# AnishDelft/ModelCompression

Measured on NVIDIA B200. Metric: yolov2_416_pruned_fwd_images_per_sec, higher is better.
Workload: dtype bf16

## Files before the change

include/mcb200.h:

```cpp
#ifndef MCB200_H_
#define MCB200_H_

#include <stddef.h>
#include <stdint.h>

#ifdef __cplusplus
extern "C" {
#endif

#define MCB200_VERSION 100
#define MC_MAX_SEGMENTS 64

int mc_version(void);
const char* mc_last_error_string(void);
int mc_device_ok(void);


int mc_kth_abs_select(const float* const* h_seg_ptrs, const int64_t* h_seg_sizes, int nseg,
                      int64_t k, float gamma, float* d_out3,
                      void* d_ws, size_t ws_bytes, void* stream);
size_t mc_workspace_bytes_kth_abs_select(int64_t n_total);

int mc_weight_prune_masks(const float* const* h_w_ptrs, float* const* h_mask_ptrs, const int64_t* h_seg_sizes,
                          int nseg, int64_t k, float gamma, float* d_out3, void* d_ws, size_t ws_bytes,
                          void* stream);
int mc_debug_select_used_fast(const void* d_ws, void* stream);
int mc_debug_select_tstamps(const void* d_ws, unsigned long long* h_out12, void* stream);

int mc_mask_apply_gt(float* const* h_w_ptrs, float* const* h_mask_ptrs, const int64_t* h_seg_sizes,
                     int nseg, const float* d_thr, int apply, void* stream);

int mc_apply_masks(float* const* h_w_ptrs, const float* const* h_mask_ptrs,
                   const int64_t* h_seg_sizes, int nseg, void* stream);

int mc_count_zeros(const float* const* h_w_ptrs, const int64_t* h_seg_sizes, int nseg,
                   int64_t* d_counts, void* stream);

int mc_masked_residual(const float* const* h_w_ptrs, const float* const* h_mask_ptrs,
                       const int64_t* h_seg_sizes, int nseg, double* d_out, void* stream);


int mc_filter_values(const float* const* h_w_ptrs, const int* h_O, const int* h_C, const int* h_kh,
                     const int* h_kw, int nlayers, float* d_values, void* stream);

int mc_filter_threshold(const float* d_values, int n, int64_t k, double gamma, double* d_thr,
                        void* d_ws, size_t ws_bytes, void* stream);
size_t mc_workspace_bytes_filter_threshold(int n);

int mc_filter_masks(const float* d_values, const double* d_thr, const int* h_O, const int* h_per_filter,
                    int nlayers, float* const* h_mask_ptrs, uint8_t* d_keep, void* stream);

int mc_filter_prune(const float* const* h_w_ptrs, const int* h_O, const int* h_C, const int* h_kh, const int* h_kw,
                    int nlayers, int64_t k, double gamma, float* d_values, double* d_thr,
                    float* const* h_mask_ptrs, uint8_t* d_keep, void* d_ws, size_t ws_bytes, void* stream);
size_t mc_workspace_bytes_filter_prune(void);

int mc_filter_prune_greedy(const float* const* h_w_ptrs, const int* h_O, const int* h_C, const int* h_kh,
                           const int* h_kw, int nlayers, int64_t zeros0, int64_t total_params, double perc,
                           int max_picks, int32_t* d_picks, int64_t* d_result, float* const* h_mask_ptrs,
                           void* d_ws, size_t ws_bytes, void* stream);
size_t mc_workspace_bytes_filter_prune_greedy(int n_filters);


int mc_decode_region(const float* d_head, int B, int H, int W, int A, int nc, const float* h_anchors,
                     float conf_thresh, int only_objectness,
                     float* d_boxes, float* d_cls, int* d_counts, void* stream);

int mc_nms_batched(float* d_boxes, const int* d_counts, int B, int cap, float nms_thresh,
                   int* d_keep, int* d_keep_counts, void* stream);

int mc_nms_detect(float* d_boxes, const int* d_counts, int B, int cap, float nms_thresh, int* d_keep,
                  int* d_keep_counts, const float* d_cls, int nc, float conf_thresh, int* d_row_counts,
                  int* d_cand_counts, void* stream);

int mc_compact_detections(const float* d_boxes, const int* d_keep, const int* d_keep_counts, const float* d_cls,
                          int B, int cap, int nc, float conf_thresh, int first_image,
                          const int64_t* d_row_offsets, float* d_out, void* stream);

int mc_bbox_ious(const float* d_boxes1, const float* d_boxes2, int64_t n, int x1y1x2y2, float* d_out, void* stream);


enum { MC_EPI_PNHWC = 0,
       MC_EPI_REORG2 = 1,
       MC_EPI_NCHW_F32 = 2,
       MC_EPI_DECODE = 4 };

typedef struct mc_decode_params {
  float* d_boxes;
  float* d_cls;
  float* d_head;
  int A, nc;
  float conf_thresh;
  int only_objectness;
  float anchors[32];
} mc_decode_params;

typedef struct mc_conv_desc {
  const void* d_in;
  const void* d_wpack;
  const float* d_scale;
  const float* d_shift;
  void* d_out;
  int B, H, W;
  int Cin, Cin_ld;
  int N, Npad;
  int ksize;
  int leaky;
  int epi_mode;
  int ldc, ch_off;
  int block_n;
  int stages;
  int block_k;
  int in_cols;
  const mc_decode_params* decode;
  void* d_ws;
  size_t ws_bytes;
  float* d_stat_sum;
  float* d_stat_sumsq;
} mc_conv_desc;

int mc_conv_fwd(const mc_conv_desc* desc, void* stream);
size_t mc_workspace_bytes_conv_fwd(const mc_conv_desc* desc);

int mc_conv_last_plan(int info[8]);

int mc_conv_direct_supported(int Cin, int N, int ksize);
int mc_conv_direct_fwd(const void* d_in, int in_is_nchw_f32, const float* d_w, const float* d_scale,
                       const float* d_shift, void* d_out, int B, int H, int W, int Cin, int Cin_ld, int N, int ldc,
                       int ksize, int leaky, int pool, void* stream);

int mc_conv_thin_geometry(int ksize, int Cin, int N, int pool, int N2, int* ct, int* nt, int* n2t);
int mc_conv_thin_fwd(const void* d_in, const float* h_w, const float* h_scale, const float* h_shift, const float* h_w2,
                     const float* h_scale2, const float* h_shift2, void* d_out, int B, int H, int W, int Cin, int Cin_ld,
                     int N, int ldc, int ksize, int leaky, int pool, int N2, int leaky2, void* stream);

int mc_conv_im2col_supported(int Cin, int in_is_nchw_f32, int N, int pool);
int mc_conv_im2col_geometry(int Cin, int in_is_nchw_f32, int N, int pool, int* cl, int* npos, int* nb, int* kpad);
int mc_conv_im2col_fwd(const void* d_in, int in_is_nchw_f32, const void* d_wexp, const float* d_scale,
                       const float* d_shift, void* d_out, int B, int H, int W, int Cin, int Cin_ld, int N, int ldc,
                       int leaky, int pool, void* stream);

int mc_conv_window_supported(int Cin, int in_kind, int N, int pool);
int mc_conv_window_geometry(int Cin, int in_kind, int N, int pool, int* npos, int* nb, int* kcols);
int mc_conv_window_fwd(const void* d_in, int in_kind, const void* d_w, const float* d_scale, const float* d_shift,
                       void* d_out, int B, int H, int W, int Cin, int N, int ldc, int leaky, int pool, void* stream);

int mc_debug_conv_trace(void* d_buf);

int mc_debug_im2col_timeout(void);

int mc_pack_conv_weights(const float* d_w, const float* d_mask, int O, int C, int ksize,
                         const int* d_oidx, int n_o, const int* d_cidx, int n_c,
                         void* d_wpack, int Npad, int Kc, void* stream);

int mc_maxpool2x2(const void* d_in, void* d_out, int B, int H, int W, int C, int ld_in, int ld_out,
                  void* stream);

int mc_unpack_pnhwc(const void* d_in, float* d_out, int B, int H, int W, int C, int ld_in, int ch_off,
                    void* stream);

int mc_reorg_nchw(const float* d_in, float* d_out, int B, int C, int H, int W, int stride, void* stream);

int mc_pack_pnhwc(const float* d_in, void* d_out, int B, int H, int W, int C, int ld_out, void* stream);



int mc_col_stats(const void* d_z, int64_t rows, int C, int ld, int ch_off, float* d_sum, float* d_sumsq, void* stream);

int mc_bn_finalize(const float* d_sum, const float* d_sumsq, int C, double count, const float* d_gamma,
                   const float* d_beta, float eps, float momentum, float* d_running_mean, float* d_running_var,
                   float* d_scale, float* d_shift, float* d_mean, float* d_invstd, void* stream);

int mc_bn_apply(const void* d_z, int ld_z, int B, int H, int W, int C, const float* d_scale, const float* d_shift,
                int leaky, void* d_out, int ld_out, int ch_off, int reorg, void* stream);

int mc_bn_backward(const void* d_z, int ld_z, const void* d_da, int ld_da, int ch_off, int reorg, int B, int H, int W,
                   int C, const float* d_mean, const float* d_invstd, const float* d_gamma, const float* d_beta,
                   int leaky, float* d_dbeta, float* d_dgamma, void* d_dz, int ld_dz, void* stream);

int mc_maxpool2x2_backward(const void* d_a_full, int ld_a, const void* d_dpooled, int ld_dp, int B, int H, int W, int C,
                           void* d_dfull, int ld_df, int accumulate, void* stream);

int mc_bn_pool_supported(int C);
int mc_bn_apply_pool(const void* d_z, int ld_z, int B, int H, int W, int C, const float* d_scale, const float* d_shift,
                     int leaky, void* d_pooled, int ld_p, void* stream);
int mc_bn_pool_backward(const void* d_z, int ld_z, const void* d_dpooled, int ld_dp, int B, int H, int W, int C,
                        const float* d_scale, const float* d_shift, const float* d_mean, const float* d_invstd,
                        const float* d_gamma, const float* d_beta, int leaky, float* d_dbeta, float* d_dgamma, void* d_dz,
                        int ld_dz, void* stream);

size_t mc_workspace_bytes_region_loss(int nB);
int mc_region_loss(const float* d_output, const float* d_target, int nB, int nA, int nC, int nH, int nW,
                   const double* h_anchors, float coord_scale, float noobject_scale, float object_scale,
                   float class_scale, float thresh, float* d_grad, float* d_loss, int* d_counts, void* d_ws,
                   size_t ws_bytes, void* stream);

int mc_voc_table(const float* d_dets, int64_t n, const float* d_sizes, float def_w, float def_h, int64_t* d_img,
                 int64_t* d_cls, double* d_conf, double* d_corners, void* stream);
size_t mc_workspace_bytes_voc_match(int64_t n, int64_t m);
int mc_voc_match(const int64_t* d_key, const double* d_corners, int64_t n, const int64_t* d_gkey, const double* d_gbox,
                 const uint8_t* d_gdiff, int64_t m, double ovthresh, double* d_tp, double* d_fp, void* d_ws,
                 size_t ws_bytes, void* stream);

int mc_pack_conv_weights_dgrad(const float* d_w, const float* d_mask, int O, int C, int ksize, void* d_wpack, int Cpad,
                               int Ko, void* stream);

int mc_conv_wgrad(const void* d_a, int lda, int C, const void* d_dz, int ld_dz, int O, int B, int H, int W, int ksize,
                  const float* d_mask, float* d_dw, int accumulate, void* d_ws, size_t ws_bytes, void* stream);
size_t mc_workspace_bytes_conv_wgrad(int B, int H, int W, int C, int O, int ksize);

size_t mc_workspace_bytes_conv_wgrad_first(int B, int H, int W, int C, int O);
int mc_conv_wgrad_first(const float* d_x, const void* d_dz, int ld_dz, int B, int H, int W, int C, int O,
                        const float* d_mask, float* d_dw, void* d_ws, size_t ws_bytes, void* stream);

int mc_sgd_momentum_step(float* const* h_param_ptrs, const float* const* h_grad_ptrs, float* const* h_buf_ptrs,
                         const int64_t* h_sizes, int nseg, float lr, float momentum, float weight_decay,
                         int first_step, void* stream);

#ifdef __cplusplus
}
#endif
#endif
```

modelcompression_b200/_lib.py:

```python
import ctypes
import os
from ctypes import (POINTER, c_char_p, c_double, c_float, c_int, c_int64, c_size_t, c_uint8, c_void_p)

_HERE = os.path.dirname(os.path.abspath(__file__))
LIB_PATH = os.path.join(_HERE, "libmcb200.so")

MC_MAX_SEGMENTS = 64
MC_EPI_PNHWC, MC_EPI_REORG2, MC_EPI_NCHW_F32, MC_EPI_DECODE = 0, 1, 2, 4


class McError(RuntimeError):
    """A libmcb200 entry point returned a non-zero status."""


class mc_decode_params(ctypes.Structure):
    _fields_ = [
        ("d_boxes", c_void_p), ("d_cls", c_void_p), ("d_head", c_void_p),
        ("A", c_int), ("nc", c_int), ("conf_thresh", c_float), ("only_objectness", c_int),
        ("anchors", c_float * 32),
    ]


class mc_conv_desc(ctypes.Structure):
    _fields_ = [
        ("d_in", c_void_p), ("d_wpack", c_void_p), ("d_scale", c_void_p), ("d_shift", c_void_p), ("d_out", c_void_p),
        ("B", c_int), ("H", c_int), ("W", c_int),
        ("Cin", c_int), ("Cin_ld", c_int),
        ("N", c_int), ("Npad", c_int),
        ("ksize", c_int), ("leaky", c_int), ("epi_mode", c_int),
        ("ldc", c_int), ("ch_off", c_int),
        ("block_n", c_int), ("stages", c_int), ("block_k", c_int), ("in_cols", c_int),
        ("decode", POINTER(mc_decode_params)),
        ("d_ws", c_void_p), ("ws_bytes", c_size_t),
        ("d_stat_sum", c_void_p), ("d_stat_sumsq", c_void_p),
    ]


_SIGNATURES = {
    "mc_version": (c_int, []),
    "mc_last_error_string": (c_char_p, []),
    "mc_device_ok": (c_int, []),
    "mc_kth_abs_select": (c_int, [POINTER(c_void_p), POINTER(c_int64), c_int, c_int64, c_float, c_void_p,
                                  c_void_p, c_size_t, c_void_p]),
    "mc_workspace_bytes_kth_abs_select": (c_size_t, [c_int64]),
    "mc_weight_prune_masks": (c_int, [POINTER(c_void_p), POINTER(c_void_p), POINTER(c_int64), c_int, c_int64, c_float,
                                      c_void_p, c_void_p, c_size_t, c_void_p]),
    "mc_debug_select_used_fast": (c_int, [c_void_p, c_void_p]),
    "mc_debug_select_tstamps": (c_int, [c_void_p, c_void_p, c_void_p]),
    "mc_mask_apply_gt": (c_int, [POINTER(c_void_p), POINTER(c_void_p), POINTER(c_int64), c_int, c_void_p, c_int,
                                 c_void_p]),
    "mc_apply_masks": (c_int, [POINTER(c_void_p), POINTER(c_void_p), POINTER(c_int64), c_int, c_void_p]),
    "mc_count_zeros": (c_int, [POINTER(c_void_p), POINTER(c_int64), c_int, c_void_p, c_void_p]),
    "mc_masked_residual": (c_int, [POINTER(c_void_p), POINTER(c_void_p), POINTER(c_int64), c_int, c_void_p,
                                   c_void_p]),
    "mc_filter_values": (c_int, [POINTER(c_void_p), POINTER(c_int), POINTER(c_int), POINTER(c_int), POINTER(c_int),
                                 c_int, c_void_p, c_void_p]),
    "mc_filter_threshold": (c_int, [c_void_p, c_int, c_int64, c_double, c_void_p, c_void_p, c_size_t, c_void_p]),
    "mc_workspace_bytes_filter_threshold": (c_size_t, [c_int]),
    "mc_filter_masks": (c_int, [c_void_p, c_void_p, POINTER(c_int), POINTER(c_int), c_int, POINTER(c_void_p),
                                c_void_p, c_void_p]),
    "mc_filter_prune": (c_int, [POINTER(c_void_p), POINTER(c_int), POINTER(c_int), POINTER(c_int), POINTER(c_int), c_int,
                                c_int64, c_double, c_void_p, c_void_p, POINTER(c_void_p), c_void_p, c_void_p, c_size_t,
                                c_void_p]),
    "mc_workspace_bytes_filter_prune": (c_size_t, []),
    "mc_filter_prune_greedy": (c_int, [POINTER(c_void_p), POINTER(c_int), POINTER(c_int), POINTER(c_int),
                                       POINTER(c_int), c_int, c_int64, c_int64, c_double, c_int, c_void_p, c_void_p,
                                       POINTER(c_void_p), c_void_p, c_size_t, c_void_p]),
    "mc_workspace_bytes_filter_prune_greedy": (c_size_t, [c_int]),
    "mc_decode_region": (c_int, [c_void_p, c_int, c_int, c_int, c_int, c_int, POINTER(c_float), c_float, c_int,
                                 c_void_p, c_void_p, c_void_p, c_void_p]),
    "mc_nms_batched": (c_int, [c_void_p, c_void_p, c_int, c_int, c_float, c_void_p, c_void_p, c_void_p]),
    "mc_nms_detect": (c_int, [c_void_p, c_void_p, c_int, c_int, c_float, c_void_p, c_void_p, c_void_p, c_int, c_float,
                              c_void_p, c_void_p, c_void_p]),
    "mc_compact_detections": (c_int, [c_void_p, c_void_p, c_void_p, c_void_p, c_int, c_int, c_int, c_float, c_int,
                                      c_void_p, c_void_p, c_void_p]),
    "mc_bbox_ious": (c_int, [c_void_p, c_void_p, c_int64, c_int, c_void_p, c_void_p]),
    "mc_reorg_nchw": (c_int, [c_void_p, c_void_p, c_int, c_int, c_int, c_int, c_int, c_void_p]),
    "mc_conv_fwd": (c_int, [POINTER(mc_conv_desc), c_void_p]),
    "mc_workspace_bytes_conv_fwd": (c_size_t, [POINTER(mc_conv_desc)]),
    "mc_conv_last_plan": (c_int, [POINTER(c_int)]),
    "mc_conv_direct_supported": (c_int, [c_int, c_int, c_int]),
    "mc_conv_direct_fwd": (c_int, [c_void_p, c_int, c_void_p, c_void_p, c_void_p, c_void_p, c_int, c_int, c_int, c_int,
                                   c_int, c_int, c_int, c_int, c_int, c_int, c_void_p]),
    "mc_conv_thin_geometry": (c_int, [c_int, c_int, c_int, c_int, c_int, POINTER(c_int), POINTER(c_int), POINTER(c_int)]),
    "mc_conv_thin_fwd": (c_int, [c_void_p, c_void_p, c_void_p, c_void_p, c_void_p, c_void_p, c_void_p, c_void_p, c_int,
                                 c_int, c_int, c_int, c_int, c_int, c_int, c_int, c_int, c_int, c_int, c_int, c_void_p]),
    "mc_conv_im2col_supported": (c_int, [c_int, c_int, c_int, c_int]),
    "mc_conv_im2col_geometry": (c_int, [c_int, c_int, c_int, c_int, POINTER(c_int), POINTER(c_int), POINTER(c_int),
                                        POINTER(c_int)]),
    "mc_conv_im2col_fwd": (c_int, [c_void_p, c_int, c_void_p, c_void_p, c_void_p, c_void_p, c_int, c_int, c_int, c_int,
                                   c_int, c_int, c_int, c_int, c_int, c_void_p]),
    "mc_debug_im2col_timeout": (c_int, []),
    "mc_debug_conv_trace": (c_int, [c_void_p]),
    "mc_conv_window_supported": (c_int, [c_int, c_int, c_int, c_int]),
    "mc_conv_window_geometry": (c_int, [c_int, c_int, c_int, c_int, POINTER(c_int), POINTER(c_int), POINTER(c_int)]),
    "mc_conv_window_fwd": (c_int, [c_void_p, c_int, c_void_p, c_void_p, c_void_p, c_void_p, c_int, c_int, c_int, c_int,
                                   c_int, c_int, c_int, c_int, c_void_p]),
    "mc_pack_conv_weights": (c_int, [c_void_p, c_void_p, c_int, c_int, c_int, c_void_p, c_int, c_void_p, c_int,
                                     c_void_p, c_int, c_int, c_void_p]),
    "mc_maxpool2x2": (c_int, [c_void_p, c_void_p, c_int, c_int, c_int, c_int, c_int, c_int, c_void_p]),
    "mc_unpack_pnhwc": (c_int, [c_void_p, c_void_p, c_int, c_int, c_int, c_int, c_int, c_int, c_void_p]),
    "mc_pack_pnhwc": (c_int, [c_void_p, c_void_p, c_int, c_int, c_int, c_int, c_int, c_void_p]),
    "mc_col_stats": (c_int, [c_void_p, c_int64, c_int, c_int, c_int, c_void_p, c_void_p, c_void_p]),
    "mc_bn_finalize": (c_int, [c_void_p, c_void_p, c_int, c_double, c_void_p, c_void_p, c_float, c_float, c_void_p,
                               c_void_p, c_void_p, c_void_p, c_void_p, c_void_p, c_void_p]),
    "mc_bn_apply": (c_int, [c_void_p, c_int, c_int, c_int, c_int, c_int, c_void_p, c_void_p, c_int, c_void_p, c_int,
                            c_int, c_int, c_void_p]),
    "mc_bn_backward": (c_int, [c_void_p, c_int, c_void_p, c_int, c_int, c_int, c_int, c_int, c_int, c_int, c_void_p,
                               c_void_p, c_void_p, c_void_p, c_int, c_void_p, c_void_p, c_void_p, c_int, c_void_p]),
    "mc_maxpool2x2_backward": (c_int, [c_void_p, c_int, c_void_p, c_int, c_int, c_int, c_int, c_int, c_void_p, c_int,
                                       c_int, c_void_p]),
    "mc_workspace_bytes_region_loss": (c_size_t, [c_int]),
    "mc_region_loss": (c_int, [c_void_p, c_void_p, c_int, c_int, c_int, c_int, c_int, POINTER(c_double), c_float, c_float,
                               c_float, c_float, c_float, c_void_p, c_void_p, c_void_p, c_void_p, c_size_t, c_void_p]),
    "mc_voc_table": (c_int, [c_void_p, c_int64, c_void_p, c_float, c_float, c_void_p, c_void_p, c_void_p, c_void_p, c_void_p]),
    "mc_workspace_bytes_voc_match": (c_size_t, [c_int64, c_int64]),
    "mc_voc_match": (c_int, [c_void_p, c_void_p, c_int64, c_void_p, c_void_p, c_void_p, c_int64, c_double, c_void_p,
                             c_void_p, c_void_p, c_size_t, c_void_p]),
    "mc_bn_pool_supported": (c_int, [c_int]),
    "mc_bn_apply_pool": (c_int, [c_void_p, c_int, c_int, c_int, c_int, c_int, c_void_p, c_void_p, c_int, c_void_p, c_int,
                                 c_void_p]),
    "mc_bn_pool_backward": (c_int, [c_void_p, c_int, c_void_p, c_int, c_int, c_int, c_int, c_int, c_void_p, c_void_p,
                                    c_void_p, c_void_p, c_void_p, c_void_p, c_int, c_void_p, c_void_p, c_void_p, c_int,
                                    c_void_p]),
    "mc_pack_conv_weights_dgrad": (c_int, [c_void_p, c_void_p, c_int, c_int, c_int, c_void_p, c_int, c_int, c_void_p]),
    "mc_conv_wgrad": (c_int, [c_void_p, c_int, c_int, c_void_p, c_int, c_int, c_int, c_int, c_int, c_int, c_void_p,
                              c_void_p, c_int, c_void_p, c_size_t, c_void_p]),
    "mc_workspace_bytes_conv_wgrad": (c_size_t, [c_int, c_int, c_int, c_int, c_int, c_int]),
    "mc_conv_wgrad_first": (c_int, [c_void_p, c_void_p, c_int, c_int, c_int, c_int, c_int, c_int, c_void_p, c_void_p,
                                    c_void_p, c_size_t, c_void_p]),
    "mc_workspace_bytes_conv_wgrad_first": (c_size_t, [c_int, c_int, c_int, c_int, c_int]),
    "mc_sgd_momentum_step": (c_int, [POINTER(c_void_p), POINTER(c_void_p), POINTER(c_void_p), POINTER(c_int64), c_int,
                                     c_float, c_float, c_float, c_int, c_void_p]),
}

EXPORTED_SYMBOLS = tuple(sorted(_SIGNATURES))

_lib = None


def load():
    global _lib
    if _lib is not None:
        return _lib
    if not os.path.exists(LIB_PATH):
        raise ImportError(
            "modelcompression_b200: %s is not built. There is no CPU/PyTorch fallback for this path; build it with "
            "`python -c 'import __graft_entry__ as g; g.build()'` or `make -C modelcompression_b200/csrc`." % LIB_PATH)
    lib = ctypes.CDLL(LIB_PATH)
    for name, (res, args) in _SIGNATURES.items():
        fn = getattr(lib, name)
        fn.restype = res
        fn.argtypes = args
    _lib = lib
    return lib


def check(rc, what=""):
    if rc != 0:
        msg = load().mc_last_error_string()
        raise McError("%s failed (%d): %s" % (what or "libmcb200 call", rc, msg.decode() if msg else "?"))


def stream_ptr():
    import torch
    return c_void_p(torch.cuda.current_stream().cuda_stream)


def ptr_array(tensors):
    arr = (c_void_p * len(tensors))()
    for i, t in enumerate(tensors):
        arr[i] = None if t is None else t.data_ptr()
    return arr


def int64_array(vals):
    return (c_int64 * len(vals))(*[int(v) for v in vals])


def int_array(vals):
    return (c_int * len(vals))(*[int(v) for v in vals])


def require_cuda(t, what):
    if not t.is_cuda:
        raise RuntimeError(
            "%s: tensor is on %s. modelcompression_b200 runs this path on a B200 (sm_100a) only; there is no CPU "
            "fallback (move the model/tensors to CUDA)." % (what, t.device))
```

modelcompression_b200/csrc/conv_tcgen05.cu:

```cuda
#include <cuda.h>
#include <stdio.h>
#include <stdlib.h>
#include "common.cuh"
#include "ptx_sm100.cuh"
#include "tmap.cuh"
#include "decode_math.cuh"

namespace {

constexpr int BLOCK_M = 128;
constexpr int MAX_STAGES = 8;
constexpr int MAX_A_STAGES = 3;
constexpr int A_BOX_ROWS = BLOCK_M + 8;
constexpr int A_BOX_BYTES = A_BOX_ROWS * 128;
constexpr int A_BOX_STRIDE = 18 * 1024;
constexpr int ACC_STAGES = 2;
constexpr int NUM_THREADS = 192;

struct ConvKParams {
  int M_rows;
  int N;
  int Npad;
  int num_kb;
  int kb_per_tap;
  int block_k;
  int ksize;
  int Wp, Hp, W, H;
  int block_n, stages, tmem_cols, acc_stride;
  int out_pitch;
  int out_chunk;
  int tma_bufs;
  float* stat_sum;
  float* stat_sumsq;
  unsigned int wp_mul, wp_shr, hp_mul, hp_shr;
  int last_ksteps;
  int share_dx, a_stages;
  int m_tiles, n_tiles;
  uint32_t idesc;
  const float* scale;
  const float* shift;
  void* out;
  int ldc, ch_off, epi_mode, leaky;
  int sk_first, sk_units;
  int sk_gper, sk_total_g;
  int sk_clusters;
  unsigned int* sk_count;
  float* sk_part;
  float* dec_boxes;
  float* dec_cls;
  float* dec_head;
  int dec_A, dec_nc, dec_only_obj;
  float dec_thresh;
  McAnchors dec_anc;
  unsigned long long* dbg;
};

__device__ __forceinline__ void conv_stamp(const ConvKParams& p, int slot) {
  if (p.dbg != nullptr && slot < 32) {
    unsigned long long t;
    asm volatile("mov.u64 %0, %%globaltimer;" : "=l"(t));
    p.dbg[(size_t)blockIdx.x * 32 + slot] = t;
  }
}

template <bool LEAKY>
__device__ __forceinline__ void scale_act16(const uint32_t (&r)[16], const float* __restrict__ sc,
                                            const float* __restrict__ sh, bool interior, float (&v)[16]) {
#pragma unroll
  for (int q = 0; q < 4; ++q) {
    const float4 a = *reinterpret_cast<const float4*>(sc + 4 * q);
    const float4 b = *reinterpret_cast<const float4*>(sh + 4 * q);
    v[4 * q + 0] = fmaf(__uint_as_float(r[4 * q + 0]), a.x, b.x);
    v[4 * q + 1] = fmaf(__uint_as_float(r[4 * q + 1]), a.y, b.y);
    v[4 * q + 2] = fmaf(__uint_as_float(r[4 * q + 2]), a.z, b.z);
    v[4 * q + 3] = fmaf(__uint_as_float(r[4 * q + 3]), a.w, b.w);
  }
#pragma unroll
  for (int j = 0; j < 16; ++j) {
    if (LEAKY) v[j] = fmaxf(v[j], 0.1f * v[j]);
    v[j] = interior ? v[j] : 0.f;
  }
}

template <int MODE>
__device__ __forceinline__ void store16(const ConvKParams& p, const float (&v)[16], int nbase, long long out_row_base,
                                        bool vec_ok) {
  if (MODE == MC_EPI_NCHW_F32 || MODE == MC_EPI_DECODE) {
    float* out_f = reinterpret_cast<float*>(p.out);
    const long long hw = (long long)p.H * p.W;
#pragma unroll
    for (int j = 0; j < 16; ++j)
      if (nbase + j < p.N) out_f[out_row_base + (long long)(nbase + j) * hw] = v[j];
  } else {
    __nv_bfloat16* out_bf = reinterpret_cast<__nv_bfloat16*>(p.out) + out_row_base;
#pragma unroll
    for (int g = 0; g < 2; ++g) {
      const int n = nbase + g * 8;
      if (n >= p.N) continue;
      const bool full = n + 8 <= p.N;
      if (vec_ok && (full || (MODE == MC_EPI_PNHWC && p.ch_off + n + 8 <= p.ldc))) {
        float w[8];
#pragma unroll
        for (int j = 0; j < 8; ++j) w[j] = (full || n + j < p.N) ? v[g * 8 + j] : 0.f;
        __nv_bfloat162 h0 = __floats2bfloat162_rn(w[0], w[1]);
        __nv_bfloat162 h1 = __floats2bfloat162_rn(w[2], w[3]);
        __nv_bfloat162 h2 = __floats2bfloat162_rn(w[4], w[5]);
        __nv_bfloat162 h3 = __floats2bfloat162_rn(w[6], w[7]);
        uint4 pk;
        pk.x = *reinterpret_cast<uint32_t*>(&h0);
        pk.y = *reinterpret_cast<uint32_t*>(&h1);
        pk.z = *reinterpret_cast<uint32_t*>(&h2);
        pk.w = *reinterpret_cast<uint32_t*>(&h3);
        *reinterpret_cast<uint4*>(out_bf + n) = pk;
      } else {
#pragma unroll
        for (int j = 0; j < 8; ++j)
          if (n + j < p.N) out_bf[n + j] = __float2bfloat16_rn(v[g * 8 + j]);
      }
    }
  }
}

__device__ __forceinline__ void pack16_to_smem(const float (&v)[16], uint8_t* dst) {
#pragma unroll
  for (int g = 0; g < 2; ++g) {
    __nv_bfloat162 h0 = __floats2bfloat162_rn(v[g * 8 + 0], v[g * 8 + 1]);
    __nv_bfloat162 h1 = __floats2bfloat162_rn(v[g * 8 + 2], v[g * 8 + 3]);
    __nv_bfloat162 h2 = __floats2bfloat162_rn(v[g * 8 + 4], v[g * 8 + 5]);
    __nv_bfloat162 h3 = __floats2bfloat162_rn(v[g * 8 + 6], v[g * 8 + 7]);
    uint4 pk;
    pk.x = *reinterpret_cast<uint32_t*>(&h0);
    pk.y = *reinterpret_cast<uint32_t*>(&h1);
    pk.z = *reinterpret_cast<uint32_t*>(&h2);
    pk.w = *reinterpret_cast<uint32_t*>(&h3);
    *reinterpret_cast<uint4*>(dst + g * 16) = pk;
  }
}

__device__ __forceinline__ void pack16_to_slab(const float (&v)[16], uint8_t* row, int chunk, int lane) {
#pragma unroll
  for (int g = 0; g < 2; ++g) {
    __nv_bfloat162 h0 = __floats2bfloat162_rn(v[g * 8 + 0], v[g * 8 + 1]);
    __nv_bfloat162 h1 = __floats2bfloat162_rn(v[g * 8 + 2], v[g * 8 + 3]);
    __nv_bfloat162 h2 = __floats2bfloat162_rn(v[g * 8 + 4], v[g * 8 + 5]);
    __nv_bfloat162 h3 = __floats2bfloat162_rn(v[g * 8 + 6], v[g * 8 + 7]);
    uint4 pk;
    pk.x = *reinterpret_cast<uint32_t*>(&h0);
    pk.y = *reinterpret_cast<uint32_t*>(&h1);
    pk.z = *reinterpret_cast<uint32_t*>(&h2);
    pk.w = *reinterpret_cast<uint32_t*>(&h3);
    *reinterpret_cast<uint4*>(row + (((chunk + g) ^ (lane & 7)) << 4)) = pk;
  }
}

__device__ __forceinline__ void slab_stats(const uint8_t* sb, float* acc , int col0, int lane) {
  float s0 = 0.f, s1 = 0.f, q0 = 0.f, q1 = 0.f;
  const int j = lane >> 2, w = lane & 3;
#pragma unroll 8
  for (int r = 0; r < 32; ++r) {
    const uint32_t u = *reinterpret_cast<const uint32_t*>(sb + r * 128 + ((j ^ (r & 7)) << 4) + w * 4);
    const float a = __uint_as_float(u << 16), b = __uint_as_float(u & 0xffff0000u);
    s0 += a; s1 += b;
    q0 = fmaf(a, a, q0); q1 = fmaf(b, b, q1);
  }
  acc[col0 + 2 * lane] += s0;
  acc[col0 + 2 * lane + 1] += s1;
  acc[256 + col0 + 2 * lane] += q0;
  acc[256 + col0 + 2 * lane + 1] += q1;
}
__device__ __forceinline__ void flush_stats(const ConvKParams& p, float* acc, int n0, int lane) {
  for (int c = lane; c < p.block_n; c += 32) {
    if (n0 + c < p.N) {
      atomicAdd(p.stat_sum + n0 + c, acc[c]);
      atomicAdd(p.stat_sumsq + n0 + c, acc[256 + c]);
    }
    acc[c] = 0.f;
    acc[256 + c] = 0.f;
  }
  __syncwarp();
}

template <bool LEAKY, bool PAIR, bool WIDE_LD, typename AddFn>
__device__ __forceinline__ void epilogue_tile_tma(const ConvKParams& p, const CUtensorMap* tm_out, uint32_t taddr_row,
                                                  const float* sc, const float* sh, bool interior, bool in_buf,
                                                  int row0, int n0, long long out_row_base, bool vec_ok, uint8_t* slab,
                                                  int& buf, uint64_t* empty_bar, AddFn add, float* stat_acc = nullptr) {
  const int lane = threadIdx.x & 31;
  int cols_valid = ((p.N - n0 + 7) >> 3) << 3;
  if (cols_valid > p.block_n) cols_valid = p.block_n;
  const int full_cols = p.block_n & ~63;
  for (int cc = 0; cc < full_cols && cc < cols_valid; cc += 64) {
    uint8_t* sb = slab + (size_t)buf * 4096;
    if (lane == 0) {
      if (p.tma_bufs >= 2) ptx::bulk_wait_group_read<1>();
      else ptx::bulk_wait_group_read<0>();
    }
    __syncwarp();
    uint8_t* mine = sb + lane * 128;
    if (WIDE_LD) {
      uint32_t r[4][16];
#pragma unroll
      for (int q = 0; q < 4; ++q) ptx::tmem_ld_32x32b_x16(taddr_row + (uint32_t)(cc + 16 * q), r[q]);
      ptx::tmem_ld_wait();
#pragma unroll
      for (int q = 0; q < 4; ++q) {
        add(r[q], cc + 16 * q);
        float v[16];
        scale_act16<LEAKY>(r[q], sc + cc + 16 * q, sh + cc + 16 * q, interior, v);
        pack16_to_slab(v, mine, 2 * q, lane);
      }
    } else {
#pragma unroll
      for (int h = 0; h < 2; ++h) {
        uint32_t r0[16], r1[16];
        ptx::tmem_ld_32x32b_x16(taddr_row + (uint32_t)(cc + 32 * h), r0);
        ptx::tmem_ld_32x32b_x16(taddr_row + (uint32_t)(cc + 32 * h + 16), r1);
        ptx::tmem_ld_wait();
        add(r0, cc + 32 * h);
        add(r1, cc + 32 * h + 16);
        float v[16];
        scale_act16<LEAKY>(r0, sc + cc + 32 * h, sh + cc + 32 * h, interior, v);
        pack16_to_slab(v, mine, 4 * h, lane);
        scale_act16<LEAKY>(r1, sc + cc + 32 * h + 16, sh + cc + 32 * h + 16, interior, v);
        pack16_to_slab(v, mine, 4 * h + 2, lane);
      }
    }
    ptx::fence_proxy_async_smem();
    __syncwarp();
    if (lane == 0) {
      ptx::tma_store_2d(tm_out, sb, n0 + cc, row0);
      ptx::bulk_commit_group();
    }
    if (stat_acc != nullptr) slab_stats(sb, stat_acc, cc, lane);
    if (p.tma_bufs >= 2) buf ^= 1;
  }
  for (int c0 = full_cols; c0 < p.block_n; c0 += 32) {
    uint32_t r0[16], r1[16];
    const bool two = c0 + 16 < p.block_n;
    ptx::tmem_ld_32x32b_x16(taddr_row + (uint32_t)c0, r0);
    if (two) ptx::tmem_ld_32x32b_x16(taddr_row + (uint32_t)(c0 + 16), r1);
    ptx::tmem_ld_wait();
    if (!in_buf) continue;
    add(r0, c0);
    if (two) add(r1, c0 + 16);
    float v[16];
    scale_act16<LEAKY>(r0, sc + c0, sh + c0, interior, v);
    store16<MC_EPI_PNHWC>(p, v, n0 + c0, out_row_base, vec_ok);
    if (two) {
      scale_act16<LEAKY>(r1, sc + c0 + 16, sh + c0 + 16, interior, v);
      store16<MC_EPI_PNHWC>(p, v, n0 + c0 + 16, out_row_base, vec_ok);
    }
  }
  ptx::tc_fence_before();
  __syncwarp();
  if (lane == 0) {
    if (PAIR) ptx::mbar_arrive_leader(empty_bar);
    else ptx::mbar_arrive(empty_bar);
  }
}

template <int MODE, bool LEAKY, bool PAIR = false, bool WIDE_LD = false>
__device__ __forceinline__ void epilogue_loop(const ConvKParams& p, uint32_t tmem_base, uint64_t* tmem_full_bar,
                                              uint64_t* tmem_empty_bar, float* s_ss, uint8_t* s_out = nullptr,
                                              const CUtensorMap* tm_out = nullptr,
                                              int tile0 = -1, int tile_step = 0, int total_units = 0, int pair_rank = 0) {
  const int warp_idx = threadIdx.x >> 5;
  const int lane = threadIdx.x & 31;
  const int et = threadIdx.x - 64;
  const int quarter = warp_idx & 3;
  const int total_tiles = PAIR ? total_units : p.m_tiles * p.n_tiles;
  if (!PAIR) { tile0 = blockIdx.x; tile_step = gridDim.x; }
  const bool vec_ok = ((p.ldc | p.ch_off) & 7) == 0 && (MODE != MC_EPI_REORG2 || (p.N & 7) == 0);
  int as = 0;
  uint32_t aphase = 0;
  int slab_buf = 0;
  float* stat_acc = nullptr;
  int stat_n0 = -1;
  if (MODE == MC_EPI_PNHWC && p.tma_bufs > 0 && p.stat_sum != nullptr) {
    stat_acc = reinterpret_cast<float*>(s_out + (size_t)4 * p.tma_bufs * 4096) + quarter * 512;
    for (int c = lane; c < 512; c += 32) stat_acc[c] = 0.f;
    __syncwarp();
  }
  const bool one_n_tile = p.n_tiles == 1;
  if (one_n_tile) {
    for (int i = et; i < p.block_n; i += 128) {
      const bool ok = i < p.Npad;
      s_ss[i] = ok ? __ldg(p.scale + i) : 0.f;
      s_ss[256 + i] = ok ? __ldg(p.shift + i) : 0.f;
    }
    asm volatile("bar.sync 1, 128;" ::: "memory");
  }
  int ti = 0;
  for (int tile = tile0; tile < total_tiles; tile += tile_step, ++ti) {
    const int n0 = (tile % p.n_tiles) * p.block_n;
    const int m0 = (PAIR ? 2 * (tile / p.n_tiles) + pair_rank : tile / p.n_tiles) * BLOCK_M;
    float* sc = s_ss + (one_n_tile ? 0 : as * 512);
    float* sh = sc + 256;
    if (!one_n_tile) {
      for (int i = et; i < p.block_n; i += 128) {
        const bool ok = (n0 + i) < p.Npad;
        sc[i] = ok ? __ldg(p.scale + n0 + i) : 0.f;
        sh[i] = ok ? __ldg(p.shift + n0 + i) : 0.f;
      }
    }
    const int row = m0 + quarter * 32 + lane;
    const int t = (int)(__umulhi((unsigned int)row, p.wp_mul) >> p.wp_shr);
    const int x = row - t * p.Wp;
    const int b = (int)(__umulhi((unsigned int)t, p.hp_mul) >> p.hp_shr);
    const int y = t - b * p.Hp;
    const bool in_buf = row < p.M_rows;
    const bool interior = in_buf && (x < p.W) && (y < p.H);
    long long out_row_base = 0;
    bool do_store = false;
    if (MODE == MC_EPI_PNHWC) {
      out_row_base = (long long)row * p.ldc + p.ch_off;
      do_store = in_buf;
    } else if (MODE == MC_EPI_REORG2) {
      const int Wo = p.W / 2 + 1, Ho = p.H / 2 + 1;
      const long long orow = ((long long)b * Ho + (y >> 1)) * Wo + (x >> 1);
      out_row_base = orow * p.ldc + p.ch_off + ((y & 1) * 2 + (x & 1)) * p.N;
      do_store = interior;
    } else {
      out_row_base = ((long long)b * p.N * p.H + y) * p.W + x;
      do_store = interior;
    }
    if (!one_n_tile) asm volatile("bar.sync 1, 128;" ::: "memory");

    ptx::mbar_wait(&tmem_full_bar[as], aphase);
    ptx::tc_fence_after();
    if (!PAIR && et == 0 && ti < 8) conv_stamp(p, 12 + 2 * ti);
    const uint32_t taddr_row = tmem_base + ((uint32_t)(quarter * 32) << 16) + (uint32_t)(as * p.acc_stride);

    if (MODE == MC_EPI_PNHWC && p.tma_bufs > 0) {
      if (stat_acc != nullptr && n0 != stat_n0) {
        if (stat_n0 >= 0) flush_stats(p, stat_acc, stat_n0, lane);
        stat_n0 = n0;
      }
      epilogue_tile_tma<LEAKY, PAIR, WIDE_LD>(p, tm_out, taddr_row, sc, sh, interior, in_buf, m0 + quarter * 32, n0, out_row_base,
                                     vec_ok, s_out + (size_t)quarter * p.tma_bufs * 4096, slab_buf, &tmem_empty_bar[as],
                                     [](uint32_t (&)[16], int) {}, stat_acc);
      if (!PAIR && et == 0 && ti < 8) conv_stamp(p, 13 + 2 * ti);
      if (++as == ACC_STAGES) { as = 0; aphase ^= 1u; }
      continue;
    }

    if (MODE == MC_EPI_PNHWC && s_out != nullptr) {
      const int pitch = p.out_pitch;
      const int chunk = p.out_chunk;
      uint8_t* wbuf = s_out + (size_t)quarter * 32 * pitch;
      uint8_t* mine = wbuf + (size_t)lane * pitch;
      const int row0 = m0 + quarter * 32;
      int cols_left = ((p.N - n0 + 7) >> 3) << 3;
      if (cols_left > p.block_n) cols_left = p.block_n;
      for (int cc = 0; cc < p.block_n; cc += chunk) {
        const int cw = (p.block_n - cc < chunk) ? p.block_n - cc : chunk;
        for (int c0 = 0; c0 < cw; c0 += 32) {
          uint32_t r0[16], r1[16];
          const bool two = c0 + 16 < cw;
          ptx::tmem_ld_32x32b_x16(taddr_row + (uint32_t)(cc + c0), r0);
          if (two) ptx::tmem_ld_32x32b_x16(taddr_row + (uint32_t)(cc + c0 + 16), r1);
          ptx::tmem_ld_wait();
          float v[16];
          scale_act16<LEAKY>(r0, sc + cc + c0, sh + cc + c0, interior, v);
          pack16_to_smem(v, mine + c0 * 2);
          if (two) {
            scale_act16<LEAKY>(r1, sc + cc + c0 + 16, sh + cc + c0 + 16, interior, v);
            pack16_to_smem(v, mine + (c0 + 16) * 2);
          }
        }
        if (cc + chunk >= p.block_n) {
          ptx::tc_fence_before();
          __syncwarp();
          if (lane == 0) {
            if (PAIR) ptx::mbar_arrive_leader(&tmem_empty_bar[as]);
            else ptx::mbar_arrive(&tmem_empty_bar[as]);
          }
        } else {
          __syncwarp();
        }
        int cols_w = cols_left - cc;
        if (cols_w > cw) cols_w = cw;
        if (cols_w > 0) {
          const int cpr = cols_w >> 3;
          int r = lane / cpr, c = lane - r * cpr;
          const int dr = 32 / cpr, dc = 32 - dr * cpr;
          __nv_bfloat16* obase = reinterpret_cast<__nv_bfloat16*>(p.out) + p.ch_off + n0 + cc;
          while (r < 32) {
            if (row0 + r < p.M_rows)
              *reinterpret_cast<uint4*>(obase + (long long)(row0 + r) * p.ldc + c * 8) =
                  *reinterpret_cast<const uint4*>(wbuf + (size_t)r * pitch + c * 16);
            r += dr; c += dc;
            if (c >= cpr) { c -= cpr; ++r; }
          }
        }
        __syncwarp();
      }
      if (!PAIR && et == 0 && ti < 8) conv_stamp(p, 13 + 2 * ti);
      if (++as == ACC_STAGES) { as = 0; aphase ^= 1u; }
      continue;
    }

    if (MODE == MC_EPI_DECODE) {
      const int pitch_f = p.block_n + 1;
      float* mine = reinterpret_cast<float*>(s_out) + (size_t)(quarter * 32 + lane) * pitch_f;
      for (int c0 = 0; c0 < p.block_n; c0 += 16) {
        uint32_t r0[16];
        ptx::tmem_ld_32x32b_x16(taddr_row + (uint32_t)c0, r0);
        ptx::tmem_ld_wait();
        float v[16];
        scale_act16<LEAKY>(r0, sc + c0, sh + c0, true, v);
#pragma unroll
        for (int j = 0; j < 16; ++j) mine[c0 + j] = v[j];
      }
      ptx::tc_fence_before();
      __syncwarp();
      if (lane == 0) ptx::mbar_arrive(&tmem_empty_bar[as]);
      if (interior) {
        const int A = p.dec_A, nc = p.dec_nc, F = 5 + p.dec_nc;
        const long long P = (long long)p.H * p.W * A;
        const long long slot0 = (long long)(y * p.W + x) * A;
        if (p.dec_head != nullptr) {
          float* hd = p.dec_head + ((long long)b * p.N * p.H + y) * p.W + x;
          const long long hw = (long long)p.H * p.W;
          for (int n = 0; n < p.N; ++n) hd[n * hw] = mine[n];
        }
        for (int a = 0; a < A; ++a) {
          const float* row = mine + a * F;
          const McDecoded d = mc_decode_anchor([row](int f) { return row[f]; }, nc, x, y, p.W, p.H, p.dec_anc.w[a],
                                               p.dec_anc.h[a], p.dec_thresh, p.dec_only_obj);
          float* dst = p.dec_boxes + ((long long)b * P + slot0 + a) * 8;
          reinterpret_cast<float4*>(dst)[0] = make_float4(d.bx, d.by, d.bw, d.bh);
          reinterpret_cast<float4*>(dst)[1] =
              make_float4(d.conf, d.cmax, (float)d.cid, d.cand ? (float)(slot0 + a) : -1.0f);
          if (d.cand && p.dec_cls != nullptr) {
            float* cd = p.dec_cls + ((long long)b * P + slot0 + a) * nc;
            for (int c = 0; c < nc; ++c) cd[c] = __fdiv_rn(expf(__fsub_rn(row[5 + c], d.cls_max_logit)), d.cls_sum);
          }
        }
      }
      __syncwarp();
      if (++as == ACC_STAGES) { as = 0; aphase ^= 1u; }
      continue;
    }

    for (int c0 = 0; c0 < p.block_n; c0 += 32) {
      uint32_t r0[16], r1[16];
      const bool two = c0 + 16 < p.block_n;
      ptx::tmem_ld_32x32b_x16(taddr_row + (uint32_t)c0, r0);
      if (two) ptx::tmem_ld_32x32b_x16(taddr_row + (uint32_t)(c0 + 16), r1);
      ptx::tmem_ld_wait();
      if (!do_store) continue;
      float v[16];
      scale_act16<LEAKY>(r0, sc + c0, sh + c0, interior, v);
      store16<MODE>(p, v, n0 + c0, out_row_base, vec_ok);
      if (two) {
        scale_act16<LEAKY>(r1, sc + c0 + 16, sh + c0 + 16, interior, v);
        store16<MODE>(p, v, n0 + c0 + 16, out_row_base, vec_ok);
      }
    }
    ptx::tc_fence_before();
    __syncwarp();
    if (lane == 0) {
      if (PAIR) ptx::mbar_arrive_leader(&tmem_empty_bar[as]);
      else ptx::mbar_arrive(&tmem_empty_bar[as]);
    }
    if (!PAIR && et == 0 && ti < 8) conv_stamp(p, 13 + 2 * ti);
    if (++as == ACC_STAGES) { as = 0; aphase ^= 1u; }
  }
  if (stat_acc != nullptr && stat_n0 >= 0) flush_stats(p, stat_acc, stat_n0, lane);
  if (MODE == MC_EPI_PNHWC && p.tma_bufs > 0 && lane == 0) ptx::bulk_wait_group_read<0>();
}

template <int MINB>
__global__ void __launch_bounds__(NUM_THREADS, MINB)
conv_gemm_tcgen05_kernel(const __grid_constant__ CUtensorMap tmap_a, const __grid_constant__ CUtensorMap tmap_b,
                         const __grid_constant__ CUtensorMap tmap_abox, const __grid_constant__ CUtensorMap tmap_out,
                         const ConvKParams p) {
  extern __shared__ __align__(1024) uint8_t smem_raw[];
  const uint32_t a_tile_bytes = (uint32_t)(BLOCK_M * p.block_k * 2);
  const uint32_t b_tile_bytes = (uint32_t)(p.block_n * p.block_k * 2);
  const uint32_t stage_bytes = a_tile_bytes + b_tile_bytes;
  uint8_t* smem = smem_raw;
  {
    uint32_t a = ptx::smem_u32(smem);
    smem += (1024u - (a & 1023u)) & 1023u;
  }
  uint8_t* tiles = smem;
  const uint32_t a_row_bytes = (uint32_t)p.block_k * 2u;
  const uint32_t a_box_bytes = (uint32_t)A_BOX_ROWS * a_row_bytes;
  const uint32_t a_box_stride = p.block_k == 64 ? (uint32_t)A_BOX_STRIDE : (uint32_t)A_BOX_STRIDE / 2u;
  uint8_t* b_ring = tiles + (size_t)p.a_stages * a_box_stride;
  uint8_t* aux = p.share_dx ? b_ring + (size_t)p.stages * b_tile_bytes : tiles + (size_t)p.stages * stage_bytes;
  uint64_t* full_bar = reinterpret_cast<uint64_t*>(aux);
  uint64_t* empty_bar = full_bar + MAX_STAGES;
  uint64_t* tmem_full_bar = empty_bar + MAX_STAGES;
  uint64_t* tmem_empty_bar = tmem_full_bar + ACC_STAGES;
  uint64_t* afull_bar = tmem_empty_bar + ACC_STAGES;
  uint64_t* aempty_bar = afull_bar + MAX_A_STAGES;
  uint32_t* tmem_ptr_smem = reinterpret_cast<uint32_t*>(aempty_bar + MAX_A_STAGES);
  float* s_ss = reinterpret_cast<float*>(aux + 512);
  uint8_t* s_out = aux + 5120;

  const int warp_idx = threadIdx.x >> 5;
  const int lane = threadIdx.x & 31;
  const int total_tiles = p.m_tiles * p.n_tiles;
  if (threadIdx.x == 0) conv_stamp(p, 0);

  if (warp_idx == 0 && lane == 0) {
    ptx::prefetch_tensormap(&tmap_a);
    ptx::prefetch_tensormap(&tmap_b);
    for (int s = 0; s < p.stages; ++s) {
      ptx::mbar_init(&full_bar[s], 1);
      ptx::mbar_init(&empty_bar[s], 1);
    }
    for (int a = 0; a < ACC_STAGES; ++a) {
      ptx::mbar_init(&tmem_full_bar[a], 1);
      ptx::mbar_init(&tmem_empty_bar[a], 4);
    }
    for (int a = 0; a < MAX_A_STAGES; ++a) {
      ptx::mbar_init(&afull_bar[a], 1);
      ptx::mbar_init(&aempty_bar[a], 1);
    }
    ptx::prefetch_tensormap(&tmap_abox);
    if (p.tma_bufs > 0) ptx::prefetch_tensormap(&tmap_out);
    ptx::fence_barrier_init();
  }
  if (warp_idx == 1) {
    ptx::tmem_alloc(tmem_ptr_smem, (uint32_t)p.tmem_cols);
    ptx::tmem_relinquish();
  }
  ptx::tc_fence_before();
  __syncthreads();
  ptx::tc_fence_after();
  const uint32_t tmem_base = *tmem_ptr_smem;
  if (threadIdx.x == 0) conv_stamp(p, 1);

  if (warp_idx == 0) {
    if (lane == 0 && p.share_dx) {
      int s = 0, sa = 0;
      uint32_t phase = 0, pha = 0;
      for (int tile = blockIdx.x; tile < total_tiles; tile += gridDim.x) {
        const int n0 = (tile % p.n_tiles) * p.block_n;
        const int m0 = (tile / p.n_tiles) * BLOCK_M;
        for (int g = 0; g < 3 * p.kb_per_tap; ++g) {
          const int dy = g / p.kb_per_tap, cb = g - dy * p.kb_per_tap;
          ptx::mbar_wait(&aempty_bar[sa], pha ^ 1u);
          ptx::mbar_arrive_expect_tx(&afull_bar[sa], a_box_bytes);
          ptx::tma_load_2d(tiles + (size_t)sa * a_box_stride, &tmap_abox, &afull_bar[sa], cb * p.block_k,
                           m0 + (dy - 1) * p.Wp - 1);
          if (++sa == p.a_stages) { sa = 0; pha ^= 1u; }
          for (int dx = 0; dx < 3; ++dx) {
            const int kb = (dy * 3 + dx) * p.kb_per_tap + cb;
            ptx::mbar_wait(&empty_bar[s], phase ^ 1u);
            ptx::mbar_arrive_expect_tx(&full_bar[s], b_tile_bytes);
            ptx::tma_load_2d(b_ring + (size_t)s * b_tile_bytes, &tmap_b, &full_bar[s], kb * p.block_k, n0);
            if (++s == p.stages) { s = 0; phase ^= 1u; }
          }
        }
      }
      conv_stamp(p, 3);
    } else if (lane == 0) {
      int s = 0;
      uint32_t phase = 0;
      for (int tile = blockIdx.x; tile < total_tiles; tile += gridDim.x) {
        const int n0 = (tile % p.n_tiles) * p.block_n;
        const int m0 = (tile / p.n_tiles) * BLOCK_M;
        for (int kb = 0; kb < p.num_kb; ++kb) {
          const int tap = kb / p.kb_per_tap;
          const int cb = kb - tap * p.kb_per_tap;
          int row_off = 0;
          if (p.ksize == 3) row_off = (tap / 3 - 1) * p.Wp + (tap % 3 - 1);
          ptx::mbar_wait(&empty_bar[s], phase ^ 1u);
          uint8_t* a_dst = tiles + (size_t)s * stage_bytes;
          uint8_t* b_dst = a_dst + a_tile_bytes;
          ptx::mbar_arrive_expect_tx(&full_bar[s], stage_bytes);
          ptx::tma_load_2d(a_dst, &tmap_a, &full_bar[s], cb * p.block_k, m0 + row_off);
          ptx::tma_load_2d(b_dst, &tmap_b, &full_bar[s], kb * p.block_k, n0);
          if (++s == p.stages) { s = 0; phase ^= 1u; }
        }
      }
      conv_stamp(p, 3);
    }
  } else if (warp_idx == 1) {
    if (p.share_dx) {
      int s = 0, sa = 0, as = 0;
      uint32_t phase = 0, pha = 0, aphase = 0;
      int ti = 0;
      for (int tile = blockIdx.x; tile < total_tiles; tile += gridDim.x, ++ti) {
        ptx::mbar_wait(&tmem_empty_bar[as], aphase ^ 1u);
        ptx::tc_fence_after();
        const uint32_t tmem_acc = tmem_base + (uint32_t)(as * p.acc_stride);
        for (int g = 0; g < 3 * p.kb_per_tap; ++g) {
          const int dy = g / p.kb_per_tap, cb = g - dy * p.kb_per_tap;
          const int nk = (cb == p.kb_per_tap - 1) ? p.last_ksteps : (int)(a_row_bytes >> 5);
          ptx::mbar_wait(&afull_bar[sa], pha);
          if (ti == 0 && g == 0 && lane == 0) conv_stamp(p, 4);
          const uint32_t a_addr = ptx::smem_u32(tiles + (size_t)sa * a_box_stride);
          for (int dx = 0; dx < 3; ++dx) {
            ptx::mbar_wait(&full_bar[s], phase);
            ptx::tc_fence_after();
            const uint32_t b_addr = ptx::smem_u32(b_ring + (size_t)s * b_tile_bytes);
            const bool k64 = p.block_k == 64;
            const uint64_t adesc = k64 ? ptx::make_sw128_kmajor_desc(a_addr + (uint32_t)dx * 128u)
                                       : ptx::make_sw64_kmajor_desc(a_addr + (uint32_t)dx * 64u);
            const uint64_t bdesc = k64 ? ptx::make_sw128_kmajor_desc(b_addr) : ptx::make_sw64_kmajor_desc(b_addr);
            if (ptx::elect_one()) {
#pragma unroll
              for (int k = 0; k < 4; ++k)
                if (k < nk)
                  ptx::umma_bf16_ss(tmem_acc, adesc + (uint64_t)(2 * k), bdesc + (uint64_t)(2 * k), p.idesc,
                                    (g > 0 || dx > 0 || k > 0) ? 1u : 0u);
              ptx::umma_commit(&empty_bar[s]);
              if (dx == 2) ptx::umma_commit(&aempty_bar[sa]);
              if (dx == 2 && g == 3 * p.kb_per_tap - 1) ptx::umma_commit(&tmem_full_bar[as]);
            }
            __syncwarp();
            if (++s == p.stages) { s = 0; phase ^= 1u; }
          }
          if (++sa == p.a_stages) { sa = 0; pha ^= 1u; }
        }
        if (lane == 0 && ti < 6) conv_stamp(p, 5 + ti);
        if (++as == ACC_STAGES) { as = 0; aphase ^= 1u; }
      }
    } else {
      int s = 0;
      uint32_t phase = 0;
      int as = 0;
      uint32_t aphase = 0;
      int ti = 0;
      for (int tile = blockIdx.x; tile < total_tiles; tile += gridDim.x, ++ti) {
        ptx::mbar_wait(&tmem_empty_bar[as], aphase ^ 1u);
        ptx::tc_fence_after();
        const uint32_t tmem_acc = tmem_base + (uint32_t)(as * p.acc_stride);
        int cb_i = 0;
        for (int kb = 0; kb < p.num_kb; ++kb) {
          ptx::mbar_wait(&full_bar[s], phase);
          ptx::tc_fence_after();
          if (ti == 0 && kb == 0 && lane == 0) conv_stamp(p, 4);
          const uint32_t a_addr = ptx::smem_u32(tiles + (size_t)s * stage_bytes);
          const bool k64 = p.block_k == 64;
          const uint64_t adesc = k64 ? ptx::make_sw128_kmajor_desc(a_addr) : ptx::make_sw64_kmajor_desc(a_addr);
          const uint64_t bdesc = k64 ? ptx::make_sw128_kmajor_desc(a_addr + a_tile_bytes)
                                     : ptx::make_sw64_kmajor_desc(a_addr + a_tile_bytes);
          const int ksteps = (cb_i == p.kb_per_tap - 1) ? p.last_ksteps : p.block_k / 16;
          if (++cb_i == p.kb_per_tap) cb_i = 0;
          if (ptx::elect_one()) {
#pragma unroll
            for (int k = 0; k < 4; ++k) {
              if (k < ksteps)
                ptx::umma_bf16_ss(tmem_acc, adesc + (uint64_t)(2 * k), bdesc + (uint64_t)(2 * k), p.idesc,
                                  (kb > 0 || k > 0) ? 1u : 0u);
            }
            ptx::umma_commit(&empty_bar[s]);
            if (kb == p.num_kb - 1) ptx::umma_commit(&tmem_full_bar[as]);
          }
          __syncwarp();
          if (++s == p.stages) { s = 0; phase ^= 1u; }
        }
        if (lane == 0 && ti < 6) conv_stamp(p, 5 + ti);
        if (++as == ACC_STAGES) { as = 0; aphase ^= 1u; }
      }
    }
  } else {
    if (p.epi_mode == MC_EPI_PNHWC) {
      uint8_t* so = (p.out_pitch || p.tma_bufs) ? s_out : nullptr;
      if (p.leaky) epilogue_loop<MC_EPI_PNHWC, true, false, MINB == 1>(p, tmem_base, tmem_full_bar, tmem_empty_bar, s_ss, so, &tmap_out);
      else epilogue_loop<MC_EPI_PNHWC, false, false, MINB == 1>(p, tmem_base, tmem_full_bar, tmem_empty_bar, s_ss, so, &tmap_out);
    } else if (p.epi_mode == MC_EPI_REORG2) {
      if (p.leaky) epilogue_loop<MC_EPI_REORG2, true>(p, tmem_base, tmem_full_bar, tmem_empty_bar, s_ss);
      else epilogue_loop<MC_EPI_REORG2, false>(p, tmem_base, tmem_full_bar, tmem_empty_bar, s_ss);
    } else if (p.epi_mode == MC_EPI_DECODE) {
      epilogue_loop<MC_EPI_DECODE, false>(p, tmem_base, tmem_full_bar, tmem_empty_bar, s_ss, s_out);
    } else {
      if (p.leaky) epilogue_loop<MC_EPI_NCHW_F32, true>(p, tmem_base, tmem_full_bar, tmem_empty_bar, s_ss);
      else epilogue_loop<MC_EPI_NCHW_F32, false>(p, tmem_base, tmem_full_bar, tmem_empty_bar, s_ss);
    }
  }

  ptx::tc_fence_before();
  __syncthreads();
  if (threadIdx.x == 0) conv_stamp(p, 30);
  if (warp_idx == 1) ptx::tmem_dealloc(tmem_base, (uint32_t)p.tmem_cols);
}

struct PairWork {
  int unit;
  int g0, g1;
  int kind;
  int aux;
};

struct PairWorkIter {
  int next_full, step, sk_first;
  int sk_state;
  int c, G, gper, T, units;
  __device__ __forceinline__ void init(const ConvKParams& p, int cluster_id, int num_clusters) {
    next_full = cluster_id;
    step = num_clusters;
    sk_first = p.sk_first;
    c = cluster_id; G = p.sk_clusters; gper = p.sk_gper; T = p.sk_total_g; units = p.sk_units;
    sk_state = (p.sk_units > 0 && c < G) ? 0 : 2;
  }
  __device__ __forceinline__ int span_begin(int cl) const { return (int)(((long long)cl * T) / G); }
  __device__ __forceinline__ void describe(int u, int a, int b, PairWork& w) const {
    w.unit = sk_first + u;
    w.g0 = a;
    w.g1 = b;
    int cf = c;
    while (cf > 0 && span_begin(cf) > u * gper) --cf;
    if (b == gper) {
      w.kind = (a == 0) ? 0 : 2;
      w.aux = c - cf;
    } else {
      w.kind = 1;
      w.aux = c - cf;
    }
  }
  __device__ __forceinline__ bool next(PairWork& w) {
    if (next_full < sk_first) {
      w.unit = next_full; w.g0 = 0; w.g1 = -1; w.kind = 0; w.aux = 0;
      next_full += step;
      return true;
    }
    if (sk_state == 2) return false;
    const int r0 = span_begin(c), r1 = span_begin(c + 1);
    if (r1 <= r0) { sk_state = 2; return false; }
    const int u0 = r0 / gper, u1 = (r1 - 1) / gper;
    if (u0 == u1) {
      sk_state = 2;
      describe(u0, r0 - u0 * gper, r1 - u0 * gper, w);
      return true;
    }
    if (sk_state == 0) {
      sk_state = 1;
      describe(u1, 0, r1 - u1 * gper, w);
      return true;
    }
    sk_state = 2;
    describe(u0, r0 - u0 * gper, gper, w);
    return true;
  }
};

template <int MODE, bool LEAKY>
__device__ __forceinline__ void epilogue_loop_pair(const ConvKParams& p, uint32_t tmem_base, uint64_t* tmem_full_bar,
                                                   uint64_t* tmem_empty_bar, float* s_ss, int cluster_id, int num_clusters,
                                                   int pair_rank, uint8_t* s_out, const CUtensorMap* tm_out) {
  const int warp_idx = threadIdx.x >> 5;
  const int lane = threadIdx.x & 31;
  const int et = threadIdx.x - 64;
  const int quarter = warp_idx & 3;
  const bool vec_ok = ((p.ldc | p.ch_off) & 7) == 0 && (MODE != MC_EPI_REORG2 || (p.N & 7) == 0);
  int as = 0;
  uint32_t aphase = 0;
  int slab_buf = 0;
  float* stat_acc = nullptr;
  int stat_n0 = -1;
  if (MODE == MC_EPI_PNHWC && p.tma_bufs > 0 && p.stat_sum != nullptr) {
    stat_acc = reinterpret_cast<float*>(s_out + (size_t)4 * p.tma_bufs * 4096) + quarter * 512;
    for (int c = lane; c < 512; c += 32) stat_acc[c] = 0.f;
    __syncwarp();
  }
  const bool one_n_tile = p.n_tiles == 1;
  if (one_n_tile) {
    for (int i = et; i < p.block_n; i += 128) {
      const bool ok = i < p.Npad;
      s_ss[i] = ok ? __ldg(p.scale + i) : 0.f;
      s_ss[256 + i] = ok ? __ldg(p.shift + i) : 0.f;
    }
    asm volatile("bar.sync 1, 128;" ::: "memory");
  }
  PairWorkIter it;
  it.init(p, cluster_id, num_clusters);
  PairWork w;
  int ti = -1;
  while (it.next(w)) {
    ++ti;
    const int tile = w.unit;
    const int n0 = (tile % p.n_tiles) * p.block_n;
    const int m0 = (2 * (tile / p.n_tiles) + pair_rank) * BLOCK_M;
    float* sc = s_ss + (one_n_tile ? 0 : as * 512);
    float* sh = sc + 256;
    if (!one_n_tile) {
      for (int i = et; i < p.block_n; i += 128) {
        const bool ok = (n0 + i) < p.Npad;
        sc[i] = ok ? __ldg(p.scale + n0 + i) : 0.f;
        sh[i] = ok ? __ldg(p.shift + n0 + i) : 0.f;
      }
    }
    const int row = m0 + quarter * 32 + lane;
    const int t = (int)(__umulhi((unsigned int)row, p.wp_mul) >> p.wp_shr);
    const int x = row - t * p.Wp;
    const int b = (int)(__umulhi((unsigned int)t, p.hp_mul) >> p.hp_shr);
    const int y = t - b * p.Hp;
    const bool in_buf = row < p.M_rows;
    const bool interior = in_buf && (x < p.W) && (y < p.H);
    long long out_row_base = 0;
    bool do_store = false;
    if (MODE == MC_EPI_PNHWC) {
      out_row_base = (long long)row * p.ldc + p.ch_off;
      do_store = in_buf;
    } else if (MODE == MC_EPI_REORG2) {
      const int Wo = p.W / 2 + 1, Ho = p.H / 2 + 1;
      const long long orow = ((long long)b * Ho + (y >> 1)) * Wo + (x >> 1);
      out_row_base = orow * p.ldc + p.ch_off + ((y & 1) * 2 + (x & 1)) * p.N;
      do_store = interior;
    } else {
      out_row_base = ((long long)b * p.N * p.H + y) * p.W + x;
      do_store = interior;
    }
    if (!one_n_tile) asm volatile("bar.sync 1, 128;" ::: "memory");

    ptx::mbar_wait(&tmem_full_bar[as], aphase);
    ptx::tc_fence_after();
    if (et == 0 && ti < 8) conv_stamp(p, 12 + 2 * ti);
    const uint32_t taddr_row = tmem_base + ((uint32_t)(quarter * 32) << 16) + (uint32_t)(as * p.acc_stride);
    const int u_sk = tile - p.sk_first;
    const int prow = pair_rank * 128 + quarter * 32 + lane;
    const size_t slot_stride = (size_t)256 * p.block_n;
    float* part_unit = p.sk_part + (size_t)(u_sk < 0 ? 0 : u_sk) * 3 * slot_stride;
    auto part_ptr = [&](int slot, int col) -> float* {
      return part_unit + (size_t)slot * slot_stride + ((size_t)(col >> 2) * 256 + prow) * 4;
    };
    if (w.kind == 1) {
      for (int c0 = 0; c0 < p.block_n; c0 += 32) {
        uint32_t r0[16], r1[16];
        const bool two = c0 + 16 < p.block_n;
        ptx::tmem_ld_32x32b_x16(taddr_row + (uint32_t)c0, r0);
        if (two) ptx::tmem_ld_32x32b_x16(taddr_row + (uint32_t)(c0 + 16), r1);
        ptx::tmem_ld_wait();
#pragma unroll
        for (int q = 0; q < 4; ++q)
          *reinterpret_cast<uint4*>(part_ptr(w.aux, c0 + 4 * q)) = make_uint4(r0[4 * q], r0[4 * q + 1], r0[4 * q + 2], r0[4 * q + 3]);
        if (two) {
#pragma unroll
          for (int q = 0; q < 4; ++q)
            *reinterpret_cast<uint4*>(part_ptr(w.aux, c0 + 16 + 4 * q)) = make_uint4(r1[4 * q], r1[4 * q + 1], r1[4 * q + 2], r1[4 * q + 3]);
        }
      }
      ptx::tc_fence_before();
      __threadfence();
      __syncwarp();
      if (lane == 0) {
        atomicAdd(p.sk_count + u_sk, 1u);
        ptx::mbar_arrive_leader(&tmem_empty_bar[as]);
      }
    } else {
      const int nparts = w.kind == 2 ? w.aux : 0;
      if (nparts > 0) {
        if (lane == 0) {
          const unsigned int want = 8u * (unsigned int)nparts;
          unsigned int spins = 0;
          while (*reinterpret_cast<volatile unsigned int*>(p.sk_count + u_sk) < want) {
            if (++spins > (1u << 24)) __trap();
          }
          if (atomicAdd(p.sk_count + 256 + u_sk, 1u) == 7u) {
            p.sk_count[256 + u_sk] = 0u;
            p.sk_count[u_sk] = 0u;
          }
        }
        __syncwarp();
        __threadfence();
      }
      if (MODE == MC_EPI_PNHWC && p.tma_bufs > 0) {
        if (stat_acc != nullptr && n0 != stat_n0) {
          if (stat_n0 >= 0) flush_stats(p, stat_acc, stat_n0, lane);
          stat_n0 = n0;
        }
        epilogue_tile_tma<LEAKY, true, true>(p, tm_out, taddr_row, sc, sh, interior, in_buf, m0 + quarter * 32, n0, out_row_base,
                                       vec_ok, s_out + (size_t)quarter * p.tma_bufs * 4096, slab_buf, &tmem_empty_bar[as],
                                       [&](uint32_t (&r)[16], int col) {
                                         for (int s2 = 0; s2 < nparts; ++s2) {
#pragma unroll
                                           for (int q = 0; q < 4; ++q) {
                                             const float4 a = __ldcg(reinterpret_cast<const float4*>(part_ptr(s2, col + 4 * q)));
                                             r[4 * q] = __float_as_uint(__uint_as_float(r[4 * q]) + a.x);
                                             r[4 * q + 1] = __float_as_uint(__uint_as_float(r[4 * q + 1]) + a.y);
                                             r[4 * q + 2] = __float_as_uint(__uint_as_float(r[4 * q + 2]) + a.z);
                                             r[4 * q + 3] = __float_as_uint(__uint_as_float(r[4 * q + 3]) + a.w);
                                           }
                                         }
                                       }, stat_acc);
        if (et == 0 && ti < 8) conv_stamp(p, 13 + 2 * ti);
        if (++as == ACC_STAGES) { as = 0; aphase ^= 1u; }
        continue;
      }
      for (int c0 = 0; c0 < p.block_n; c0 += 32) {
        uint32_t r0[16], r1[16];
        const bool two = c0 + 16 < p.block_n;
        ptx::tmem_ld_32x32b_x16(taddr_row + (uint32_t)c0, r0);
        if (two) ptx::tmem_ld_32x32b_x16(taddr_row + (uint32_t)(c0 + 16), r1);
        ptx::tmem_ld_wait();
        if (!do_store) continue;
        for (int s2 = 0; s2 < nparts; ++s2) {
#pragma unroll
          for (int q = 0; q < 4; ++q) {
            const float4 a = __ldcg(reinterpret_cast<const float4*>(part_ptr(s2, c0 + 4 * q)));
            r0[4 * q] = __float_as_uint(__uint_as_float(r0[4 * q]) + a.x);
            r0[4 * q + 1] = __float_as_uint(__uint_as_float(r0[4 * q + 1]) + a.y);
            r0[4 * q + 2] = __float_as_uint(__uint_as_float(r0[4 * q + 2]) + a.z);
            r0[4 * q + 3] = __float_as_uint(__uint_as_float(r0[4 * q + 3]) + a.w);
          }
          if (two) {
#pragma unroll
            for (int q = 0; q < 4; ++q) {
              const float4 a = __ldcg(reinterpret_cast<const float4*>(part_ptr(s2, c0 + 16 + 4 * q)));
              r1[4 * q] = __float_as_uint(__uint_as_float(r1[4 * q]) + a.x);
              r1[4 * q + 1] = __float_as_uint(__uint_as_float(r1[4 * q + 1]) + a.y);
              r1[4 * q + 2] = __float_as_uint(__uint_as_float(r1[4 * q + 2]) + a.z);
              r1[4 * q + 3] = __float_as_uint(__uint_as_float(r1[4 * q + 3]) + a.w);
            }
          }
        }
        float v[16];
        scale_act16<LEAKY>(r0, sc + c0, sh + c0, interior, v);
        store16<MODE>(p, v, n0 + c0, out_row_base, vec_ok);
        if (two) {
          scale_act16<LEAKY>(r1, sc + c0 + 16, sh + c0 + 16, interior, v);
          store16<MODE>(p, v, n0 + c0 + 16, out_row_base, vec_ok);
        }
      }
      ptx::tc_fence_before();
      __syncwarp();
      if (lane == 0) ptx::mbar_arrive_leader(&tmem_empty_bar[as]);
    }
    if (et == 0 && ti < 8) conv_stamp(p, 13 + 2 * ti);
    if (++as == ACC_STAGES) { as = 0; aphase ^= 1u; }
  }
  if (stat_acc != nullptr && stat_n0 >= 0) flush_stats(p, stat_acc, stat_n0, lane);
  if (MODE == MC_EPI_PNHWC && p.tma_bufs > 0 && lane == 0) ptx::bulk_wait_group_read<0>();
}

__global__ void __cluster_dims__(2, 1, 1) __launch_bounds__(NUM_THREADS, 1)
conv_gemm_tcgen05_pair_kernel(const __grid_constant__ CUtensorMap tmap_b, const __grid_constant__ CUtensorMap tmap_abox,
                              const __grid_constant__ CUtensorMap tmap_out, const ConvKParams p) {
  extern __shared__ __align__(1024) uint8_t smem_raw[];
  const uint32_t b_half_bytes = (uint32_t)(p.block_n / 2 * 128);
  uint8_t* smem = smem_raw;
  {
    uint32_t a = ptx::smem_u32(smem);
    smem += (1024u - (a & 1023u)) & 1023u;
  }
  uint8_t* tiles = smem;
  uint8_t* b_ring = tiles + (size_t)p.a_stages * A_BOX_STRIDE;
  uint8_t* aux = b_ring + (size_t)p.stages * b_half_bytes;
  uint64_t* full_bar = reinterpret_cast<uint64_t*>(aux);
  uint64_t* empty_bar = full_bar + MAX_STAGES;
  uint64_t* tmem_full_bar = empty_bar + MAX_STAGES;
  uint64_t* tmem_empty_bar = tmem_full_bar + ACC_STAGES;
  uint64_t* afull_bar = tmem_empty_bar + ACC_STAGES;
  uint64_t* aempty_bar = afull_bar + MAX_A_STAGES;
  uint32_t* tmem_ptr_smem = reinterpret_cast<uint32_t*>(aempty_bar + MAX_A_STAGES);
  float* s_ss = reinterpret_cast<float*>(aux + 512);
  uint8_t* s_out = aux + 5120;

  const int warp_idx = threadIdx.x >> 5;
  const int lane = threadIdx.x & 31;
  const int rank = (int)ptx::cluster_ctarank();
  const int cluster_id = blockIdx.x >> 1, num_clusters = gridDim.x >> 1;
  if (threadIdx.x == 0) conv_stamp(p, 0);

  if (warp_idx == 0 && lane == 0) {
    ptx::prefetch_tensormap(&tmap_b);
    ptx::prefetch_tensormap(&tmap_abox);
    if (p.tma_bufs > 0) ptx::prefetch_tensormap(&tmap_out);
    for (int s = 0; s < p.stages; ++s) {
      ptx::mbar_init(&full_bar[s], 1);
      ptx::mbar_init(&empty_bar[s], 1);
    }
    for (int a = 0; a < ACC_STAGES; ++a) {
      ptx::mbar_init(&tmem_full_bar[a], 1);
      ptx::mbar_init(&tmem_empty_bar[a], 8);
    }
    for (int a = 0; a < MAX_A_STAGES; ++a) {
      ptx::mbar_init(&afull_bar[a], 1);
      ptx::mbar_init(&aempty_bar[a], 1);
    }
    ptx::fence_barrier_init();
  }
  if (warp_idx == 1) {
    ptx::tmem_alloc_pair(tmem_ptr_smem, (uint32_t)p.tmem_cols);
    ptx::tmem_relinquish_pair();
  }
  ptx::tc_fence_before();
  ptx::cluster_sync_all();
  ptx::tc_fence_after();
  const uint32_t tmem_base = *tmem_ptr_smem;
  if (threadIdx.x == 0) conv_stamp(p, 1);

  if (warp_idx == 0) {
    if (lane == 0) {
      int s = 0, sa = 0;
      uint32_t phase = 0, pha = 0;
      PairWorkIter it;
      it.init(p, cluster_id, num_clusters);
      PairWork w;
      while (it.next(w)) {
        const int unit = w.unit;
        const int n0 = (unit % p.n_tiles) * p.block_n + rank * (p.block_n / 2);
        const int m0 = (2 * (unit / p.n_tiles) + rank) * BLOCK_M;
        const int gb = w.g0, ge = w.g1 < 0 ? 3 * p.kb_per_tap : w.g1;
        for (int g = gb; g < ge; ++g) {
          const int dy = g / p.kb_per_tap, cb = g - dy * p.kb_per_tap;
          ptx::mbar_wait(&aempty_bar[sa], pha ^ 1u);
          if (rank == 0) ptx::mbar_arrive_expect_tx(&afull_bar[sa], 2 * A_BOX_BYTES);
          ptx::tma_load_2d_pair(tiles + (size_t)sa * A_BOX_STRIDE, &tmap_abox, &afull_bar[sa], cb * 64,
                                m0 + (dy - 1) * p.Wp - 1);
          if (++sa == p.a_stages) { sa = 0; pha ^= 1u; }
          for (int dx = 0; dx < 3; ++dx) {
            const int kb = (dy * 3 + dx) * p.kb_per_tap + cb;
            ptx::mbar_wait(&empty_bar[s], phase ^ 1u);
            if (rank == 0) ptx::mbar_arrive_expect_tx(&full_bar[s], 2 * b_half_bytes);
            ptx::tma_load_2d_pair(b_ring + (size_t)s * b_half_bytes, &tmap_b, &full_bar[s], kb * 64, n0);
            if (++s == p.stages) { s = 0; phase ^= 1u; }
          }
        }
      }
      conv_stamp(p, 3);
    }
  } else if (warp_idx == 1) {
    if (rank == 0) {
      int s = 0, sa = 0, as = 0;
      uint32_t phase = 0, pha = 0, aphase = 0;
      PairWorkIter it;
      it.init(p, cluster_id, num_clusters);
      PairWork w;
      int ti = -1;
      while (it.next(w)) {
        ++ti;
        ptx::mbar_wait(&tmem_empty_bar[as], aphase ^ 1u);
        ptx::tc_fence_after();
        const uint32_t tmem_acc = tmem_base + (uint32_t)(as * p.acc_stride);
        const int gb = w.g0, ge = w.g1 < 0 ? 3 * p.kb_per_tap : w.g1;
        for (int g = gb; g < ge; ++g) {
          const int nk = ((g % p.kb_per_tap) == p.kb_per_tap - 1) ? p.last_ksteps : 4;
          ptx::mbar_wait(&afull_bar[sa], pha);
          if (ti == 0 && g == gb && lane == 0) conv_stamp(p, 4);
          const uint32_t a_addr = ptx::smem_u32(tiles + (size_t)sa * A_BOX_STRIDE);
          for (int dx = 0; dx < 3; ++dx) {
            ptx::mbar_wait(&full_bar[s], phase);
            ptx::tc_fence_after();
            const uint64_t adesc = ptx::make_sw128_kmajor_desc(a_addr + (uint32_t)dx * 128u);
            const uint64_t bdesc = ptx::make_sw128_kmajor_desc(ptx::smem_u32(b_ring + (size_t)s * b_half_bytes));
            if (ptx::elect_one()) {
#pragma unroll
              for (int k = 0; k < 4; ++k)
                if (k < nk)
                  ptx::umma_bf16_ss_pair(tmem_acc, adesc + (uint64_t)(2 * k), bdesc + (uint64_t)(2 * k), p.idesc,
                                         (g > gb || dx > 0 || k > 0) ? 1u : 0u);
              ptx::umma_commit_pair(&empty_bar[s]);
              if (dx == 2) ptx::umma_commit_pair(&aempty_bar[sa]);
              if (dx == 2 && g == ge - 1) ptx::umma_commit_pair(&tmem_full_bar[as]);
            }
            __syncwarp();
            if (++s == p.stages) { s = 0; phase ^= 1u; }
          }
          if (++sa == p.a_stages) { sa = 0; pha ^= 1u; }
        }
        if (lane == 0 && ti < 6) conv_stamp(p, 5 + ti);
        if (++as == ACC_STAGES) { as = 0; aphase ^= 1u; }
      }
    }
  } else {
    if (p.epi_mode == MC_EPI_PNHWC) {
      if (p.leaky) epilogue_loop_pair<MC_EPI_PNHWC, true>(p, tmem_base, tmem_full_bar, tmem_empty_bar, s_ss, cluster_id, num_clusters, rank, s_out, &tmap_out);
      else epilogue_loop_pair<MC_EPI_PNHWC, false>(p, tmem_base, tmem_full_bar, tmem_empty_bar, s_ss, cluster_id, num_clusters, rank, s_out, &tmap_out);
    } else if (p.epi_mode == MC_EPI_REORG2) {
      if (p.leaky) epilogue_loop_pair<MC_EPI_REORG2, true>(p, tmem_base, tmem_full_bar, tmem_empty_bar, s_ss, cluster_id, num_clusters, rank, s_out, &tmap_out);
      else epilogue_loop_pair<MC_EPI_REORG2, false>(p, tmem_base, tmem_full_bar, tmem_empty_bar, s_ss, cluster_id, num_clusters, rank, s_out, &tmap_out);
    } else {
      if (p.leaky) epilogue_loop_pair<MC_EPI_NCHW_F32, true>(p, tmem_base, tmem_full_bar, tmem_empty_bar, s_ss, cluster_id, num_clusters, rank, s_out, &tmap_out);
      else epilogue_loop_pair<MC_EPI_NCHW_F32, false>(p, tmem_base, tmem_full_bar, tmem_empty_bar, s_ss, cluster_id, num_clusters, rank, s_out, &tmap_out);
    }
  }

  ptx::tc_fence_before();
  ptx::cluster_sync_all();
  if (warp_idx == 1) ptx::tmem_dealloc_pair(tmem_base, (uint32_t)p.tmem_cols);
}

int pick_block_n(int Npad, int m_tiles, int num_kb, int num_sms, bool share_dx) {
  int best = 16;
  double best_cost = 1e30;
  for (int bn = 16; bn <= 256; bn += 16) {
    const int n_tiles = (Npad + bn - 1) / bn;
    const long long tiles = (long long)n_tiles * m_tiles;
    const long long rounds = (tiles + num_sms - 1) / num_sms;
    double per_kb = 2.0 * bn;
    if (128.0 + bn > per_kb) per_kb = 128.0 + bn;
    const double feed = 13.3 * ((share_dx ? 17.0 / 3.0 : 16.0) + bn / 8.0);
    if (feed > per_kb) per_kb = feed;
    const double main = per_kb * num_kb, epi = 12.0 * bn + 400.0;
    const double cost = (double)rounds * (main > epi ? main : epi) + epi + 2500.0;
    if (cost < best_cost - 1e-9) {
      best_cost = cost;
      best = bn;
    }
  }
  return best;
}

}

static thread_local int g_last_plan[8] = {0, 0, 0, 0, 0, 0, 0, 0};
static unsigned long long* g_conv_dbg = nullptr;

extern "C" int mc_debug_conv_trace(void* d_buf) {
  g_conv_dbg = reinterpret_cast<unsigned long long*>(d_buf);
  return 0;
}

extern "C" int mc_conv_last_plan(int info[8]) {
  MC_CHECK_ARG(info != nullptr, "mc_conv_last_plan: null pointer");
  for (int i = 0; i < 8; ++i) info[i] = g_last_plan[i];
  return 0;
}

extern "C" size_t mc_workspace_bytes_conv_fwd(const mc_conv_desc* d) {
  if (d == nullptr || d->ksize != 3 || d->Cin <= 32 || d->Npad < 192) return 0;
  const int clusters = mc_num_sms() / 2;
  return (size_t)2048 + (size_t)clusters * 3 * 256 * 256 * sizeof(float);
}

extern "C" int mc_conv_fwd(const mc_conv_desc* d, void* stream_) {
  cudaStream_t stream = reinterpret_cast<cudaStream_t>(stream_);
  MC_CHECK_ARG(d != nullptr, "mc_conv_fwd: null descriptor");
  MC_CHECK_ARG(d->d_in && d->d_wpack && d->d_scale && d->d_shift && (d->d_out || d->epi_mode == MC_EPI_DECODE),
               "mc_conv_fwd: null pointer");
  MC_CHECK_ARG(d->ksize == 1 || d->ksize == 3, "mc_conv_fwd: ksize must be 1 or 3 (got %d)", d->ksize);
  MC_CHECK_ARG(d->B > 0 && d->H > 0 && d->W > 0 && d->Cin > 0 && d->N > 0, "mc_conv_fwd: bad dims");
  MC_CHECK_ARG((d->Cin_ld % 8) == 0 && d->Cin <= d->Cin_ld, "mc_conv_fwd: Cin_ld must be a multiple of 8 >= Cin");
  MC_CHECK_ARG((d->Npad % 16) == 0 && d->Npad >= d->N, "mc_conv_fwd: Npad must be a multiple of 16 >= N");
  MC_CHECK_ARG(((uintptr_t)d->d_in & 15) == 0 && ((uintptr_t)d->d_wpack & 15) == 0 && ((uintptr_t)d->d_out & 15) == 0,
               "mc_conv_fwd: pointers must be 16-byte aligned");
  MC_CHECK_ARG(d->epi_mode == MC_EPI_PNHWC || d->epi_mode == MC_EPI_REORG2 || d->epi_mode == MC_EPI_NCHW_F32 ||
                   d->epi_mode == MC_EPI_DECODE,
               "mc_conv_fwd: unsupported epilogue mode %d", d->epi_mode);
  const bool decode = d->epi_mode == MC_EPI_DECODE;
  if (decode) {
    const mc_decode_params* q = d->decode;
    MC_CHECK_ARG(q != nullptr && q->d_boxes != nullptr, "mc_conv_fwd: MC_EPI_DECODE needs decode parameters with d_boxes");
    MC_CHECK_ARG(q->A > 0 && q->A <= MC_MAX_ANCHORS && q->nc > 0 && q->A * (5 + q->nc) == d->N,
                 "mc_conv_fwd: decode needs N == A*(5+nc) (N %d, A %d, nc %d)", d->N, q->A, q->nc);
    MC_CHECK_ARG(d->Npad <= 256 && d->leaky == 0, "mc_conv_fwd: decode needs a linear head of <= 256 channels");
    MC_CHECK_ARG(((uintptr_t)q->d_boxes & 15) == 0, "mc_conv_fwd: d_boxes must be 16-byte aligned");
  }
  if (d->epi_mode == MC_EPI_REORG2) MC_CHECK_ARG((d->H % 2) == 0 && (d->W % 2) == 0, "mc_conv_fwd: reorg needs even H,W");

  const int ntaps = d->ksize * d->ksize;
  const int BLOCK_K = d->block_k == 32 ? 32 : 64;
  MC_CHECK_ARG(d->block_k == 0 || d->block_k == 32 || d->block_k == 64, "mc_conv_fwd: block_k must be 0, 32 or 64");
  const int A_TILE_BYTES = BLOCK_M * BLOCK_K * 2;
  const int Kc = ((d->Cin + BLOCK_K - 1) / BLOCK_K) * BLOCK_K;
  const long long M_rows = (long long)d->B * (d->H + 1) * (d->W + 1);
  MC_CHECK_ARG(M_rows < (1ll << 31), "mc_conv_fwd: too many rows");
  const int m_tiles = (int)((M_rows + BLOCK_M - 1) / BLOCK_M);

  const int share_dx = (d->ksize == 3 && (BLOCK_K == 64 || m_tiles >= 2048)) ? 1 : 0;
  const int a_box_stride = BLOCK_K == 64 ? A_BOX_STRIDE : A_BOX_STRIDE / 2;
  int block_n = d->block_n;
  if (decode) block_n = d->Npad;
  if (block_n <= 0) block_n = pick_block_n(d->Npad, m_tiles, (ntaps * Kc + 63) / 64, mc_num_sms(), false);
  const bool want_stats = d->d_stat_sum != nullptr || d->d_stat_sumsq != nullptr;
  if (want_stats) {
    MC_CHECK_ARG(d->d_stat_sum != nullptr && d->d_stat_sumsq != nullptr, "mc_conv_fwd: d_stat_sum and d_stat_sumsq go together");
    MC_CHECK_ARG(d->epi_mode == MC_EPI_PNHWC && ((d->ldc | d->ch_off) & 7) == 0 && d->N >= 33,
                 "mc_conv_fwd: statistics need the PNHWC epilogue, 8-aligned pitch / offset and more than 32 channels");
    block_n = (block_n + 63) / 64 * 64;
    if (block_n > 256) block_n = 256;
  }
  MC_CHECK_ARG(block_n >= 16 && block_n <= 256 && (block_n % 16) == 0, "mc_conv_fwd: block_n %d invalid", block_n);
  const int n_tiles = (d->Npad + block_n - 1) / block_n;

  const int stage_bytes = A_TILE_BYTES + block_n * BLOCK_K * 2;
  const long long total_tiles = (long long)n_tiles * m_tiles;
  const int acc_stride = block_n == 16 ? 16 : ((block_n + 31) / 32) * 32;
  int tmem_cols = 32;
  while (tmem_cols < ACC_STAGES * acc_stride) tmem_cols <<= 1;
  const int num_kb = ntaps * (Kc / BLOCK_K);
  constexpr size_t AUX_BYTES = 5120 + 1024;

  const bool wide_ok = d->ksize == 3 && m_tiles >= 1024;
  const bool tma_out = d->epi_mode == MC_EPI_PNHWC && block_n >= 64 && ((d->ldc | d->ch_off) & 7) == 0;
  auto tma_bufs_for = [&](int ctas_) -> int { return tma_out ? (ctas_ == 1 ? 2 : 1) : 0; };
  const bool stage_out = !tma_out && d->epi_mode == MC_EPI_PNHWC && block_n >= 32 && (block_n <= 96 || wide_ok) &&
                         ((d->ldc | d->ch_off) & 7) == 0;
  const int out_chunk = block_n <= 96 ? block_n : 64;
  const int out_pitch = stage_out ? out_chunk * 2 + 16 : 0;
  auto out_stage_for = [&](int ctas_) -> size_t {
    return decode ? (size_t)128 * (block_n + 1) * 4
                  : (tma_out ? (size_t)tma_bufs_for(ctas_) * 4 * 4096 + (want_stats ? 4 * 512 * sizeof(float) : 0)
                             : (size_t)128 * out_pitch);
  };
  auto plan_ring = [&](int ctas, int* st, int* ast, size_t* bytes) -> bool {
    const size_t out_stage_bytes = out_stage_for(ctas);
    const long long cap = (ctas == 1 ? 220 * 1024 - (long long)AUX_BYTES : (227 * 1024) / ctas - 1024 - (long long)AUX_BYTES) - (long long)out_stage_bytes;
    if (share_dx) {
      const int b_bytes = block_n * BLOCK_K * 2;
      int a = ctas == 1 ? MAX_A_STAGES : 2;
      long long stg = (cap - (long long)a * a_box_stride) / b_bytes;
      if (stg > MAX_STAGES) stg = MAX_STAGES;
      if (stg < 3) return false;
      *st = (int)stg; *ast = a;
      *bytes = (size_t)a * a_box_stride + (size_t)stg * b_bytes + AUX_BYTES + out_stage_bytes;
    } else {
      long long stg = cap / stage_bytes;
      if (stg > MAX_STAGES) stg = MAX_STAGES;
      if (stg > num_kb * 4) stg = num_kb * 4;
      if (stg < (ctas == 1 ? 1 : 3)) return false;
      *st = (int)stg; *ast = 0;
      *bytes = (size_t)stg * stage_bytes + AUX_BYTES + out_stage_bytes;
    }
    return true;
  };
  int ctas = 1;
  {
    const double main_cycles = (double)num_kb * (BLOCK_K / 64.0) * (2.0 * block_n > 128.0 + block_n ? 2.0 * block_n : 128.0 + block_n);
    const bool narrow = main_cycles < 6000.0;
    for (int c = 3; c >= 2 && narrow; --c) {
      int st, ast;
      size_t bytes;
      if (c * tmem_cols > 512 || total_tiles < (long long)c * mc_num_sms() || !plan_ring(c, &st, &ast, &bytes)) continue;
      ctas = c;
      break;
    }
  }
  int stages = d->stages;
  int a_stages = 0;
  size_t smem_bytes;
  if (stages <= 0) {
    MC_CHECK_ARG(plan_ring(ctas, &stages, &a_stages, &smem_bytes), "mc_conv_fwd: no shared-memory ring fits block_n %d", block_n);
  } else {
    ctas = 1;
    if (share_dx) {
      a_stages = MAX_A_STAGES;
      MC_CHECK_ARG(stages >= 2 && stages <= MAX_STAGES, "mc_conv_fwd: stages %d invalid", stages);
      smem_bytes = (size_t)a_stages * a_box_stride + (size_t)stages * block_n * BLOCK_K * 2 + AUX_BYTES + out_stage_for(1);
    } else {
      MC_CHECK_ARG(stages >= 1 && stages <= MAX_STAGES, "mc_conv_fwd: stages %d invalid", stages);
      smem_bytes = (size_t)stages * stage_bytes + AUX_BYTES + out_stage_for(1);
    }
  }
  MC_CHECK_ARG(smem_bytes <= 227 * 1024, "mc_conv_fwd: smem %zu too large", smem_bytes);

  const bool pair_legal = share_dx && BLOCK_K == 64 && d->stages <= 0 && (block_n % 16) == 0 && block_n >= 64 && m_tiles >= 2;
  const bool use_pair = !decode && pair_legal && block_n >= 192 && num_kb >= 36;
  if (use_pair) {
    ctas = 1;
    a_stages = MAX_A_STAGES;
    const int b_half = block_n / 2 * 128;
    const int slab_bytes = tma_bufs_for(1) * 4 * 4096 + (want_stats ? 4 * 512 * (int)sizeof(float) : 0);
    stages = (220 * 1024 - a_stages * A_BOX_STRIDE - slab_bytes) / b_half;
    if (stages > MAX_STAGES) stages = MAX_STAGES;
    smem_bytes = (size_t)a_stages * A_BOX_STRIDE + (size_t)stages * b_half + AUX_BYTES + slab_bytes;
  }

  CUtensorMap tm_a, tm_b, tm_abox;
  MC_CHECK_ARG(d->in_cols == 0 || (d->in_cols >= d->Cin && d->in_cols <= d->Cin_ld), "mc_conv_fwd: in_cols %d outside [Cin, Cin_ld]", d->in_cols);
  const uint64_t in_cols = d->in_cols ? (uint64_t)d->in_cols : (uint64_t)d->Cin;
  int rc = mc_make_tmap_2d_bf16_k(&tm_a, d->d_in, (uint64_t)M_rows, in_cols, (uint64_t)d->Cin_ld, BLOCK_M, BLOCK_K);
  if (rc) return rc;
  tm_abox = tm_a;
  if (share_dx) {
    rc = mc_make_tmap_2d_bf16_k(&tm_abox, d->d_in, (uint64_t)M_rows, in_cols, (uint64_t)d->Cin_ld, A_BOX_ROWS, BLOCK_K);
    if (rc) return rc;
  }
  rc = mc_make_tmap_2d_bf16_k(&tm_b, d->d_wpack, (uint64_t)d->Npad, (uint64_t)ntaps * Kc, (uint64_t)ntaps * Kc,
                              (uint32_t)(use_pair ? block_n / 2 : block_n), BLOCK_K);
  if (rc) return rc;

  CUtensorMap tm_out = tm_a;
  const int tma_bufs = tma_bufs_for(use_pair ? 1 : ctas);
  if (tma_bufs) {
    uint64_t ocols = (uint64_t)((d->N + 7) / 8 * 8);
    if (ocols > (uint64_t)(d->ldc - d->ch_off)) ocols = (uint64_t)(d->ldc - d->ch_off);
    rc = mc_make_tmap_2d_bf16_k(&tm_out, reinterpret_cast<const __nv_bfloat16*>(d->d_out) + d->ch_off, (uint64_t)M_rows, ocols,
                                (uint64_t)d->ldc, 32, 64);
    if (rc) return rc;
  }

  ConvKParams p;
  p.M_rows = (int)M_rows;
  p.N = d->N;
  p.Npad = d->Npad;
  p.kb_per_tap = Kc / BLOCK_K;
  p.block_k = BLOCK_K;
  p.num_kb = ntaps * p.kb_per_tap;
  p.ksize = d->ksize;
  p.W = d->W;
  p.H = d->H;
  p.Wp = d->W + 1;
  p.Hp = d->H + 1;
  p.block_n = block_n;
  p.stages = stages;
  p.share_dx = share_dx;
  {
    const int rem = d->Cin - (Kc / BLOCK_K - 1) * BLOCK_K;
    p.last_ksteps = (rem + 15) / 16;
  }
  p.a_stages = a_stages;
  p.out_pitch = use_pair ? 0 : out_pitch;
  p.out_chunk = out_chunk;
  p.tma_bufs = tma_bufs;
  p.stat_sum = d->d_stat_sum;
  p.stat_sumsq = d->d_stat_sumsq;
  {
    auto magic = [](unsigned int dv, unsigned int* mul, unsigned int* shr) {
      unsigned int l = 0;
      while ((1u << l) < dv) ++l;
      const unsigned long long pw = 31ull + l;
      *mul = (unsigned int)((((unsigned long long)1 << pw) + dv - 1) / dv);
      *shr = (unsigned int)(pw - 32);
    };
    magic((unsigned int)(d->W + 1), &p.wp_mul, &p.wp_shr);
    magic((unsigned int)(d->H + 1), &p.hp_mul, &p.hp_shr);
  }
  p.acc_stride = acc_stride;
  p.tmem_cols = tmem_cols;
  p.m_tiles = m_tiles;
  p.n_tiles = n_tiles;
  p.idesc = (1u << 4) | (1u << 7) | (1u << 10) | ((uint32_t)(block_n >> 3) << 17) | ((uint32_t)(BLOCK_M >> 4) << 24);
  p.scale = d->d_scale;
  p.shift = d->d_shift;
  p.out = d->d_out;
  p.ldc = d->ldc;
  p.ch_off = d->ch_off;
  p.epi_mode = d->epi_mode;
  p.leaky = d->leaky;
  p.sk_first = 0; p.sk_units = 0; p.sk_gper = 0; p.sk_total_g = 0; p.sk_clusters = 0; p.sk_count = nullptr; p.sk_part = nullptr;
  p.dbg = g_conv_dbg;
  p.dec_boxes = p.dec_cls = p.dec_head = nullptr;
  p.dec_A = p.dec_nc = p.dec_only_obj = 0;
  p.dec_thresh = 0.f;
  if (decode) {
    const mc_decode_params* q = d->decode;
    p.dec_boxes = q->d_boxes;
    p.dec_cls = q->d_cls;
    p.dec_head = q->d_head;
    p.dec_A = q->A;
    p.dec_nc = q->nc;
    p.dec_only_obj = q->only_objectness;
    p.dec_thresh = q->conf_thresh;
    for (int a = 0; a < MC_MAX_ANCHORS; ++a) {
      p.dec_anc.w[a] = a < q->A ? q->anchors[2 * a] : 0.f;
      p.dec_anc.h[a] = a < q->A ? q->anchors[2 * a + 1] : 0.f;
    }
  }

  if (use_pair) {
    p.idesc = (1u << 4) | (1u << 7) | (1u << 10) | ((uint32_t)(block_n >> 3) << 17) | ((uint32_t)(256 >> 4) << 24);
    p.acc_stride = ((block_n + 31) / 32) * 32;
    p.tmem_cols = 32;
    while (p.tmem_cols < ACC_STAGES * p.acc_stride) p.tmem_cols <<= 1;
    static int max_clusters = -1;
    if (max_clusters < 0) {
      MC_CUDA(cudaFuncSetAttribute(conv_gemm_tcgen05_pair_kernel, cudaFuncAttributeMaxDynamicSharedMemorySize, 227 * 1024));
      cudaLaunchConfig_t cfg = {};
      cfg.gridDim = dim3(2 * (mc_num_sms() / 2));
      cfg.blockDim = dim3(NUM_THREADS);
      cfg.dynamicSmemBytes = 222 * 1024;
      cudaLaunchAttribute at[1];
      at[0].id = cudaLaunchAttributeClusterDimension;
      at[0].val.clusterDim.x = 2; at[0].val.clusterDim.y = 1; at[0].val.clusterDim.z = 1;
      cfg.attrs = at;
      cfg.numAttrs = 1;
      int n = 0;
      if (cudaOccupancyMaxActiveClusters(&n, conv_gemm_tcgen05_pair_kernel, &cfg) != cudaSuccess || n < 1) {
        cudaGetLastError();
        n = mc_num_sms() / 2;
      }
      max_clusters = n;
    }
    const int m_pairs = (m_tiles + 1) / 2;
    const long long units = (long long)m_pairs * n_tiles;
    const int clusters = (int)(units < max_clusters ? units : max_clusters);
    p.sk_first = (int)units;
    p.sk_units = 0;
    p.sk_gper = 3 * p.kb_per_tap;
    p.sk_total_g = 0;
    p.sk_clusters = 0;
    p.sk_count = nullptr;
    p.sk_part = nullptr;
    {
      const long long full = units / clusters, rem = units % clusters;
      const size_t need = mc_workspace_bytes_conv_fwd(d);
      if (full >= 1 && rem > 0 && rem * 2 <= (long long)clusters && d->d_ws != nullptr && need > 0 &&
          d->ws_bytes >= need && ((uintptr_t)d->d_ws & 255) == 0) {
        p.sk_first = (int)(full * clusters);
        p.sk_units = (int)rem;
        p.sk_total_g = (int)rem * p.sk_gper;
        p.sk_clusters = (int)(3 * rem < clusters ? 3 * rem : clusters);
        p.sk_count = reinterpret_cast<unsigned int*>(d->d_ws);
        p.sk_part = reinterpret_cast<float*>(reinterpret_cast<uint8_t*>(d->d_ws) + 2048);
      }
    }
    g_last_plan[0] = 1; g_last_plan[1] = block_n; g_last_plan[2] = 1; g_last_plan[3] = p.sk_units; g_last_plan[4] = 1;
    g_last_plan[5] = stages; g_last_plan[6] = 2 * clusters; g_last_plan[7] = BLOCK_K;
    conv_gemm_tcgen05_pair_kernel<<<2 * clusters, NUM_THREADS, smem_bytes, stream>>>(tm_b, tm_abox, tm_out, p);
    MC_LAUNCH_CHECK("conv_gemm_tcgen05_pair_kernel");
    return 0;
  }

  static bool attr_set = false;
  if (!attr_set) {
    MC_CUDA(cudaFuncSetAttribute(conv_gemm_tcgen05_kernel<1>, cudaFuncAttributeMaxDynamicSharedMemorySize, 227 * 1024));
    MC_CUDA(cudaFuncSetAttribute(conv_gemm_tcgen05_kernel<2>, cudaFuncAttributeMaxDynamicSharedMemorySize, 113 * 1024));
    MC_CUDA(cudaFuncSetAttribute(conv_gemm_tcgen05_kernel<3>, cudaFuncAttributeMaxDynamicSharedMemorySize, 112 * 1024));
    attr_set = true;
  }
  const long long max_ctas = (long long)mc_num_sms() * ctas;
  const int grid = (int)(total_tiles < max_ctas ? total_tiles : max_ctas);
  g_last_plan[0] = 0; g_last_plan[1] = block_n; g_last_plan[2] = ctas; g_last_plan[3] = 0;
  g_last_plan[4] = share_dx; g_last_plan[5] = stages; g_last_plan[6] = grid; g_last_plan[7] = BLOCK_K;
  if (ctas >= 3)
    conv_gemm_tcgen05_kernel<3><<<grid, NUM_THREADS, smem_bytes, stream>>>(tm_a, tm_b, tm_abox, tm_out, p);
  else if (ctas == 2)
    conv_gemm_tcgen05_kernel<2><<<grid, NUM_THREADS, smem_bytes, stream>>>(tm_a, tm_b, tm_abox, tm_out, p);
  else
    conv_gemm_tcgen05_kernel<1><<<grid, NUM_THREADS, smem_bytes, stream>>>(tm_a, tm_b, tm_abox, tm_out, p);
  MC_LAUNCH_CHECK("conv_gemm_tcgen05_kernel");
  return 0;
}
```

modelcompression_b200/csrc/ptx_sm100.cuh:

```cuda
#pragma once
#include <stdint.h>
#include <cuda_runtime.h>

namespace ptx {

__device__ __forceinline__ uint32_t smem_u32(const void* p) {
  return static_cast<uint32_t>(__cvta_generic_to_shared(p));
}

__device__ __forceinline__ bool elect_one() {
  uint32_t pred = 0;
  asm volatile(
      "{\n\t"
      ".reg .pred P;\n\t"
      "elect.sync _|P, 0xffffffff;\n\t"
      "selp.b32 %0, 1, 0, P;\n\t"
      "}\n"
      : "=r"(pred));
  return pred != 0;
}

__device__ __forceinline__ void mbar_init(uint64_t* bar, uint32_t count) {
  asm volatile("mbarrier.init.shared::cta.b64 [%0], %1;" ::"r"(smem_u32(bar)), "r"(count) : "memory");
}
__device__ __forceinline__ void fence_barrier_init() {
  asm volatile("fence.mbarrier_init.release.cluster;" ::: "memory");
}
__device__ __forceinline__ void fence_proxy_async_smem() {
  asm volatile("fence.proxy.async.shared::cta;" ::: "memory");
}
__device__ __forceinline__ void mbar_arrive_expect_tx(uint64_t* bar, uint32_t bytes) {
  asm volatile("mbarrier.arrive.expect_tx.shared::cta.b64 _, [%0], %1;" ::"r"(smem_u32(bar)), "r"(bytes)
               : "memory");
}
__device__ __forceinline__ void mbar_arrive(uint64_t* bar) {
  asm volatile("mbarrier.arrive.shared::cta.b64 _, [%0];" ::"r"(smem_u32(bar)) : "memory");
}
__device__ __forceinline__ bool mbar_try_wait(uint64_t* bar, uint32_t parity) {
  uint32_t ok;
#ifdef MC_SPIN_WAIT
  asm volatile(
      "{\n\t"
      ".reg .pred P;\n\t"
      "mbarrier.try_wait.parity.shared::cta.b64 P, [%1], %2;\n\t"
      "selp.b32 %0, 1, 0, P;\n\t"
      "}\n"
      : "=r"(ok)
      : "r"(smem_u32(bar)), "r"(parity)
      : "memory");
#else
  asm volatile(
      "{\n\t"
      ".reg .pred P;\n\t"
      "mbarrier.try_wait.parity.shared::cta.b64 P, [%1], %2, %3;\n\t"
      "selp.b32 %0, 1, 0, P;\n\t"
      "}\n"
      : "=r"(ok)
      : "r"(smem_u32(bar)), "r"(parity), "r"(10000u)
      : "memory");
#endif
  return ok != 0;
}
__device__ __forceinline__ void mbar_wait(uint64_t* bar, uint32_t parity, unsigned int* dbg_flag = nullptr,
                                          unsigned int dbg_code = 0) {
  uint32_t spins = 0;
  while (!mbar_try_wait(bar, parity)) {
    if (++spins > (1u << 16)) {
      if (dbg_flag != nullptr) {
        atomicCAS(dbg_flag, 0u, dbg_code);
        return;
      }
      if (spins > (1u << 18)) __trap();
    }
  }
}

__device__ __forceinline__ void prefetch_tensormap(const void* tmap) {
  asm volatile("prefetch.tensormap [%0];" ::"l"(reinterpret_cast<uint64_t>(tmap)) : "memory");
}
__device__ __forceinline__ void tma_load_2d(void* smem_dst, const void* tmap, uint64_t* bar, int c0, int c1) {
  asm volatile(
      "cp.async.bulk.tensor.2d.shared::cluster.global.mbarrier::complete_tx::bytes [%0], [%1, {%3, %4}], [%2];"
      ::"r"(smem_u32(smem_dst)), "l"(reinterpret_cast<uint64_t>(tmap)), "r"(smem_u32(bar)), "r"(c0), "r"(c1)
      : "memory");
}
__device__ __forceinline__ void tma_load_3d(void* smem_dst, const void* tmap, uint64_t* bar, int c0, int c1,
                                            int c2) {
  asm volatile(
      "cp.async.bulk.tensor.3d.shared::cluster.global.mbarrier::complete_tx::bytes [%0], [%1, {%3, %4, %5}], [%2];"
      ::"r"(smem_u32(smem_dst)), "l"(reinterpret_cast<uint64_t>(tmap)), "r"(smem_u32(bar)), "r"(c0), "r"(c1),
      "r"(c2)
      : "memory");
}

__device__ __forceinline__ void tma_load_4d(void* smem_dst, const void* tmap, uint64_t* bar, int c0, int c1,
                                            int c2, int c3) {
  asm volatile(
      "cp.async.bulk.tensor.4d.shared::cluster.global.mbarrier::complete_tx::bytes [%0], [%1, {%3, %4, %5, %6}], [%2];"
      ::"r"(smem_u32(smem_dst)), "l"(reinterpret_cast<uint64_t>(tmap)), "r"(smem_u32(bar)), "r"(c0), "r"(c1),
      "r"(c2), "r"(c3)
      : "memory");
}

__device__ __forceinline__ void tma_store_2d(const void* tmap, const void* smem_src, int c0, int c1) {
  asm volatile("cp.async.bulk.tensor.2d.global.shared::cta.bulk_group [%0, {%2, %3}], [%1];"
               ::"l"(reinterpret_cast<uint64_t>(tmap)), "r"(smem_u32(smem_src)), "r"(c0), "r"(c1)
               : "memory");
}
__device__ __forceinline__ void bulk_commit_group() { asm volatile("cp.async.bulk.commit_group;" ::: "memory"); }
template <int N>
__device__ __forceinline__ void bulk_wait_group_read() {
  asm volatile("cp.async.bulk.wait_group.read %0;" ::"n"(N) : "memory");
}

__device__ __forceinline__ void tmem_alloc(uint32_t* smem_dst, uint32_t ncols) {
  asm volatile("tcgen05.alloc.cta_group::1.sync.aligned.shared::cta.b32 [%0], %1;" ::"r"(smem_u32(smem_dst)),
               "r"(ncols)
               : "memory");
}
__device__ __forceinline__ void tmem_relinquish() {
  asm volatile("tcgen05.relinquish_alloc_permit.cta_group::1.sync.aligned;" ::: "memory");
}
__device__ __forceinline__ void tmem_dealloc(uint32_t taddr, uint32_t ncols) {
  asm volatile("tcgen05.dealloc.cta_group::1.sync.aligned.b32 %0, %1;" ::"r"(taddr), "r"(ncols) : "memory");
}
__device__ __forceinline__ void tc_fence_before() {
  asm volatile("tcgen05.fence::before_thread_sync;" ::: "memory");
}
__device__ __forceinline__ void tc_fence_after() {
  asm volatile("tcgen05.fence::after_thread_sync;" ::: "memory");
}
__device__ __forceinline__ void umma_bf16_ss(uint32_t tmem_d, uint64_t adesc, uint64_t bdesc, uint32_t idesc,
                                             uint32_t accumulate) {
  asm volatile(
      "{\n\t"
      ".reg .pred p;\n\t"
      "setp.ne.b32 p, %4, 0;\n\t"
      "tcgen05.mma.cta_group::1.kind::f16 [%0], %1, %2, %3, p;\n\t"
      "}\n" ::"r"(tmem_d),
      "l"(adesc), "l"(bdesc), "r"(idesc), "r"(accumulate)
      : "memory");
}
__device__ __forceinline__ void umma_commit(uint64_t* bar) {
  asm volatile("tcgen05.commit.cta_group::1.mbarrier::arrive::one.shared::cluster.b64 [%0];" ::"r"(smem_u32(bar))
               : "memory");
}
constexpr uint32_t kPeerBitMask = 0xFEFFFFFFu;

__device__ __forceinline__ uint32_t cluster_ctarank() {
  uint32_t r;
  asm volatile("mov.u32 %0, %%cluster_ctarank;" : "=r"(r));
  return r;
}
__device__ __forceinline__ void cluster_sync_all() {
  asm volatile("barrier.cluster.arrive.release.aligned;\n\tbarrier.cluster.wait.acquire.aligned;" ::: "memory");
}
__device__ __forceinline__ void tma_load_2d_pair(void* smem_dst, const void* tmap, uint64_t* bar, int c0, int c1) {
  asm volatile(
      "cp.async.bulk.tensor.2d.cta_group::2.shared::cluster.global.mbarrier::complete_tx::bytes [%0], [%1, {%3, %4}], [%2];"
      ::"r"(smem_u32(smem_dst)), "l"(reinterpret_cast<uint64_t>(tmap)), "r"(smem_u32(bar) & kPeerBitMask), "r"(c0), "r"(c1)
      : "memory");
}
__device__ __forceinline__ void mbar_arrive_leader(uint64_t* bar) {
  asm volatile("mbarrier.arrive.release.cluster.shared::cluster.b64 _, [%0];" ::"r"(smem_u32(bar) & kPeerBitMask)
               : "memory");
}
__device__ __forceinline__ void tmem_alloc_pair(uint32_t* smem_dst, uint32_t ncols) {
  asm volatile("tcgen05.alloc.cta_group::2.sync.aligned.shared::cta.b32 [%0], %1;" ::"r"(smem_u32(smem_dst)),
               "r"(ncols)
               : "memory");
}
__device__ __forceinline__ void tmem_relinquish_pair() {
  asm volatile("tcgen05.relinquish_alloc_permit.cta_group::2.sync.aligned;" ::: "memory");
}
__device__ __forceinline__ void tmem_dealloc_pair(uint32_t taddr, uint32_t ncols) {
  asm volatile("tcgen05.dealloc.cta_group::2.sync.aligned.b32 %0, %1;" ::"r"(taddr), "r"(ncols) : "memory");
}
__device__ __forceinline__ void umma_bf16_ss_pair(uint32_t tmem_d, uint64_t adesc, uint64_t bdesc, uint32_t idesc,
                                                  uint32_t accumulate) {
  asm volatile(
      "{\n\t"
      ".reg .pred p;\n\t"
      "setp.ne.b32 p, %4, 0;\n\t"
      "tcgen05.mma.cta_group::2.kind::f16 [%0], %1, %2, %3, p;\n\t"
      "}\n" ::"r"(tmem_d),
      "l"(adesc), "l"(bdesc), "r"(idesc), "r"(accumulate)
      : "memory");
}
__device__ __forceinline__ void umma_commit_pair(uint64_t* bar) {
  asm volatile(
      "tcgen05.commit.cta_group::2.mbarrier::arrive::one.shared::cluster.multicast::cluster.b64 [%0], %1;"
      ::"r"(smem_u32(bar)), "h"((uint16_t)3)
      : "memory");
}

__device__ __forceinline__ void tmem_ld_32x32b_x16(uint32_t taddr, uint32_t (&r)[16]) {
  asm volatile(
      "tcgen05.ld.sync.aligned.32x32b.x16.b32 "
      "{%0, %1, %2, %3, %4, %5, %6, %7, %8, %9, %10, %11, %12, %13, %14, %15}, [%16];"
      : "=r"(r[0]), "=r"(r[1]), "=r"(r[2]), "=r"(r[3]), "=r"(r[4]), "=r"(r[5]), "=r"(r[6]), "=r"(r[7]),
        "=r"(r[8]), "=r"(r[9]), "=r"(r[10]), "=r"(r[11]), "=r"(r[12]), "=r"(r[13]), "=r"(r[14]), "=r"(r[15])
      : "r"(taddr));
}
__device__ __forceinline__ void tmem_ld_wait() { asm volatile("tcgen05.wait::ld.sync.aligned;" ::: "memory"); }

__device__ __forceinline__ uint64_t make_sw128_kmajor_desc(uint32_t smem_addr) {
  uint64_t d = 0;
  d |= (uint64_t)((smem_addr & 0x3FFFF) >> 4);
  d |= (uint64_t)1 << 16;
  d |= (uint64_t)(1024 >> 4) << 32;
  d |= (uint64_t)1 << 46;
  d |= (uint64_t)2 << 61;
  return d;
}

__device__ __forceinline__ uint64_t make_sw64_kmajor_desc(uint32_t smem_addr) {
  uint64_t d = 0;
  d |= (uint64_t)((smem_addr & 0x3FFFF) >> 4);
  d |= (uint64_t)1 << 16;
  d |= (uint64_t)(512 >> 4) << 32;
  d |= (uint64_t)1 << 46;
  d |= (uint64_t)4 << 61;
  return d;
}

}
```

modelcompression_b200/engine.py:

```python
import ctypes
import weakref

import torch
import torch.nn as nn

from . import _lib


def _round_up(x, m):
    return (x + m - 1) // m * m


def _pitch(n):
    ld = _round_up(n, 8)
    if n <= 16:
        return ld
    if n <= 32:
        return 32
    full = _round_up(n, 64)
    return full if full * 4 <= ld * 5 else ld


def _c_floats(t):
    vals = t.flatten().tolist()
    return (ctypes.c_float * len(vals))(*vals)


def _thin_host_weights(wd, sc, sh, ct, nt):
    n, c, k, _ = wd.shape
    wt = torch.zeros(k * k, ct, nt)
    wt[:, :c, :n] = wd.to(torch.bfloat16).float().permute(2, 3, 1, 0).reshape(k * k, c, n).cpu()
    sct = torch.zeros(nt)
    sht = torch.zeros(nt)
    sct[:n] = sc.float().cpu()
    sht[:n] = sh.float().cpu()
    return _c_floats(wt), _c_floats(sct), _c_floats(sht)


class _TensorRef(object):

    def __init__(self, buf_id, H, W, c_orig, colsrc, const, ch_off=0):
        self.buf_id = buf_id
        self.H, self.W = H, W
        self.c_orig = c_orig
        self.colsrc = colsrc
        self.const = const
        self.ch_off = ch_off

    @property
    def c_phys(self):
        return len(self.colsrc)


class _Buf(object):
    def __init__(self, H, W, ld, zero_init=False, fp32_nchw_channels=0):
        self.H, self.W, self.ld = H, W, ld
        self.zero_init = zero_init
        self.dead = False
        self.fp32_nchw_channels = fp32_nchw_channels


class CompiledDarknet(object):
    def __init__(self, model, shrink=True):
        self.lib = _lib.load()
        params = list(model.parameters())
        if not params:
            raise RuntimeError("Darknet has no parameters")
        self.device = params[0].device
        _lib.require_cuda(params[0], "Darknet.forward")
        with torch.cuda.device(self.device):
            if self.lib.mc_device_ok() != 1:
                raise RuntimeError("Darknet.forward: " + self.lib.mc_last_error_string().decode())
        self.shrink = bool(shrink)
        self.use_thin = int(getattr(model, 'b200_thin', 2))
        self.bufs = []
        self.ops = []
        self.block_out = {}
        self.flops_per_image = 0
        self._alloc = {}
        self._graphs = {}
        self._graph_seen = {}
        self.use_graph = True
        self.in_hw = None
        self._compile(model)

    def _new_buf(self, H, W, ld, **kw):
        self.bufs.append(_Buf(H, W, ld, **kw))
        return len(self.bufs) - 1

    def _compile(self, model):
        blocks = model.blocks
        H, W = model.height, model.width
        if H % 32 or W % 32:
            raise NotImplementedError("input size must be a multiple of 32 (cfg has %dx%d)" % (W, H))
        self.in_hw = (H, W)
        cat_of = {}
        ind = -2
        for block in blocks:
            ind += 1
            if block['type'] == 'route':
                layers = [int(i) if int(i) > 0 else int(i) + ind for i in block['layers'].split(',')]
                if len(layers) == 2:
                    cat_of[layers[0]] = (ind, 0)
                    cat_of[layers[1]] = (ind, 1)
                elif len(layers) != 1:
                    raise NotImplementedError("route with %d inputs" % len(layers))
        n_models = len(model.models)
        last_conv = max(i for i, b in enumerate(blocks[1:]) if b['type'] == 'convolutional')

        cur = None
        cur_hw = (H, W)
        cat_state = {}
        ind = -2
        skip_next_pool = False
        for bi, block in enumerate(blocks):
            ind += 1
            btype = block['type']
            if btype == 'net':
                in_ch = int(block['channels'])
                continue
            if btype == 'convolutional':
                seq = model.models[ind]
                conv = seq[0]
                bn = seq[1] if int(block['batch_normalize']) else None
                act = block['activation']
                if act not in ('leaky', 'linear'):
                    raise NotImplementedError("activation '%s'" % act)
                k = conv.kernel_size[0]
                if conv.kernel_size != (k, k) or k not in (1, 3) or conv.stride != (1, 1) or \
                        conv.padding != ((k - 1) // 2, (k - 1) // 2) or conv.groups != 1 or conv.dilation != (1, 1):
                    raise NotImplementedError("conv %s is outside the B200 path (need k in {1,3}, stride 1, 'same' "
                                              "padding)" % (conv,))
                is_head = (ind == last_conv)
                nxt = blocks[bi + 1] if bi + 1 < len(blocks) else None
                nxt_is_pool = nxt is not None and nxt['type'] == 'maxpool' and int(nxt['size']) == 2 and \
                    int(nxt['stride']) == 2
                nxt_is_reorg = nxt is not None and nxt['type'] == 'reorg' and int(nxt['stride']) == 2
                cur, fused = self._compile_conv(conv, bn, act == 'leaky', cur, cur_hw, in_ch, is_head, ind, cat_of,
                                                cat_state, nxt_is_pool, nxt_is_reorg)
                self.block_out[ind] = cur
                if fused == 'pool':
                    skip_next_pool = True
                    cur_hw = (cur.H, cur.W)
                elif fused == 'reorg':
                    skip_next_pool = True
                    cur_hw = (cur.H, cur.W)
            elif btype == 'maxpool':
                if skip_next_pool:
                    skip_next_pool = False
                    self.block_out[ind] = cur
                    continue
                if int(block['size']) != 2 or int(block['stride']) != 2:
                    raise NotImplementedError("maxpool size=%s stride=%s" % (block['size'], block['stride']))
                src = cur
                Ho, Wo = src.H // 2, src.W // 2
                ld = _pitch(src.c_phys)
                bid = self._new_buf(Ho, Wo, ld, zero_init=True)
                self.ops.append(dict(kind='pool', src=src, dst_buf=bid, C=src.c_phys, name='pool@%d' % ind))
                cur = _TensorRef(bid, Ho, Wo, src.c_orig, list(src.colsrc), src.const)
                cur_hw = (Ho, Wo)
                self.block_out[ind] = cur
            elif btype == 'reorg':
                if skip_next_pool:
                    skip_next_pool = False
                    self.block_out[ind] = cur
                    continue
                raise NotImplementedError("reorg that does not directly follow a convolution")
            elif btype == 'route':
                layers = [int(i) if int(i) > 0 else int(i) + ind for i in block['layers'].split(',')]
                if len(layers) == 1:
                    cur = self.block_out[layers[0]]
                else:
                    st = cat_state.get(ind)
                    if st is None or len(st['parts']) != 2:
                        raise NotImplementedError("concat inputs must both be produced by convolutions (cfg block %d)" % bi)
                    p0, p1 = st['parts'][0], st['parts'][1]
                    colsrc = list(p0.colsrc) + [-1] * (p1.ch_off - p0.c_phys)
                    have_ones = -2 in colsrc
                    for c in p1.colsrc:
                        if c >= 0:
                            colsrc.append(c + p0.c_orig)
                        elif c == -2 and not have_ones:
                            colsrc.append(-2)
                            have_ones = True
                        else:
                            colsrc.append(-1)
                    cur = _TensorRef(st['buf_id'], p0.H, p0.W, p0.c_orig + p1.c_orig, colsrc,
                                     torch.cat([p0.const, p1.const]))
                cur_hw = (cur.H, cur.W)
                self.block_out[ind] = cur
            elif btype == 'region':
                continue
            else:
                raise NotImplementedError("cfg block type '%s'" % btype)
        self.out_ref = cur
        del n_models
        if self.use_thin >= 2:
            routed = set()
            ind = -2
            for block in blocks:
                ind += 1
                if block['type'] == 'route':
                    routed.update(int(i) if int(i) > 0 else int(i) + ind for i in block['layers'].split(','))
            self._fuse_thin_pairs(routed)

    def _fuse_thin_pairs(self, routed):
        i = 0
        while i + 1 < len(self.ops):
            a, b = self.ops[i], self.ops[i + 1]
            i += 1
            if a['kind'] != 'thin' or a['pool'] or a['ksize'] != 3 or a['N2'] or a['ind'] in routed:
                continue
            if b['kind'] == 'conv':
                if b['ksize'] != 1 or not b.get('plain') or b['epi'] != _lib.MC_EPI_PNHWC or b['ch_off'] != 0:
                    continue
                b_ld = b['ldc']
            elif b['kind'] == 'thin':
                if b['ksize'] != 1 or b['N2']:
                    continue
                b_ld = b['ld']
            else:
                continue
            if b['src'].buf_id != a['dst_buf'] or b['src'].ch_off != 0 or b['Cin'] != a['N']:
                continue
            ct, nt, n2t = ctypes.c_int(), ctypes.c_int(), ctypes.c_int()
            if self.lib.mc_conv_thin_geometry(3, a['Cin'], a['N'], 0, b['N'], ctypes.byref(ct), ctypes.byref(nt),
                                              ctypes.byref(n2t)) != 1:
                continue
            ct, nt, n2t = ct.value, nt.value, n2t.value
            if self.bufs[a['src'].buf_id].ld < ct or b_ld < _round_up(n2t, 8):
                continue
            taps, ct0, nt0 = 9, a['hw_shape'][1], a['hw_shape'][2]
            w1 = torch.tensor(list(a['hw'])).view(taps, ct0, nt0)
            w1p = torch.zeros(taps, ct, nt)
            w1p[:, :min(ct, ct0), :min(nt, nt0)] = w1[:, :min(ct, ct0), :min(nt, nt0)]
            sc1 = torch.zeros(nt)
            sh1 = torch.zeros(nt)
            sc1[:a['N']] = torch.tensor(list(a['hsc']))[:a['N']]
            sh1[:a['N']] = torch.tensor(list(a['hsh']))[:a['N']]
            w2 = torch.zeros(nt, n2t)
            sc2 = torch.zeros(n2t)
            sh2 = torch.zeros(n2t)
            if b['kind'] == 'conv':
                w2[:a['N'], :b['N']] = b['wpack'][:b['N'], :a['N']].float().t().cpu()
                sc2[:b['N']] = b['scale'][:b['N']].cpu()
                sh2[:b['N']] = b['shift'][:b['N']].cpu()
            else:
                wb = torch.tensor(list(b['hw'])).view(b['hw_shape'])[0]
                w2[:a['N'], :b['N']] = wb[:a['N'], :b['N']]
                sc2[:b['N']] = torch.tensor(list(b['hsc']))[:b['N']]
                sh2[:b['N']] = torch.tensor(list(b['hsh']))[:b['N']]
            fused = dict(a)
            fused.update(hw=_c_floats(w1p), hsc=_c_floats(sc1), hsh=_c_floats(sh1), hw_shape=(taps, ct, nt),
                         hw2=_c_floats(w2), hsc2=_c_floats(sc2), hsh2=_c_floats(sh2), N2=b['N'], leaky2=b['leaky'],
                         dst_buf=b['dst_buf'], ld=b_ld, name='thin@%d+%d' % (a['ind'], b['ind']),
                         flops_per_image=a['flops_per_image'] + b['flops_per_image'], fused_n1=a['N'])
            self.bufs[a['dst_buf']].dead = True
            self.block_out.pop(a['ind'], None)
            self.ops[i - 1:i + 1] = [fused]

    def _compile_conv(self, conv, bn, leaky, src, src_hw, in_ch, is_head, ind, cat_of, cat_state, nxt_is_pool,
                      nxt_is_reorg):
        dev = self.device
        H, W = src_hw
        w = conv.weight.data.float()
        if getattr(conv, 'mask_flag', False):
            w = w * conv.mask.to(dev)
        O, Corig = w.shape[0], w.shape[1]
        k = w.shape[2]
        taps = k * k
        if bn is not None:
            scale = bn.weight.data.float() / torch.sqrt(bn.running_var.float() + bn.eps)
            shift = bn.bias.data.float() - bn.running_mean.float() * scale
        else:
            scale = torch.ones(O, device=dev)
            shift = conv.bias.data.float() if conv.bias is not None else torch.zeros(O, device=dev)
        if src is None:
            in_colsrc, in_const, c_in_orig = list(range(in_ch)), torch.zeros(in_ch), in_ch
        else:
            in_colsrc, in_const, c_in_orig = src.colsrc, src.const, src.c_orig
        if c_in_orig != Corig:
            raise RuntimeError("conv at block %d expects %d input channels, graph provides %d" % (ind, Corig, c_in_orig))
        if self.shrink and not is_head:
            alive = (w.abs().amax(dim=(1, 2, 3)) > 0)
            if not bool(alive.any()):
                alive[0] = True
            keep = torch.nonzero(alive).flatten()
        else:
            keep = torch.arange(O, device=dev)
        n_keep = int(keep.numel())
        const_out = torch.zeros(O)
        need_ones_out = False
        if n_keep < O:
            dead = torch.ones(O, dtype=torch.bool, device=dev)
            dead[keep] = False
            cval = shift.clone()
            if leaky:
                cval = torch.where(cval > 0, cval, 0.1 * cval)
            cval = torch.where(dead, cval, torch.zeros_like(cval))
            const_out = cval.cpu()
            need_ones_out = bool((const_out != 0).any())
        out_colsrc = [int(i) for i in keep.tolist()] + ([-2] if need_ones_out else [])
        n_phys = len(out_colsrc)
        in_has_const = bool((in_const != 0).any())
        w_aug = w
        if in_has_const:
            if -2 not in in_colsrc:
                raise RuntimeError("internal: constant input channels without a ones channel")
            w1 = torch.einsum('ocrs,c->ors', w, in_const.to(dev))
            w_aug = torch.cat([w, w1[:, None]], dim=1)
        cidx = [(c if c >= 0 else (Corig if (c == -2 and in_has_const) else -1)) for c in in_colsrc]
        c_phys_in = len(cidx)
        op_flops = 2 * H * W * n_keep * sum(1 for c in in_colsrc if c >= 0) * taps
        self.flops_per_image += op_flops
        o_list = [int(i) for i in keep.tolist()] + ([-1] if need_ones_out else [])
        sc = torch.cat([scale[keep], torch.zeros(1, device=dev)]) if need_ones_out else scale[keep]
        sh = torch.cat([shift[keep], torch.ones(1, device=dev)]) if need_ones_out else shift[keep]
        Npad = _round_up(n_phys, 16)
        scale_p = torch.zeros(Npad, device=dev)
        shift_p = torch.zeros(Npad, device=dev)
        scale_p[:n_phys] = sc
        shift_p[:n_phys] = sh

        plain_dst = (ind not in cat_of) and not (nxt_is_reorg and (ind + 1) in cat_of) and not is_head
        first = src is None
        pool = 1 if nxt_is_pool else 0

        def gathered_fp32():
            rows = torch.tensor([o if o >= 0 else 0 for o in o_list], dtype=torch.long, device=dev)
            cols = torch.tensor([c if c >= 0 else 0 for c in cidx], dtype=torch.long, device=dev)
            wd = w_aug[rows][:, cols].clone()
            wd[torch.tensor([o < 0 for o in o_list], device=dev)] = 0
            wd[:, torch.tensor([c < 0 for c in cidx], device=dev)] = 0
            return wd

        if self.use_thin and plain_dst and not first and src.ch_off == 0 and (not pool or (H % 2 == 0 and W % 2 == 0)):
            ct, nt = ctypes.c_int(), ctypes.c_int()
            src_ld = self.bufs[src.buf_id].ld
            if self.lib.mc_conv_thin_geometry(k, c_phys_in, n_phys, pool, 0, ctypes.byref(ct), ctypes.byref(nt), None) == 1 \
                    and src_ld >= ct.value and _pitch(n_phys) >= _round_up(nt.value, 8):
                ct, nt = ct.value, nt.value
                Ho, Wo = (H // 2, W // 2) if pool else (H, W)
                ld = _pitch(n_phys)
                bid = self._new_buf(Ho, Wo, ld, zero_init=True)
                hw, hsc, hsh = _thin_host_weights(gathered_fp32(), sc, sh, ct, nt)
                self.ops.append(dict(kind='thin', src=src, hw=hw, hsc=hsc, hsh=hsh, hw_shape=(taps, ct, nt), dst_buf=bid, N=n_phys, Cin=c_phys_in,
                                     H=H, W=W, ld=ld, pool=pool, ksize=k, leaky=int(leaky), N2=0, leaky2=0, ind=ind,
                                     name='thin%s@%d' % ('+pool' if pool else '', ind), flops_per_image=op_flops))
                return _TensorRef(bid, Ho, Wo, O, out_colsrc, const_out), ('pool' if pool else None)

        win_kind = None
        if plain_dst and k == 3 and (not pool or (H % 2 == 0 and W % 2 == 0)):
            if first and pool and c_phys_in <= 3 and n_phys <= 8:
                win_kind = 1
            elif not first and not pool and src.ch_off == 0 and self.bufs[src.buf_id].ld == 8 and c_phys_in <= 8:
                win_kind = 0
        if win_kind is not None and self.lib.mc_conv_window_supported(c_phys_in, win_kind, n_phys, pool) == 1:
            npos, nb, kcols = ctypes.c_int(), ctypes.c_int(), ctypes.c_int()
            _lib.check(self.lib.mc_conv_window_geometry(c_phys_in, win_kind, n_phys, pool, ctypes.byref(npos),
                                                        ctypes.byref(nb), ctypes.byref(kcols)), "mc_conv_window_geometry")
            npos, nb, kcols = npos.value, nb.value, kcols.value
            wd = gathered_fp32().permute(0, 2, 3, 1)
            if win_kind == 0:
                wk = torch.zeros(nb, 10, 8, device=dev)
                wk[:n_phys, :9, :c_phys_in] = wd.reshape(n_phys, 9, c_phys_in)
            else:
                wk = torch.zeros(nb, 4, 4, 4, device=dev)
                for dy in range(2):
                    for dx in range(2):
                        r0 = (dy * 2 + dx) * npos
                        wk[r0:r0 + n_phys, dy:dy + 3, dx:dx + 3, :c_phys_in] = wd
            wk = wk.reshape(nb, kcols).to(torch.bfloat16).contiguous()
            Ho, Wo = (H // 2, W // 2) if pool else (H, W)
            ld = _pitch(n_phys)
            bid = self._new_buf(Ho, Wo, ld, zero_init=True)
            n_sc = max(_round_up(npos, 16), 16)
            sc2 = torch.zeros(n_sc, device=dev)
            sh2 = torch.zeros(n_sc, device=dev)
            sc2[:n_phys] = sc
            sh2[:n_phys] = sh
            self.ops.append(dict(kind='window', src=src, w=wk, scale=sc2, shift=sh2, dst_buf=bid, N=n_phys, Cin=c_phys_in,
                                 H=H, W=W, ld=ld, pool=pool, leaky=int(leaky), in_kind=win_kind,
                                 name='window%s@%d' % ('+pool' if pool else '', ind), flops_per_image=op_flops))
            return _TensorRef(bid, Ho, Wo, O, out_colsrc, const_out), ('pool' if pool else None)

        src_ok = first or (src.ch_off == 0 and self.bufs[src.buf_id].ld == (8 if c_phys_in <= 8 else 16))
        if plain_dst and k == 3 and src_ok and (H % 2 == 0 and W % 2 == 0 or not pool) and \
                self.lib.mc_conv_im2col_supported(c_phys_in, 1 if first else 0, n_phys, pool) == 1:
            cl, npos, nb, kpad = (ctypes.c_int(), ctypes.c_int(), ctypes.c_int(), ctypes.c_int())
            _lib.check(self.lib.mc_conv_im2col_geometry(c_phys_in, 1 if first else 0, n_phys, pool, ctypes.byref(cl),
                                                        ctypes.byref(npos), ctypes.byref(nb), ctypes.byref(kpad)),
                       "mc_conv_im2col_geometry")
            cl, npos, nb, kpad = cl.value, npos.value, nb.value, kpad.value
            wd = gathered_fp32().permute(0, 2, 3, 1)
            nb_pad = _round_up(nb, 16)
            if pool:
                wexp = torch.zeros(nb_pad, 4, 4, cl, device=dev)
                for dy in range(2):
                    for dx in range(2):
                        r0 = (dy * 2 + dx) * npos
                        wexp[r0:r0 + n_phys, dy:dy + 3, dx:dx + 3, :c_phys_in] = wd
                wexp = wexp.reshape(nb_pad, 16 * cl)
            else:
                wexp = torch.zeros(nb_pad, 3, 3, cl, device=dev)
                wexp[:n_phys, :, :, :c_phys_in] = wd
                wexp = wexp.reshape(nb_pad, 9 * cl)
            wfull = torch.zeros(nb_pad, kpad, device=dev)
            wfull[:, :wexp.shape[1]] = wexp
            Ho, Wo = (H // 2, W // 2) if pool else (H, W)
            ld = _pitch(n_phys)
            bid = self._new_buf(Ho, Wo, ld, zero_init=True)
            n_sc = max(_round_up(npos, 16), 16)
            sc2 = torch.zeros(n_sc, device=dev)
            sh2 = torch.zeros(n_sc, device=dev)
            sc2[:n_phys] = sc
            sh2[:n_phys] = sh
            self.ops.append(dict(kind='im2col', src=src, w=wfull.to(torch.bfloat16).contiguous(), scale=sc2, shift=sh2,
                                 dst_buf=bid, N=n_phys, Cin=c_phys_in, H=H, W=W, ld=ld, pool=pool, leaky=int(leaky),
                                 name='im2col%s@%d' % ('+pool' if pool else '', ind), flops_per_image=op_flops))
            return _TensorRef(bid, Ho, Wo, O, out_colsrc, const_out), ('pool' if pool else None)
        if first and plain_dst and self.lib.mc_conv_direct_supported(c_phys_in, n_phys, k) == 1:
            wd = gathered_fp32().reshape(n_phys, c_phys_in, taps)
            Ho, Wo = (H // 2, W // 2) if pool else (H, W)
            ld = _pitch(n_phys)
            bid = self._new_buf(Ho, Wo, ld, zero_init=True)
            self.ops.append(dict(kind='direct', src=src, w=wd.contiguous(), scale=scale_p, shift=shift_p, dst_buf=bid,
                                 N=n_phys, Cin=c_phys_in, H=H, W=W, ld=ld, pool=pool, ksize=k, leaky=int(leaky),
                                 name='direct%s@%d' % ('+pool' if pool else '', ind), flops_per_image=op_flops))
            return _TensorRef(bid, Ho, Wo, O, out_colsrc, const_out), ('pool' if pool else None)
        if src is None:
            bid_in = self._new_buf(H, W, 8)
            self.ops.append(dict(kind='pack_input', dst_buf=bid_in, C=in_ch, H=H, W=W, name='pack_input'))
            src = _TensorRef(bid_in, H, W, in_ch, list(range(in_ch)), torch.zeros(in_ch))

        kblk = 32 if c_phys_in <= 32 else 64
        Kc = _round_up(c_phys_in, kblk)
        wpack = torch.empty(Npad, taps * Kc, dtype=torch.bfloat16, device=dev)
        oidx_t = torch.tensor(o_list, dtype=torch.int32, device=dev)
        cidx_t = torch.tensor(cidx, dtype=torch.int32, device=dev)
        w_src = w_aug.contiguous()
        with torch.cuda.device(dev):
            _lib.check(self.lib.mc_pack_conv_weights(w_src.data_ptr(), None, w_src.shape[0], w_src.shape[1], k,
                                                     oidx_t.data_ptr(), n_phys, cidx_t.data_ptr(), c_phys_in,
                                                     wpack.data_ptr(), Npad, Kc, _lib.stream_ptr()),
                       "mc_pack_conv_weights")
        op = dict(kind='conv', src=src, wpack=wpack, scale=scale_p, shift=shift_p, N=n_phys, Npad=Npad, ksize=k,
                  leaky=int(leaky), Cin=c_phys_in, name='conv@%d' % ind, H=H, W=W, flops_per_image=op_flops, block_k=kblk,
                  ind=ind, plain=bool(plain_dst))
        fused = None
        if is_head:
            bid = self._new_buf(H, W, 0, fp32_nchw_channels=n_phys)
            op.update(epi=_lib.MC_EPI_NCHW_F32, dst_buf=bid, ldc=0, ch_off=0)
            out = _TensorRef(bid, H, W, O, out_colsrc, const_out)
        elif nxt_is_reorg and (ind + 1) in cat_of:
            route, slot = cat_of[ind + 1]
            Ho, Wo = H // 2, W // 2
            st = cat_state.setdefault(route, dict(buf_id=None, parts={}, pending=[]))
            colsrc4 = []
            for q in range(4):
                for c in out_colsrc:
                    colsrc4.append(c + q * O if c >= 0 else (c if (c == -2 and q == 0) else -1))
            out = _TensorRef(None, Ho, Wo, 4 * O, colsrc4, const_out.repeat(4))
            op.update(epi=_lib.MC_EPI_REORG2)
            st['parts'][slot] = out
            st['pending'].append((op, slot))
            fused = 'reorg'
        elif ind in cat_of:
            route, slot = cat_of[ind]
            st = cat_state.setdefault(route, dict(buf_id=None, parts={}, pending=[]))
            out = _TensorRef(None, H, W, O, out_colsrc, const_out)
            op.update(epi=_lib.MC_EPI_PNHWC)
            st['parts'][slot] = out
            st['pending'].append((op, slot))
        else:
            ld = _pitch(n_phys)
            bid = self._new_buf(H, W, ld)
            op.update(epi=_lib.MC_EPI_PNHWC, dst_buf=bid, ldc=ld, ch_off=0)
            out = _TensorRef(bid, H, W, O, out_colsrc, const_out)
        self.ops.append(op)
        for route, st in cat_state.items():
            if st['buf_id'] is None and len(st['parts']) == 2:
                p0, p1 = st['parts'][0], st['parts'][1]
                if (p0.H, p0.W) != (p1.H, p1.W):
                    raise NotImplementedError("concat of different resolutions")
                off1 = _round_up(p0.c_phys, 8)
                ld = _pitch(off1 + p1.c_phys)
                st['buf_id'] = self._new_buf(p0.H, p0.W, ld, zero_init=True)
                for pop, slot in st['pending']:
                    pop.update(dst_buf=st['buf_id'], ldc=ld, ch_off=0 if slot == 0 else off1)
                p0.buf_id = p1.buf_id = st['buf_id']
                p1.ch_off = off1
        return out, fused

    def _buffers(self, B, H, W):
        key = (B, H, W)
        got = self._alloc.get(key)
        if got is not None:
            return got
        if (H, W) != self.in_hw:
            raise NotImplementedError("this plan was compiled for %dx%d inputs (cfg width/height); got %dx%d" %
                                      (self.in_hw[1], self.in_hw[0], W, H))
        tensors = []
        for b in self.bufs:
            if b.fp32_nchw_channels or b.dead:
                tensors.append(None)
            else:
                rows = B * (b.H + 1) * (b.W + 1)
                tensors.append(torch.zeros(rows, b.ld, dtype=torch.bfloat16, device=self.device))
        self._alloc[key] = tensors
        return tensors

    def run(self, x, events=None, detect=None, repeat=1):
        if events is not None or not self.use_graph or not x.is_cuda or x.dtype not in (torch.float32, torch.uint8) or \
                not x.is_contiguous() or x.requires_grad:
            return self._run_eager(x, events, detect, repeat)
        base = (tuple(x.shape), torch.cuda.current_stream(x.device).cuda_stream, x.dtype, detect)
        key = base + (x.data_ptr(),)
        entry = self._graphs.get(key)
        if entry is not None and entry[2] is not x:
            entry = None
            key = None
        if entry is None:
            seen = 0
            if key is not None:
                ref = self._graph_seen.get(key)
                seen = (ref[1] if ref is not None and ref[0]() is x else 0) + 1
                if len(self._graph_seen) > 4096:
                    self._graph_seen.clear()
                self._graph_seen[key] = (weakref.ref(x), seen)
            if seen >= 3 and sum(1 for k in self._graphs if k[:4] == base and k[4] != 'static') < 8:
                entry = self._capture(key, x, detect)
            else:
                skey = base + ('static',)
                entry = self._graphs.get(skey)
                if entry is None:
                    cnt = self._graph_seen.get(skey, 0) + 1
                    self._graph_seen[skey] = cnt
                    if cnt < 2:
                        return self._run_eager(x, None, detect)
                    entry = self._capture(skey, torch.empty_like(x), detect)
                entry[2].copy_(x)
        entry[0].replay()
        if detect is None:
            return entry[1].clone()
        return tuple(None if t is None else t.clone() for t in entry[1])

    def _capture(self, key, x, detect):
        if len(self._graphs) >= 24:
            self._graphs.pop(next(iter(self._graphs)))
        with torch.cuda.device(self.device):
            torch.cuda.synchronize()
            graph = torch.cuda.CUDAGraph()
            with torch.cuda.graph(graph):
                out = self._run_eager(x, None, detect)
        entry = (graph, out, x)
        self._graphs[key] = entry
        return entry

    def _conv_workspace(self, nbytes):
        ws = getattr(self, '_ws', None)
        if ws is None or ws.numel() < nbytes:
            if ws is not None and self._graphs:
                raise RuntimeError("internal: conv workspace grew after a CUDA graph captured its address")
            ws = self._ws = torch.zeros(nbytes, dtype=torch.uint8, device=self.device)
        return ws

    def supports_detect(self, model):
        if not self.ops or self.ops[-1].get('epi') != _lib.MC_EPI_NCHW_F32:
            return False
        n = self.ops[-1]['N']
        return n == model.num_anchors * (5 + model.num_classes) and self.ops[-1]['Npad'] <= 256 and \
            len(model.anchors) == 2 * model.num_anchors and model.num_anchors <= 16

    def _run_eager(self, x, events=None, detect=None, repeat=1):
        if x.dim() != 4:
            raise ValueError("expected [B,3,H,W] input")
        _lib.require_cuda(x, "Darknet.forward")
        if x.device != self.device:
            raise RuntimeError("input on %s, model on %s" % (x.device, self.device))
        x = x.detach()
        u8 = x.dtype == torch.uint8 and self.ops and self.ops[0]['kind'] in ('im2col', 'window') and \
            self.ops[0]['src'] is None
        if x.dtype == torch.uint8 and not u8:
            x = x.float().div_(255.0)
        elif x.dtype not in (torch.float32, torch.uint8):
            x = x.float()
        x = x.contiguous()
        B, _, H, W = x.shape
        lib = self.lib
        with torch.cuda.device(self.device):
            bufs = list(self._buffers(B, H, W))
            stream = _lib.stream_ptr()
            out = None
            self._prev_op = None
            for op in (o for o in self.ops for _ in range(repeat if events is not None else 1)):
                kind = op['kind']
                first_rep = op is not getattr(self, '_prev_op', None)
                self._prev_op = op
                if events is not None and first_rep:
                    ev0 = torch.cuda.Event(enable_timing=True)
                    ev0.record()
                    reps_left = repeat
                if kind == 'im2col':
                    s = op['src']
                    if s is None:
                        in_ptr, nchw, cin_ld = x.data_ptr(), (2 if u8 else 1), op['Cin']
                    else:
                        in_ptr, nchw, cin_ld = bufs[s.buf_id].data_ptr(), 0, self.bufs[s.buf_id].ld
                    _lib.check(lib.mc_conv_im2col_fwd(in_ptr, nchw, op['w'].data_ptr(), op['scale'].data_ptr(),
                                                      op['shift'].data_ptr(), bufs[op['dst_buf']].data_ptr(), B,
                                                      op['H'], op['W'], op['Cin'], cin_ld, op['N'], op['ld'],
                                                      op['leaky'], op['pool'], stream), op['name'])
                elif kind == 'window':
                    s = op['src']
                    if s is None:
                        in_ptr, in_kind = x.data_ptr(), (2 if u8 else 1)
                    else:
                        in_ptr, in_kind = bufs[s.buf_id].data_ptr(), 0
                    _lib.check(lib.mc_conv_window_fwd(in_ptr, in_kind, op['w'].data_ptr(), op['scale'].data_ptr(),
                                                      op['shift'].data_ptr(), bufs[op['dst_buf']].data_ptr(), B, op['H'],
                                                      op['W'], op['Cin'], op['N'], op['ld'], op['leaky'], op['pool'],
                                                      stream), op['name'])
                elif kind == 'thin':
                    s = op['src']
                    _lib.check(lib.mc_conv_thin_fwd(bufs[s.buf_id].data_ptr(), op['hw'], op['hsc'], op['hsh'],
                                                    op.get('hw2'), op.get('hsc2'), op.get('hsh2'),
                                                    bufs[op['dst_buf']].data_ptr(), B, op['H'], op['W'], op['Cin'],
                                                    self.bufs[s.buf_id].ld, op['N'], op['ld'], op['ksize'], op['leaky'],
                                                    op['pool'], op['N2'], op['leaky2'], stream), op['name'])
                elif kind == 'direct':
                    s = op['src']
                    if s is None:
                        in_ptr, nchw, cin_ld = x.data_ptr(), 1, op['Cin']
                    else:
                        in_ptr, nchw, cin_ld = bufs[s.buf_id].data_ptr() + 2 * s.ch_off, 0, self.bufs[s.buf_id].ld
                    _lib.check(lib.mc_conv_direct_fwd(in_ptr, nchw, op['w'].data_ptr(), op['scale'].data_ptr(),
                                                      op['shift'].data_ptr(), bufs[op['dst_buf']].data_ptr(), B,
                                                      op['H'], op['W'], op['Cin'], cin_ld, op['N'], op['ld'],
                                                      op['ksize'], op['leaky'], op['pool'], stream), op['name'])
                elif kind == 'pack_input':
                    _lib.check(lib.mc_pack_pnhwc(x.data_ptr(), bufs[op['dst_buf']].data_ptr(), B, op['H'], op['W'],
                                                 op['C'], 8, stream), op['name'])
                elif kind == 'pool':
                    s = op['src']
                    sb = self.bufs[s.buf_id]
                    if s.ch_off != 0:
                        raise NotImplementedError("maxpool on a channel slice")
                    _lib.check(lib.mc_maxpool2x2(bufs[s.buf_id].data_ptr(), bufs[op['dst_buf']].data_ptr(), B, s.H, s.W,
                                                 op['C'], sb.ld, self.bufs[op['dst_buf']].ld, stream), op['name'])
                elif kind == 'conv':
                    s = op['src']
                    d = _lib.mc_conv_desc()
                    sb = self.bufs[s.buf_id]
                    d.d_in = bufs[s.buf_id].data_ptr() + 2 * s.ch_off
                    d.d_wpack = op['wpack'].data_ptr()
                    d.d_scale = op['scale'].data_ptr()
                    d.d_shift = op['shift'].data_ptr()
                    epi = op['epi']
                    dec = None
                    if epi == _lib.MC_EPI_NCHW_F32 and detect is not None:
                        thr, only_obj, want_cls = detect
                        A, nc = self.detect_geom
                        P = op['H'] * op['W'] * A
                        boxes = torch.empty(B, P, 8, dtype=torch.float32, device=self.device)
                        cls = torch.empty(B, P, nc, dtype=torch.float32, device=self.device) if want_cls else None
                        dec = _lib.mc_decode_params()
                        dec.d_boxes = boxes.data_ptr()
                        dec.d_cls = cls.data_ptr() if cls is not None else None
                        dec.d_head = None
                        dec.A, dec.nc, dec.conf_thresh, dec.only_objectness = A, nc, float(thr), 1 if only_obj else 0
                        for i, a in enumerate(self.detect_anchors):
                            dec.anchors[i] = float(a)
                        epi = _lib.MC_EPI_DECODE
                        out = (boxes, cls)
                        d.decode = ctypes.pointer(dec)
                        d.d_out = None
                    elif epi == _lib.MC_EPI_NCHW_F32:
                        out = torch.empty(B, op['N'], op['H'], op['W'], dtype=torch.float32, device=self.device)
                        bufs[op['dst_buf']] = out
                        d.d_out = out.data_ptr()
                    else:
                        d.d_out = bufs[op['dst_buf']].data_ptr()
                    d.B, d.H, d.W = B, op['H'], op['W']
                    d.Cin, d.Cin_ld = op['Cin'], sb.ld
                    d.in_cols = sb.ld - s.ch_off
                    d.N, d.Npad = op['N'], op['Npad']
                    d.ksize, d.leaky, d.epi_mode = op['ksize'], op['leaky'], epi
                    d.ldc, d.ch_off = op['ldc'], op['ch_off']
                    d.block_n = op.get('block_n', 0)
                    d.stages = op.get('stages', 0)
                    d.block_k = op.get('block_k', 0)
                    if op.get('ws_bytes') is None:
                        op['ws_bytes'] = int(lib.mc_workspace_bytes_conv_fwd(ctypes.byref(d)))
                    if op['ws_bytes']:
                        ws = self._conv_workspace(op['ws_bytes'])
                        d.d_ws, d.ws_bytes = ws.data_ptr(), ws.numel()
                    _lib.check(lib.mc_conv_fwd(ctypes.byref(d), stream), op['name'])
                else:
                    raise RuntimeError("unknown op " + kind)
                if events is not None:
                    reps_left -= 1
                    if reps_left == 0:
                        ev1 = torch.cuda.Event(enable_timing=True)
                        ev1.record()
                        events.append((op, ev0, ev1))
            self._prev_op = None
            self._last_bufs = bufs
        return out

    @property
    def num_launches(self):
        return len(self.ops)

    def block_activation(self, ind):
        ref = self.block_out[ind]
        bufs = self._last_bufs
        t = bufs[ref.buf_id]
        if t.dtype == torch.float32:
            return t
        B = t.shape[0] // ((ref.H + 1) * (ref.W + 1))
        phys = torch.empty(B, ref.c_phys, ref.H, ref.W, dtype=torch.float32, device=self.device)
        with torch.cuda.device(self.device):
            _lib.check(self.lib.mc_unpack_pnhwc(t.data_ptr(), phys.data_ptr(), B, ref.H, ref.W, ref.c_phys,
                                                self.bufs[ref.buf_id].ld, ref.ch_off, _lib.stream_ptr()),
                       "mc_unpack_pnhwc")
        full = ref.const.to(self.device).view(1, -1, 1, 1).expand(B, ref.c_orig, ref.H, ref.W).clone()
        for p, c in enumerate(ref.colsrc):
            if c >= 0:
                full[:, c] = phys[:, p]
        return full


def _plan_key(model):
    watch = getattr(model, '_b200_watch', None)
    if watch is None:
        tensors = list(model.parameters()) + list(model.buffers())
        convs = [m for m in model.modules() if getattr(m, 'name', None) == 'MaskedConv2d']
        watch = model._b200_watch = (tensors, convs, len(tensors))
    tensors, convs, _ = watch
    return (bool(getattr(model, 'b200_shrink', True)), tuple(t._version for t in tensors),
            tuple(c.weight.data_ptr() for c in convs),
            tuple((getattr(c, '_mask_epoch', 0), c.mask.data_ptr() if c.mask_flag else 0) for c in convs))


def compile_darknet(model, force=False):
    key = _plan_key(model)
    if force or model._b200_plan is None or model._b200_plan_key != key:
        model._b200_plan = CompiledDarknet(model, shrink=key[0])
        model._b200_plan_key = key
    return model._b200_plan


def darknet_detect_forward(model, x, conf_thresh, only_objectness, want_cls):
    if model.training:
        return None
    plan = compile_darknet(model)
    if not plan.supports_detect(model):
        return None
    plan.detect_geom = (int(model.num_anchors), int(model.num_classes))
    plan.detect_anchors = [float(a) for a in model.anchors]
    return plan.run(x, detect=(float(conf_thresh), 1 if only_objectness else 0, bool(want_cls)))


def darknet_forward(model, x):
    if model.training:
        from .engine_train import darknet_train_forward
        return darknet_train_forward(model, x)
    return compile_darknet(model).run(x)


def single_conv_forward(conv, x):
    lib = _lib.load()
    _lib.require_cuda(x, "MaskedConv2d.forward")
    k = conv.kernel_size[0]
    if conv.kernel_size != (k, k) or k not in (1, 3) or conv.stride != (1, 1) or \
            conv.padding != ((k - 1) // 2, (k - 1) // 2) or conv.groups != 1 or conv.dilation != (1, 1):
        raise NotImplementedError("MaskedConv2d on the B200 path needs k in {1,3}, stride 1, 'same' padding")
    dev = x.device
    x = x.detach().float().contiguous()
    B, C, H, W = x.shape
    w = conv.weight.data.float().contiguous()
    mask = conv.mask.to(dev).contiguous() if getattr(conv, 'mask_flag', False) else None
    O = w.shape[0]
    kblk = 32 if C <= 32 else 64
    ld_in, Kc, Npad, ld_out = _round_up(C, 8), _round_up(C, kblk), _round_up(O, 16), _round_up(O, 8)
    xin = torch.empty(B * (H + 1) * (W + 1), ld_in, dtype=torch.bfloat16, device=dev)
    wpack = torch.empty(Npad, k * k * Kc, dtype=torch.bfloat16, device=dev)
    scale = torch.zeros(Npad, device=dev)
    shift = torch.zeros(Npad, device=dev)
    scale[:O] = 1
    if conv.bias is not None:
        shift[:O] = conv.bias.data.float()
    yb = torch.empty(B * (H + 1) * (W + 1), ld_out, dtype=torch.bfloat16, device=dev)
    y = torch.empty(B, O, H, W, dtype=torch.float32, device=dev)
    with torch.cuda.device(dev):
        s = _lib.stream_ptr()
        _lib.check(lib.mc_pack_pnhwc(x.data_ptr(), xin.data_ptr(), B, H, W, C, ld_in, s), "mc_pack_pnhwc")
        _lib.check(lib.mc_pack_conv_weights(w.data_ptr(), None if mask is None else mask.data_ptr(), O, C, k, None, O,
                                            None, C, wpack.data_ptr(), Npad, Kc, s), "mc_pack_conv_weights")
        d = _lib.mc_conv_desc()
        d.d_in, d.d_wpack, d.d_scale, d.d_shift, d.d_out = (xin.data_ptr(), wpack.data_ptr(), scale.data_ptr(),
                                                            shift.data_ptr(), yb.data_ptr())
        d.B, d.H, d.W, d.Cin, d.Cin_ld, d.N, d.Npad = B, H, W, C, ld_in, O, Npad
        d.ksize, d.leaky, d.epi_mode, d.ldc, d.ch_off, d.block_n, d.stages = k, 0, _lib.MC_EPI_PNHWC, ld_out, 0, 0, 0
        d.block_k = kblk
        need = int(lib.mc_workspace_bytes_conv_fwd(ctypes.byref(d)))
        if need and not getattr(conv, 'b200_no_workspace', False):
            ws = torch.zeros(need, dtype=torch.uint8, device=dev)
            d.d_ws, d.ws_bytes = ws.data_ptr(), need
        _lib.check(lib.mc_conv_fwd(ctypes.byref(d), s), "mc_conv_fwd")
        _lib.check(lib.mc_unpack_pnhwc(yb.data_ptr(), y.data_ptr(), B, H, W, O, ld_out, 0, s), "mc_unpack_pnhwc")
    return y
```

Before: 82090.

## Chain consecutive 3x3 pair-cluster convs into one persistent kernel with row-counter dependencies

Adds a chained variant of the tcgen05 pair-cluster conv kernel that runs up to four consecutive 3x3 PNHWC convolutions in a single persistent launch. Work tiles are handed out through a global ticket counter and a cluster-shared ring. Each tile of a later layer spin-waits on per-row-block completion counters released by the previous layer's epilogue. This removes launch gaps and tail idle time between layers and lets layers overlap. In exchange it adds global atomics, polling with a timeout, proxy fences, and scheduling complexity on the Python side.

New measurement: 85730, median of 6. 4.4% higher.

```diff
diff --git a/include/mcb200.h b/include/mcb200.h
--- a/include/mcb200.h
+++ b/include/mcb200.h
@@ -122,6 +122,9 @@
 int mc_conv_fwd(const mc_conv_desc* desc, void* stream);
 size_t mc_workspace_bytes_conv_fwd(const mc_conv_desc* desc);
 
+int mc_conv_chain_fwd(const mc_conv_desc* descs, int n, void* stream);
+size_t mc_workspace_bytes_conv_chain(const mc_conv_desc* descs, int n);
+
 int mc_conv_last_plan(int info[8]);
 
 int mc_conv_direct_supported(int Cin, int N, int ksize);
diff --git a/modelcompression_b200/_lib.py b/modelcompression_b200/_lib.py
--- a/modelcompression_b200/_lib.py
+++ b/modelcompression_b200/_lib.py
@@ -77,6 +77,8 @@
     "mc_bbox_ious": (c_int, [c_void_p, c_void_p, c_int64, c_int, c_void_p, c_void_p]),
     "mc_reorg_nchw": (c_int, [c_void_p, c_void_p, c_int, c_int, c_int, c_int, c_int, c_void_p]),
     "mc_conv_fwd": (c_int, [POINTER(mc_conv_desc), c_void_p]),
+    "mc_conv_chain_fwd": (c_int, [POINTER(mc_conv_desc), c_int, c_void_p]),
+    "mc_workspace_bytes_conv_chain": (c_size_t, [POINTER(mc_conv_desc), c_int]),
     "mc_workspace_bytes_conv_fwd": (c_size_t, [POINTER(mc_conv_desc)]),
     "mc_conv_last_plan": (c_int, [POINTER(c_int)]),
     "mc_conv_direct_supported": (c_int, [c_int, c_int, c_int]),
diff --git a/modelcompression_b200/csrc/conv_tcgen05.cu b/modelcompression_b200/csrc/conv_tcgen05.cu
--- a/modelcompression_b200/csrc/conv_tcgen05.cu
+++ b/modelcompression_b200/csrc/conv_tcgen05.cu
@@ -1,6 +1,7 @@
 #include <cuda.h>
 #include <stdio.h>
 #include <stdlib.h>
+#include <string.h>
 #include "common.cuh"
 #include "ptx_sm100.cuh"
 #include "tmap.cuh"
@@ -684,6 +685,7 @@
 }
 
 struct PairWork {
+  int layer;
   int unit;
   int g0, g1;
   int kind;
@@ -717,6 +719,7 @@
     }
   }
   __device__ __forceinline__ bool next(PairWork& w) {
+    w.layer = 0;
     if (next_full < sk_first) {
       w.unit = next_full; w.g0 = 0; w.g1 = -1; w.kind = 0; w.aux = 0;
       next_full += step;
@@ -742,40 +745,136 @@
   }
 };
 
+constexpr int MAX_CHAIN = 4;
+constexpr int WORK_SLOTS = 4;
+constexpr unsigned long long CHAIN_POLL_NS = 1000000000ull;
+enum { CHAIN_TICKET = 0, CHAIN_DONE = 1, CHAIN_STATUS = 2, CHAIN_COUNTERS = 4 };
+
+struct PairLayer {
+  CUtensorMap tmap_b, tmap_abox, tmap_out;
+  ConvKParams p;
+  int unit_end;
+  int cnt_off;
+};
+struct PairParams {
+  PairLayer layer[MAX_CHAIN];
+  int n_layers;
+  unsigned int* chain_ws;
+};
+
+struct PairRing {
+  uint64_t* full;
+  uint64_t* empty;
+  int* val;
+  int slot;
+  uint32_t phase;
+};
+
+__device__ __forceinline__ void chain_decode(const PairParams& P, int t, PairWork& w) {
+  int l = 0;
+  while (l + 1 < P.n_layers && t >= P.layer[l].unit_end) ++l;
+  w.layer = l;
+  w.unit = t - (l > 0 ? P.layer[l - 1].unit_end : 0);
+  w.g0 = 0; w.g1 = -1; w.kind = 0; w.aux = 0;
+}
+
+__device__ __forceinline__ bool ring_take(const PairParams& P, PairRing& r, PairWork& w, bool whole_warp) {
+  ptx::mbar_wait_cluster(&r.full[r.slot], r.phase);
+  const int t = *reinterpret_cast<volatile int*>(&r.val[r.slot]);
+  if (whole_warp) __syncwarp();
+  if ((threadIdx.x & 31) == 0) ptx::mbar_arrive_leader(&r.empty[r.slot]);
+  if (++r.slot == WORK_SLOTS) { r.slot = 0; r.phase ^= 1u; }
+  if (t < 0) return false;
+  chain_decode(P, t, w);
+  return true;
+}
+
+__device__ __noinline__ void chain_wait_inputs(const PairParams& P, const PairWork& w) {
+  const PairLayer& prev = P.layer[w.layer - 1];
+  const int mp = w.unit / P.layer[w.layer].p.n_tiles;
+  int r0 = 256 * mp - prev.p.Wp - 1, r1 = 256 * mp + 264 + prev.p.Wp;
+  if (r0 < 0) r0 = 0;
+  if (r1 > prev.p.M_rows) r1 = prev.p.M_rows;
+  const unsigned int need = 8u * (unsigned int)prev.p.n_tiles;
+  const unsigned int* cnt = P.chain_ws + CHAIN_COUNTERS + prev.cnt_off;
+  const unsigned long long t0 = ptx::globaltimer();
+  for (int j = r0 / 256; j <= (r1 - 1) / 256; ++j) {
+    while (ptx::ld_acquire_gpu(cnt + j) < need) {
+      if (ptx::globaltimer() - t0 > CHAIN_POLL_NS) {
+        atomicExch(P.chain_ws + CHAIN_STATUS, 1u);
+        return;
+      }
+    }
+  }
+}
+
+__device__ __forceinline__ bool ring_claim(const PairParams& P, PairRing& r, PairWork& w) {
+  ptx::mbar_wait_cluster(&r.empty[r.slot], r.phase ^ 1u);
+  int t = (int)atomicAdd(P.chain_ws + CHAIN_TICKET, 1u);
+  if (t >= P.layer[P.n_layers - 1].unit_end) {
+    t = -1;
+  } else {
+    chain_decode(P, t, w);
+    if (w.layer > 0) chain_wait_inputs(P, w);
+    ptx::fence_proxy_async_global();
+  }
+  for (uint32_t rk = 0; rk < 2; ++rk) {
+    ptx::st_cluster_u32(ptx::mapa_shared(&r.val[r.slot], rk), (uint32_t)t);
+    ptx::mbar_arrive_cluster(ptx::mapa_shared(&r.full[r.slot], rk));
+  }
+  if (++r.slot == WORK_SLOTS) { r.slot = 0; r.phase ^= 1u; }
+  return t >= 0;
+}
+
+__device__ __forceinline__ void chain_arrive(const PairParams& P, const PairWork& w, int lane) {
+  __threadfence();
+  __syncwarp();
+  if (lane == 0) {
+    ptx::bulk_wait_group_all();
+    ptx::fence_proxy_async_global();
+    const PairLayer& L = P.layer[w.layer];
+    ptx::red_release_gpu_add(P.chain_ws + CHAIN_COUNTERS + L.cnt_off + w.unit / L.p.n_tiles, 1u);
+  }
+}
+
 template <int MODE, bool LEAKY>
-__device__ __forceinline__ void epilogue_loop_pair(const ConvKParams& p, uint32_t tmem_base, uint64_t* tmem_full_bar,
+__device__ __forceinline__ void epilogue_loop_pair(const PairParams& P, uint32_t tmem_base, uint64_t* tmem_full_bar,
                                                    uint64_t* tmem_empty_bar, float* s_ss, int cluster_id, int num_clusters,
-                                                   int pair_rank, uint8_t* s_out, const CUtensorMap* tm_out) {
+                                                   int pair_rank, uint8_t* s_out, PairRing ring) {
   const int warp_idx = threadIdx.x >> 5;
   const int lane = threadIdx.x & 31;
   const int et = threadIdx.x - 64;
   const int quarter = warp_idx & 3;
-  const bool vec_ok = ((p.ldc | p.ch_off) & 7) == 0 && (MODE != MC_EPI_REORG2 || (p.N & 7) == 0);
+  const ConvKParams& p0 = P.layer[0].p;
+  const bool chain = P.n_layers > 1;
   int as = 0;
   uint32_t aphase = 0;
   int slab_buf = 0;
   float* stat_acc = nullptr;
   int stat_n0 = -1;
-  if (MODE == MC_EPI_PNHWC && p.tma_bufs > 0 && p.stat_sum != nullptr) {
-    stat_acc = reinterpret_cast<float*>(s_out + (size_t)4 * p.tma_bufs * 4096) + quarter * 512;
+  if (MODE == MC_EPI_PNHWC && p0.tma_bufs > 0 && p0.stat_sum != nullptr) {
+    stat_acc = reinterpret_cast<float*>(s_out + (size_t)4 * p0.tma_bufs * 4096) + quarter * 512;
     for (int c = lane; c < 512; c += 32) stat_acc[c] = 0.f;
     __syncwarp();
   }
-  const bool one_n_tile = p.n_tiles == 1;
+  const bool one_n_tile = !chain && p0.n_tiles == 1;
   if (one_n_tile) {
-    for (int i = et; i < p.block_n; i += 128) {
-      const bool ok = i < p.Npad;
-      s_ss[i] = ok ? __ldg(p.scale + i) : 0.f;
-      s_ss[256 + i] = ok ? __ldg(p.shift + i) : 0.f;
+    for (int i = et; i < p0.block_n; i += 128) {
+      const bool ok = i < p0.Npad;
+      s_ss[i] = ok ? __ldg(p0.scale + i) : 0.f;
+      s_ss[256 + i] = ok ? __ldg(p0.shift + i) : 0.f;
     }
     asm volatile("bar.sync 1, 128;" ::: "memory");
   }
   PairWorkIter it;
-  it.init(p, cluster_id, num_clusters);
+  it.init(p0, cluster_id, num_clusters);
   PairWork w;
   int ti = -1;
-  while (it.next(w)) {
+  while (chain ? ring_take(P, ring, w, true) : it.next(w)) {
     ++ti;
+    const ConvKParams& p = P.layer[w.layer].p;
+    const CUtensorMap* tm_out = &P.layer[w.layer].tmap_out;
+    const bool vec_ok = ((p.ldc | p.ch_off) & 7) == 0 && (MODE != MC_EPI_REORG2 || (p.N & 7) == 0);
     const int tile = w.unit;
     const int n0 = (tile % p.n_tiles) * p.block_n;
     const int m0 = (2 * (tile / p.n_tiles) + pair_rank) * BLOCK_M;
@@ -881,6 +980,7 @@
                                            }
                                          }
                                        }, stat_acc);
+        if (chain) chain_arrive(P, w, lane);
         if (et == 0 && ti < 8) conv_stamp(p, 13 + 2 * ti);
         if (++as == ACC_STAGES) { as = 0; aphase ^= 1u; }
         continue;
@@ -927,23 +1027,24 @@
     if (et == 0 && ti < 8) conv_stamp(p, 13 + 2 * ti);
     if (++as == ACC_STAGES) { as = 0; aphase ^= 1u; }
   }
-  if (stat_acc != nullptr && stat_n0 >= 0) flush_stats(p, stat_acc, stat_n0, lane);
-  if (MODE == MC_EPI_PNHWC && p.tma_bufs > 0 && lane == 0) ptx::bulk_wait_group_read<0>();
+  if (stat_acc != nullptr && stat_n0 >= 0) flush_stats(p0, stat_acc, stat_n0, lane);
+  if (MODE == MC_EPI_PNHWC && p0.tma_bufs > 0 && lane == 0) ptx::bulk_wait_group_read<0>();
 }
 
 __global__ void __cluster_dims__(2, 1, 1) __launch_bounds__(NUM_THREADS, 1)
-conv_gemm_tcgen05_pair_kernel(const __grid_constant__ CUtensorMap tmap_b, const __grid_constant__ CUtensorMap tmap_abox,
-                              const __grid_constant__ CUtensorMap tmap_out, const ConvKParams p) {
+conv_gemm_tcgen05_pair_kernel(const __grid_constant__ PairParams P) {
   extern __shared__ __align__(1024) uint8_t smem_raw[];
-  const uint32_t b_half_bytes = (uint32_t)(p.block_n / 2 * 128);
+  const ConvKParams& p0 = P.layer[0].p;
+  const bool chain = P.n_layers > 1;
+  const uint32_t b_half_bytes = (uint32_t)(p0.block_n / 2 * 128);
   uint8_t* smem = smem_raw;
   {
     uint32_t a = ptx::smem_u32(smem);
     smem += (1024u - (a & 1023u)) & 1023u;
   }
   uint8_t* tiles = smem;
-  uint8_t* b_ring = tiles + (size_t)p.a_stages * A_BOX_STRIDE;
-  uint8_t* aux = b_ring + (size_t)p.stages * b_half_bytes;
+  uint8_t* b_ring = tiles + (size_t)p0.a_stages * A_BOX_STRIDE;
+  uint8_t* aux = b_ring + (size_t)p0.stages * b_half_bytes;
   uint64_t* full_bar = reinterpret_cast<uint64_t*>(aux);
   uint64_t* empty_bar = full_bar + MAX_STAGES;
   uint64_t* tmem_full_bar = empty_bar + MAX_STAGES;
@@ -951,6 +1052,12 @@
   uint64_t* afull_bar = tmem_empty_bar + ACC_STAGES;
   uint64_t* aempty_bar = afull_bar + MAX_A_STAGES;
   uint32_t* tmem_ptr_smem = reinterpret_cast<uint32_t*>(aempty_bar + MAX_A_STAGES);
+  PairRing ring;
+  ring.full = reinterpret_cast<uint64_t*>(aux + 256);
+  ring.empty = ring.full + WORK_SLOTS;
+  ring.val = reinterpret_cast<int*>(ring.empty + WORK_SLOTS);
+  ring.slot = 0;
+  ring.phase = 0;
   float* s_ss = reinterpret_cast<float*>(aux + 512);
   uint8_t* s_out = aux + 5120;
 
@@ -958,13 +1065,15 @@
   const int lane = threadIdx.x & 31;
   const int rank = (int)ptx::cluster_ctarank();
   const int cluster_id = blockIdx.x >> 1, num_clusters = gridDim.x >> 1;
-  if (threadIdx.x == 0) conv_stamp(p, 0);
+  if (threadIdx.x == 0) conv_stamp(p0, 0);
 
   if (warp_idx == 0 && lane == 0) {
-    ptx::prefetch_tensormap(&tmap_b);
-    ptx::prefetch_tensormap(&tmap_abox);
-    if (p.tma_bufs > 0) ptx::prefetch_tensormap(&tmap_out);
-    for (int s = 0; s < p.stages; ++s) {
+    for (int l = 0; l < P.n_layers; ++l) {
+      ptx::prefetch_tensormap(&P.layer[l].tmap_b);
+      ptx::prefetch_tensormap(&P.layer[l].tmap_abox);
+      if (p0.tma_bufs > 0) ptx::prefetch_tensormap(&P.layer[l].tmap_out);
+    }
+    for (int s = 0; s < p0.stages; ++s) {
       ptx::mbar_init(&full_bar[s], 1);
       ptx::mbar_init(&empty_bar[s], 1);
     }
@@ -976,26 +1085,33 @@
       ptx::mbar_init(&afull_bar[a], 1);
       ptx::mbar_init(&aempty_bar[a], 1);
     }
+    for (int s = 0; s < WORK_SLOTS; ++s) {
+      ptx::mbar_init(&ring.full[s], 1);
+      ptx::mbar_init(&ring.empty[s], 10);
+    }
     ptx::fence_barrier_init();
   }
   if (warp_idx == 1) {
-    ptx::tmem_alloc_pair(tmem_ptr_smem, (uint32_t)p.tmem_cols);
+    ptx::tmem_alloc_pair(tmem_ptr_smem, (uint32_t)p0.tmem_cols);
     ptx::tmem_relinquish_pair();
   }
   ptx::tc_fence_before();
   ptx::cluster_sync_all();
   ptx::tc_fence_after();
   const uint32_t tmem_base = *tmem_ptr_smem;
-  if (threadIdx.x == 0) conv_stamp(p, 1);
+  if (threadIdx.x == 0) conv_stamp(p0, 1);
 
   if (warp_idx == 0) {
     if (lane == 0) {
       int s = 0, sa = 0;
       uint32_t phase = 0, pha = 0;
       PairWorkIter it;
-      it.init(p, cluster_id, num_clusters);
+      it.init(p0, cluster_id, num_clusters);
       PairWork w;
-      while (it.next(w)) {
+      while (!chain ? it.next(w) : (rank == 0 ? ring_claim(P, ring, w) : ring_take(P, ring, w, false))) {
+        const PairLayer& L = P.layer[w.layer];
+        const ConvKParams& p = L.p;
+        if (chain && rank != 0) ptx::fence_proxy_async_global();
         const int unit = w.unit;
         const int n0 = (unit % p.n_tiles) * p.block_n + rank * (p.block_n / 2);
         const int m0 = (2 * (unit / p.n_tiles) + rank) * BLOCK_M;
@@ -1004,36 +1120,39 @@
           const int dy = g / p.kb_per_tap, cb = g - dy * p.kb_per_tap;
           ptx::mbar_wait(&aempty_bar[sa], pha ^ 1u);
           if (rank == 0) ptx::mbar_arrive_expect_tx(&afull_bar[sa], 2 * A_BOX_BYTES);
-          ptx::tma_load_2d_pair(tiles + (size_t)sa * A_BOX_STRIDE, &tmap_abox, &afull_bar[sa], cb * 64,
+          ptx::tma_load_2d_pair(tiles + (size_t)sa * A_BOX_STRIDE, &L.tmap_abox, &afull_bar[sa], cb * 64,
                                 m0 + (dy - 1) * p.Wp - 1);
           if (++sa == p.a_stages) { sa = 0; pha ^= 1u; }
           for (int dx = 0; dx < 3; ++dx) {
             const int kb = (dy * 3 + dx) * p.kb_per_tap + cb;
             ptx::mbar_wait(&empty_bar[s], phase ^ 1u);
             if (rank == 0) ptx::mbar_arrive_expect_tx(&full_bar[s], 2 * b_half_bytes);
-            ptx::tma_load_2d_pair(b_ring + (size_t)s * b_half_bytes, &tmap_b, &full_bar[s], kb * 64, n0);
+            ptx::tma_load_2d_pair(b_ring + (size_t)s * b_half_bytes, &L.tmap_b, &full_bar[s], kb * 64, n0);
             if (++s == p.stages) { s = 0; phase ^= 1u; }
           }
         }
       }
-      conv_stamp(p, 3);
+      conv_stamp(p0, 3);
     }
   } else if (warp_idx == 1) {
     if (rank == 0) {
       int s = 0, sa = 0, as = 0;
       uint32_t phase = 0, pha = 0, aphase = 0;
       PairWorkIter it;
-      it.init(p, cluster_id, num_clusters);
+      it.init(p0, cluster_id, num_clusters);
       PairWork w;
       int ti = -1;
-      while (it.next(w)) {
+      while (chain ? ring_take(P, ring, w, true) : it.next(w)) {
         ++ti;
+        const ConvKParams& p = P.layer[w.layer].p;
         ptx::mbar_wait(&tmem_empty_bar[as], aphase ^ 1u);
         ptx::tc_fence_after();
         const uint32_t tmem_acc = tmem_base + (uint32_t)(as * p.acc_stride);
-        const int gb = w.g0, ge = w.g1 < 0 ? 3 * p.kb_per_tap : w.g1;
+        const int kbt = p.kb_per_tap, lks = p.last_ksteps;
+        const uint32_t idesc = p.idesc;
+        const int gb = w.g0, ge = w.g1 < 0 ? 3 * kbt : w.g1;
         for (int g = gb; g < ge; ++g) {
-          const int nk = ((g % p.kb_per_tap) == p.kb_per_tap - 1) ? p.last_ksteps : 4;
+          const int nk = ((g % kbt) == kbt - 1) ? lks : 4;
           ptx::mbar_wait(&afull_bar[sa], pha);
           if (ti == 0 && g == gb && lane == 0) conv_stamp(p, 4);
           const uint32_t a_addr = ptx::smem_u32(tiles + (size_t)sa * A_BOX_STRIDE);
@@ -1046,37 +1165,49 @@
 #pragma unroll
               for (int k = 0; k < 4; ++k)
                 if (k < nk)
-                  ptx::umma_bf16_ss_pair(tmem_acc, adesc + (uint64_t)(2 * k), bdesc + (uint64_t)(2 * k), p.idesc,
+                  ptx::umma_bf16_ss_pair(tmem_acc, adesc + (uint64_t)(2 * k), bdesc + (uint64_t)(2 * k), idesc,
                                          (g > gb || dx > 0 || k > 0) ? 1u : 0u);
               ptx::umma_commit_pair(&empty_bar[s]);
               if (dx == 2) ptx::umma_commit_pair(&aempty_bar[sa]);
               if (dx == 2 && g == ge - 1) ptx::umma_commit_pair(&tmem_full_bar[as]);
             }
             __syncwarp();
-            if (++s == p.stages) { s = 0; phase ^= 1u; }
+            if (++s == p0.stages) { s = 0; phase ^= 1u; }
           }
-          if (++sa == p.a_stages) { sa = 0; pha ^= 1u; }
+          if (++sa == p0.a_stages) { sa = 0; pha ^= 1u; }
         }
         if (lane == 0 && ti < 6) conv_stamp(p, 5 + ti);
         if (++as == ACC_STAGES) { as = 0; aphase ^= 1u; }
       }
     }
   } else {
-    if (p.epi_mode == MC_EPI_PNHWC) {
-      if (p.leaky) epilogue_loop_pair<MC_EPI_PNHWC, true>(p, tmem_base, tmem_full_bar, tmem_empty_bar, s_ss, cluster_id, num_clusters, rank, s_out, &tmap_out);
-      else epilogue_loop_pair<MC_EPI_PNHWC, false>(p, tmem_base, tmem_full_bar, tmem_empty_bar, s_ss, cluster_id, num_clusters, rank, s_out, &tmap_out);
-    } else if (p.epi_mode == MC_EPI_REORG2) {
-      if (p.leaky) epilogue_loop_pair<MC_EPI_REORG2, true>(p, tmem_base, tmem_full_bar, tmem_empty_bar, s_ss, cluster_id, num_clusters, rank, s_out, &tmap_out);
-      else epilogue_loop_pair<MC_EPI_REORG2, false>(p, tmem_base, tmem_full_bar, tmem_empty_bar, s_ss, cluster_id, num_clusters, rank, s_out, &tmap_out);
+    if (p0.epi_mode == MC_EPI_PNHWC) {
+      if (p0.leaky) epilogue_loop_pair<MC_EPI_PNHWC, true>(P, tmem_base, tmem_full_bar, tmem_empty_bar, s_ss, cluster_id, num_clusters, rank, s_out, ring);
+      else epilogue_loop_pair<MC_EPI_PNHWC, false>(P, tmem_base, tmem_full_bar, tmem_empty_bar, s_ss, cluster_id, num_clusters, rank, s_out, ring);
+    } else if (p0.epi_mode == MC_EPI_REORG2) {
+      if (p0.leaky) epilogue_loop_pair<MC_EPI_REORG2, true>(P, tmem_base, tmem_full_bar, tmem_empty_bar, s_ss, cluster_id, num_clusters, rank, s_out, ring);
+      else epilogue_loop_pair<MC_EPI_REORG2, false>(P, tmem_base, tmem_full_bar, tmem_empty_bar, s_ss, cluster_id, num_clusters, rank, s_out, ring);
     } else {
-      if (p.leaky) epilogue_loop_pair<MC_EPI_NCHW_F32, true>(p, tmem_base, tmem_full_bar, tmem_empty_bar, s_ss, cluster_id, num_clusters, rank, s_out, &tmap_out);
-      else epilogue_loop_pair<MC_EPI_NCHW_F32, false>(p, tmem_base, tmem_full_bar, tmem_empty_bar, s_ss, cluster_id, num_clusters, rank, s_out, &tmap_out);
+      if (p0.leaky) epilogue_loop_pair<MC_EPI_NCHW_F32, true>(P, tmem_base, tmem_full_bar, tmem_empty_bar, s_ss, cluster_id, num_clusters, rank, s_out, ring);
+      else epilogue_loop_pair<MC_EPI_NCHW_F32, false>(P, tmem_base, tmem_full_bar, tmem_empty_bar, s_ss, cluster_id, num_clusters, rank, s_out, ring);
     }
   }
 
   ptx::tc_fence_before();
   ptx::cluster_sync_all();
-  if (warp_idx == 1) ptx::tmem_dealloc_pair(tmem_base, (uint32_t)p.tmem_cols);
+  if (warp_idx == 1) ptx::tmem_dealloc_pair(tmem_base, (uint32_t)p0.tmem_cols);
+  if (threadIdx.x == 0) conv_stamp(p0, 30);
+  if (chain && rank == 0 && threadIdx.x == 0) {
+    __threadfence();
+    if (atomicAdd(P.chain_ws + CHAIN_DONE, 1u) == (unsigned int)num_clusters - 1u) {
+      __threadfence();
+      const PairLayer& last = P.layer[P.n_layers - 1];
+      const int n_cnt = last.cnt_off + (last.p.m_tiles + 1) / 2;
+      for (int i = 0; i < n_cnt; ++i) P.chain_ws[CHAIN_COUNTERS + i] = 0u;
+      P.chain_ws[CHAIN_TICKET] = 0u;
+      P.chain_ws[CHAIN_DONE] = 0u;
+    }
+  }
 }
 
 int pick_block_n(int Npad, int m_tiles, int num_kb, int num_sms, bool share_dx) {
@@ -1122,8 +1253,41 @@
   return (size_t)2048 + (size_t)clusters * 3 * 256 * 256 * sizeof(float);
 }
 
-extern "C" int mc_conv_fwd(const mc_conv_desc* d, void* stream_) {
-  cudaStream_t stream = reinterpret_cast<cudaStream_t>(stream_);
+static int pair_max_clusters(int* out) {
+  static int max_clusters = -1;
+  if (max_clusters < 0) {
+    MC_CUDA(cudaFuncSetAttribute(conv_gemm_tcgen05_pair_kernel, cudaFuncAttributeMaxDynamicSharedMemorySize, 227 * 1024));
+    cudaLaunchConfig_t cfg = {};
+    cfg.gridDim = dim3(2 * (mc_num_sms() / 2));
+    cfg.blockDim = dim3(NUM_THREADS);
+    cfg.dynamicSmemBytes = 222 * 1024;
+    cudaLaunchAttribute at[1];
+    at[0].id = cudaLaunchAttributeClusterDimension;
+    at[0].val.clusterDim.x = 2; at[0].val.clusterDim.y = 1; at[0].val.clusterDim.z = 1;
+    cfg.attrs = at;
+    cfg.numAttrs = 1;
+    int n = 0;
+    if (cudaOccupancyMaxActiveClusters(&n, conv_gemm_tcgen05_pair_kernel, &cfg) != cudaSuccess || n < 1) {
+      cudaGetLastError();
+      n = mc_num_sms() / 2;
+    }
+    max_clusters = n;
+  }
+  *out = max_clusters;
+  return 0;
+}
+
+struct ConvPlan {
+  bool use_pair;
+  int ctas;
+  int grid;
+  int units;
+  size_t smem_bytes;
+  CUtensorMap tm_a, tm_b, tm_abox, tm_out;
+  ConvKParams p;
+};
+
+static int conv_plan(const mc_conv_desc* d, ConvPlan* L) {
   MC_CHECK_ARG(d != nullptr, "mc_conv_fwd: null descriptor");
   MC_CHECK_ARG(d->d_in && d->d_wpack && d->d_scale && d->d_shift && (d->d_out || d->epi_mode == MC_EPI_DECODE),
                "mc_conv_fwd: null pointer");
@@ -1352,25 +1516,9 @@
     p.acc_stride = ((block_n + 31) / 32) * 32;
     p.tmem_cols = 32;
     while (p.tmem_cols < ACC_STAGES * p.acc_stride) p.tmem_cols <<= 1;
-    static int max_clusters = -1;
-    if (max_clusters < 0) {
-      MC_CUDA(cudaFuncSetAttribute(conv_gemm_tcgen05_pair_kernel, cudaFuncAttributeMaxDynamicSharedMemorySize, 227 * 1024));
-      cudaLaunchConfig_t cfg = {};
-      cfg.gridDim = dim3(2 * (mc_num_sms() / 2));
-      cfg.blockDim = dim3(NUM_THREADS);
-      cfg.dynamicSmemBytes = 222 * 1024;
-      cudaLaunchAttribute at[1];
-      at[0].id = cudaLaunchAttributeClusterDimension;
-      at[0].val.clusterDim.x = 2; at[0].val.clusterDim.y = 1; at[0].val.clusterDim.z = 1;
-      cfg.attrs = at;
-      cfg.numAttrs = 1;
-      int n = 0;
-      if (cudaOccupancyMaxActiveClusters(&n, conv_gemm_tcgen05_pair_kernel, &cfg) != cudaSuccess || n < 1) {
-        cudaGetLastError();
-        n = mc_num_sms() / 2;
-      }
-      max_clusters = n;
-    }
+    int max_clusters = 0;
+    int rc2 = pair_max_clusters(&max_clusters);
+    if (rc2) return rc2;
     const int m_pairs = (m_tiles + 1) / 2;
     const long long units = (long long)m_pairs * n_tiles;
     const int clusters = (int)(units < max_clusters ? units : max_clusters);
@@ -1394,9 +1542,47 @@
         p.sk_part = reinterpret_cast<float*>(reinterpret_cast<uint8_t*>(d->d_ws) + 2048);
       }
     }
-    g_last_plan[0] = 1; g_last_plan[1] = block_n; g_last_plan[2] = 1; g_last_plan[3] = p.sk_units; g_last_plan[4] = 1;
-    g_last_plan[5] = stages; g_last_plan[6] = 2 * clusters; g_last_plan[7] = BLOCK_K;
-    conv_gemm_tcgen05_pair_kernel<<<2 * clusters, NUM_THREADS, smem_bytes, stream>>>(tm_b, tm_abox, tm_out, p);
+    L->use_pair = true;
+    L->ctas = 1;
+    L->grid = 2 * clusters;
+    L->units = (int)units;
+  } else {
+    const long long max_ctas = (long long)mc_num_sms() * ctas;
+    L->use_pair = false;
+    L->ctas = ctas;
+    L->grid = (int)(total_tiles < max_ctas ? total_tiles : max_ctas);
+    L->units = 0;
+  }
+  L->smem_bytes = smem_bytes;
+  L->tm_a = tm_a; L->tm_b = tm_b; L->tm_abox = tm_abox; L->tm_out = tm_out;
+  L->p = p;
+  return 0;
+}
+
+static void pair_layer(const ConvPlan& L, PairLayer* e) {
+  e->tmap_b = L.tm_b;
+  e->tmap_abox = L.tm_abox;
+  e->tmap_out = L.tm_out;
+  e->p = L.p;
+  e->unit_end = L.units;
+  e->cnt_off = 0;
+}
+
+extern "C" int mc_conv_fwd(const mc_conv_desc* d, void* stream_) {
+  cudaStream_t stream = reinterpret_cast<cudaStream_t>(stream_);
+  ConvPlan L;
+  int rc = conv_plan(d, &L);
+  if (rc) return rc;
+  const ConvKParams& p = L.p;
+  if (L.use_pair) {
+    g_last_plan[0] = 1; g_last_plan[1] = p.block_n; g_last_plan[2] = 1; g_last_plan[3] = p.sk_units; g_last_plan[4] = 1;
+    g_last_plan[5] = p.stages; g_last_plan[6] = L.grid; g_last_plan[7] = p.block_k;
+    PairParams P;
+    memset(&P, 0, sizeof(P));
+    pair_layer(L, &P.layer[0]);
+    P.n_layers = 1;
+    P.chain_ws = nullptr;
+    conv_gemm_tcgen05_pair_kernel<<<L.grid, NUM_THREADS, L.smem_bytes, stream>>>(P);
     MC_LAUNCH_CHECK("conv_gemm_tcgen05_pair_kernel");
     return 0;
   }
@@ -1408,16 +1594,108 @@
     MC_CUDA(cudaFuncSetAttribute(conv_gemm_tcgen05_kernel<3>, cudaFuncAttributeMaxDynamicSharedMemorySize, 112 * 1024));
     attr_set = true;
   }
-  const long long max_ctas = (long long)mc_num_sms() * ctas;
-  const int grid = (int)(total_tiles < max_ctas ? total_tiles : max_ctas);
-  g_last_plan[0] = 0; g_last_plan[1] = block_n; g_last_plan[2] = ctas; g_last_plan[3] = 0;
-  g_last_plan[4] = share_dx; g_last_plan[5] = stages; g_last_plan[6] = grid; g_last_plan[7] = BLOCK_K;
-  if (ctas >= 3)
-    conv_gemm_tcgen05_kernel<3><<<grid, NUM_THREADS, smem_bytes, stream>>>(tm_a, tm_b, tm_abox, tm_out, p);
-  else if (ctas == 2)
-    conv_gemm_tcgen05_kernel<2><<<grid, NUM_THREADS, smem_bytes, stream>>>(tm_a, tm_b, tm_abox, tm_out, p);
+  g_last_plan[0] = 0; g_last_plan[1] = p.block_n; g_last_plan[2] = L.ctas; g_last_plan[3] = 0;
+  g_last_plan[4] = p.share_dx; g_last_plan[5] = p.stages; g_last_plan[6] = L.grid; g_last_plan[7] = p.block_k;
+  if (L.ctas >= 3)
+    conv_gemm_tcgen05_kernel<3><<<L.grid, NUM_THREADS, L.smem_bytes, stream>>>(L.tm_a, L.tm_b, L.tm_abox, L.tm_out, p);
+  else if (L.ctas == 2)
+    conv_gemm_tcgen05_kernel<2><<<L.grid, NUM_THREADS, L.smem_bytes, stream>>>(L.tm_a, L.tm_b, L.tm_abox, L.tm_out, p);
   else
-    conv_gemm_tcgen05_kernel<1><<<grid, NUM_THREADS, smem_bytes, stream>>>(tm_a, tm_b, tm_abox, tm_out, p);
+    conv_gemm_tcgen05_kernel<1><<<L.grid, NUM_THREADS, L.smem_bytes, stream>>>(L.tm_a, L.tm_b, L.tm_abox, L.tm_out, p);
   MC_LAUNCH_CHECK("conv_gemm_tcgen05_kernel");
   return 0;
 }
+
+static size_t chain_ws_words(const mc_conv_desc* descs, int n) {
+  size_t words = CHAIN_COUNTERS;
+  for (int i = 0; i < n; ++i) {
+    const long long rows = (long long)descs[i].B * (descs[i].H + 1) * (descs[i].W + 1);
+    words += (size_t)(((rows + BLOCK_M - 1) / BLOCK_M + 1) / 2);
+  }
+  return words;
+}
+
+static bool ranges_overlap(const void* a, size_t na, const void* b, size_t nb) {
+  const uintptr_t a0 = (uintptr_t)a, b0 = (uintptr_t)b;
+  return a0 < b0 + nb && b0 < a0 + na;
+}
+
+static int chain_plan(const mc_conv_desc* descs, int n, ConvPlan* L) {
+  MC_CHECK_ARG(descs != nullptr, "mc_conv_chain_fwd: null descriptors");
+  MC_CHECK_ARG(n >= 2 && n <= MAX_CHAIN, "mc_conv_chain_fwd: %d members (2..%d)", n, MAX_CHAIN);
+  const mc_conv_desc& d0 = descs[0];
+  for (int i = 0; i < n; ++i) {
+    const mc_conv_desc& di = descs[i];
+    MC_CHECK_ARG(di.ksize == 3 && di.epi_mode == MC_EPI_PNHWC,
+                 "mc_conv_chain_fwd: member %d must be a 3x3 layer with the PNHWC epilogue", i);
+    MC_CHECK_ARG(di.d_stat_sum == nullptr && di.d_stat_sumsq == nullptr,
+                 "mc_conv_chain_fwd: member %d asks for batch statistics", i);
+    MC_CHECK_ARG(di.B == d0.B && di.H == d0.H && di.W == d0.W, "mc_conv_chain_fwd: member %d has another B, H or W", i);
+    mc_conv_desc one = di;
+    one.d_ws = nullptr;
+    one.ws_bytes = 0;
+    const int rc = conv_plan(&one, &L[i]);
+    if (rc) return rc;
+    MC_CHECK_ARG(L[i].use_pair, "mc_conv_chain_fwd: member %d does not take the CTA-pair kernel", i);
+    MC_CHECK_ARG(L[i].p.tma_bufs > 0, "mc_conv_chain_fwd: member %d does not take the TMA-store epilogue", i);
+    MC_CHECK_ARG(L[i].p.block_n == L[0].p.block_n && L[i].p.stages == L[0].p.stages && L[i].p.leaky == L[0].p.leaky &&
+                     L[i].smem_bytes == L[0].smem_bytes,
+                 "mc_conv_chain_fwd: member %d has another tile width, ring or activation", i);
+    if (i > 0) {
+      MC_CHECK_ARG(di.d_in == descs[i - 1].d_out && di.Cin_ld == descs[i - 1].ldc,
+                   "mc_conv_chain_fwd: member %d does not read member %d's output allocation", i, i - 1);
+    }
+  }
+  const size_t rows = (size_t)d0.B * (d0.H + 1) * (d0.W + 1);
+  for (int j = 0; j < n; ++j) {
+    const size_t out_bytes = rows * descs[j].ldc * 2;
+    for (int i = 0; i < n; ++i) {
+      if (i != j + 1)
+        MC_CHECK_ARG(!ranges_overlap(descs[i].d_in, rows * descs[i].Cin_ld * 2, descs[j].d_out, out_bytes),
+                     "mc_conv_chain_fwd: member %d reads member %d's output", i, j);
+      if (i != j)
+        MC_CHECK_ARG(!ranges_overlap(descs[i].d_out, rows * descs[i].ldc * 2, descs[j].d_out, out_bytes),
+                     "mc_conv_chain_fwd: members %d and %d write the same memory", i, j);
+    }
+  }
+  return 0;
+}
+
+extern "C" size_t mc_workspace_bytes_conv_chain(const mc_conv_desc* descs, int n) {
+  static thread_local ConvPlan L[MAX_CHAIN];
+  if (chain_plan(descs, n, L) != 0) return 0;
+  return chain_ws_words(descs, n) * sizeof(unsigned int);
+}
+
+extern "C" int mc_conv_chain_fwd(const mc_conv_desc* descs, int n, void* stream_) {
+  cudaStream_t stream = reinterpret_cast<cudaStream_t>(stream_);
+  static thread_local ConvPlan L[MAX_CHAIN];
+  int rc = chain_plan(descs, n, L);
+  if (rc) return rc;
+  const mc_conv_desc& d0 = descs[0];
+  const size_t need = chain_ws_words(descs, n) * sizeof(unsigned int);
+  MC_CHECK_ARG(d0.d_ws != nullptr && d0.ws_bytes >= need && ((uintptr_t)d0.d_ws & 15) == 0,
+               "mc_conv_chain_fwd: descs[0] needs a 16-byte aligned workspace of %zu bytes", need);
+
+  static thread_local PairParams P;
+  memset(&P, 0, sizeof(P));
+  int units = 0, cnt = 0;
+  for (int i = 0; i < n; ++i) {
+    pair_layer(L[i], &P.layer[i]);
+    units += L[i].units;
+    P.layer[i].unit_end = units;
+    P.layer[i].cnt_off = cnt;
+    cnt += (L[i].p.m_tiles + 1) / 2;
+  }
+  P.n_layers = n;
+  P.chain_ws = reinterpret_cast<unsigned int*>(d0.d_ws);
+  int max_clusters = 0;
+  rc = pair_max_clusters(&max_clusters);
+  if (rc) return rc;
+  const int clusters = units < max_clusters ? units : max_clusters;
+  g_last_plan[0] = 1; g_last_plan[1] = L[0].p.block_n; g_last_plan[2] = 1; g_last_plan[3] = 0; g_last_plan[4] = 1;
+  g_last_plan[5] = L[0].p.stages; g_last_plan[6] = 2 * clusters; g_last_plan[7] = 64;
+  conv_gemm_tcgen05_pair_kernel<<<2 * clusters, NUM_THREADS, L[0].smem_bytes, stream>>>(P);
+  MC_LAUNCH_CHECK("conv_gemm_tcgen05_pair_kernel");
+  return 0;
+}
diff --git a/modelcompression_b200/csrc/ptx_sm100.cuh b/modelcompression_b200/csrc/ptx_sm100.cuh
--- a/modelcompression_b200/csrc/ptx_sm100.cuh
+++ b/modelcompression_b200/csrc/ptx_sm100.cuh
@@ -113,6 +113,22 @@
   asm volatile("cp.async.bulk.wait_group.read %0;" ::"n"(N) : "memory");
 }
 
+__device__ __forceinline__ void bulk_wait_group_all() { asm volatile("cp.async.bulk.wait_group 0;" ::: "memory"); }
+__device__ __forceinline__ void fence_proxy_async_global() { asm volatile("fence.proxy.async.global;" ::: "memory"); }
+__device__ __forceinline__ void red_release_gpu_add(unsigned int* p, unsigned int v) {
+  asm volatile("red.release.gpu.global.add.u32 [%0], %1;" ::"l"(p), "r"(v) : "memory");
+}
+__device__ __forceinline__ unsigned int ld_acquire_gpu(const unsigned int* p) {
+  unsigned int v;
+  asm volatile("ld.acquire.gpu.global.u32 %0, [%1];" : "=r"(v) : "l"(p) : "memory");
+  return v;
+}
+__device__ __forceinline__ unsigned long long globaltimer() {
+  unsigned long long t;
+  asm volatile("mov.u64 %0, %%globaltimer;" : "=l"(t));
+  return t;
+}
+
 __device__ __forceinline__ void tmem_alloc(uint32_t* smem_dst, uint32_t ncols) {
   asm volatile("tcgen05.alloc.cta_group::1.sync.aligned.shared::cta.b32 [%0], %1;" ::"r"(smem_u32(smem_dst)),
                "r"(ncols)
@@ -164,6 +180,34 @@
 __device__ __forceinline__ void mbar_arrive_leader(uint64_t* bar) {
   asm volatile("mbarrier.arrive.release.cluster.shared::cluster.b64 _, [%0];" ::"r"(smem_u32(bar) & kPeerBitMask)
                : "memory");
+}
+__device__ __forceinline__ uint32_t mapa_shared(const void* p, uint32_t rank) {
+  uint32_t r;
+  asm volatile("mapa.shared::cluster.u32 %0, %1, %2;" : "=r"(r) : "r"(smem_u32(p)), "r"(rank));
+  return r;
+}
+__device__ __forceinline__ void st_cluster_u32(uint32_t cluster_addr, uint32_t v) {
+  asm volatile("st.shared::cluster.u32 [%0], %1;" ::"r"(cluster_addr), "r"(v) : "memory");
+}
+__device__ __forceinline__ void mbar_arrive_cluster(uint32_t cluster_addr) {
+  asm volatile("mbarrier.arrive.release.cluster.shared::cluster.b64 _, [%0];" ::"r"(cluster_addr) : "memory");
+}
+__device__ __forceinline__ void mbar_wait_cluster(uint64_t* bar, uint32_t parity) {
+  uint32_t spins = 0;
+  for (;;) {
+    uint32_t ok;
+    asm volatile(
+        "{\n\t"
+        ".reg .pred P;\n\t"
+        "mbarrier.try_wait.parity.acquire.cluster.shared::cta.b64 P, [%1], %2, %3;\n\t"
+        "selp.b32 %0, 1, 0, P;\n\t"
+        "}\n"
+        : "=r"(ok)
+        : "r"(smem_u32(bar)), "r"(parity), "r"(10000u)
+        : "memory");
+    if (ok) return;
+    if (++spins > (1u << 18)) __trap();
+  }
 }
 __device__ __forceinline__ void tmem_alloc_pair(uint32_t* smem_dst, uint32_t ncols) {
   asm volatile("tcgen05.alloc.cta_group::2.sync.aligned.shared::cta.b32 [%0], %1;" ::"r"(smem_u32(smem_dst)),
diff --git a/modelcompression_b200/engine.py b/modelcompression_b200/engine.py
--- a/modelcompression_b200/engine.py
+++ b/modelcompression_b200/engine.py
@@ -83,6 +83,9 @@
         self.use_graph = True
         self.in_hw = None
         self._compile(model)
+        self._chain_runs = self._chain_runs_of(self.ops)
+        self._items = {}
+        self._last_items = None
 
     def _new_buf(self, H, W, ld, **kw):
         self.bufs.append(_Buf(H, W, ld, **kw))
@@ -204,6 +207,31 @@
                     routed.update(int(i) if int(i) > 0 else int(i) + ind for i in block['layers'].split(','))
             self._fuse_thin_pairs(routed)
 
+    def _chain_runs_of(self, ops):
+        def chainable(op):
+            return op['kind'] == 'conv' and op['ksize'] == 3 and op['epi'] == _lib.MC_EPI_PNHWC
+
+        runs, i = [], 0
+        while i < len(ops):
+            if not chainable(ops[i]):
+                i += 1
+                continue
+            run, j, last = [ops[i]], i + 1, i
+            while j < len(ops) and len(run) < 4:
+                nxt = ops[j]
+                if chainable(nxt) and nxt['src'].buf_id == run[-1]['dst_buf'] and nxt['src'].ch_off == 0:
+                    run.append(nxt)
+                    last = j
+                elif nxt.get('src') is None or 'dst_buf' not in nxt or \
+                        nxt['src'].buf_id in {m['dst_buf'] for m in run} or \
+                        nxt['dst_buf'] in {m['src'].buf_id for m in run}:
+                    break
+                j += 1
+            if len(run) >= 2:
+                runs.append(run)
+            i = last + 1
+        return runs
+
     def _fuse_thin_pairs(self, routed):
         i = 0
         while i + 1 < len(self.ops):
@@ -562,7 +590,7 @@
         if ws is None or ws.numel() < nbytes:
             if ws is not None and self._graphs:
                 raise RuntimeError("internal: conv workspace grew after a CUDA graph captured its address")
-            ws = self._ws = torch.zeros(nbytes, dtype=torch.uint8, device=self.device)
+            ws = self._ws = torch.zeros(nbytes + 65536, dtype=torch.uint8, device=self.device)
         return ws
 
     def supports_detect(self, model):
@@ -571,6 +599,62 @@
         n = self.ops[-1]['N']
         return n == model.num_anchors * (5 + model.num_classes) and self.ops[-1]['Npad'] <= 256 and \
             len(model.anchors) == 2 * model.num_anchors and model.num_anchors <= 16
+
+    def _conv_desc(self, op, bufs, B):
+        s = op['src']
+        sb = self.bufs[s.buf_id]
+        d = _lib.mc_conv_desc()
+        d.d_in = bufs[s.buf_id].data_ptr() + 2 * s.ch_off
+        d.d_wpack = op['wpack'].data_ptr()
+        d.d_scale = op['scale'].data_ptr()
+        d.d_shift = op['shift'].data_ptr()
+        if op['epi'] != _lib.MC_EPI_NCHW_F32:
+            d.d_out = bufs[op['dst_buf']].data_ptr()
+        d.B, d.H, d.W = B, op['H'], op['W']
+        d.Cin, d.Cin_ld = op['Cin'], sb.ld
+        d.in_cols = sb.ld - s.ch_off
+        d.N, d.Npad = op['N'], op['Npad']
+        d.ksize, d.leaky, d.epi_mode = op['ksize'], op['leaky'], op['epi']
+        d.ldc, d.ch_off = op['ldc'], op['ch_off']
+        d.block_n = op.get('block_n', 0)
+        d.stages = op.get('stages', 0)
+        d.block_k = op.get('block_k', 0)
+        return d
+
+    def _launch_items(self, B, H, W, bufs):
+        key = (B, H, W)
+        items = self._items.get(key)
+        if items is not None:
+            return items
+        lib = self.lib
+        first, skip = {}, set()
+        with torch.cuda.device(self.device):
+            for run in self._chain_runs:
+                i = 0
+                while i < len(run) - 1:
+                    for j in range(len(run), i + 1, -1):
+                        descs = (_lib.mc_conv_desc * (j - i))(*[self._conv_desc(m, bufs, B) for m in run[i:j]])
+                        nbytes = int(lib.mc_workspace_bytes_conv_chain(descs, j - i))
+                        if nbytes:
+                            break
+                    else:
+                        i += 1
+                        continue
+                    members = run[i:j]
+                    ws_off = int(lib.mc_workspace_bytes_conv_fwd(ctypes.byref(descs[0])))
+                    ws_off = (ws_off + 255) // 256 * 256
+                    k0, k1 = self.ops.index(members[0]), self.ops.index(members[-1])
+                    ahead = [o for o in self.ops[k0 + 1:k1] if not any(o is m for m in members)]
+                    first[id(members[0])] = ahead + [dict(kind='conv', chain=members, ws_off=ws_off, ws_bytes=nbytes,
+                                                          name='chain@' + '+'.join(str(m['ind']) for m in members))]
+                    skip.update(id(o) for o in self.ops[k0 + 1:k1 + 1])
+                    i = j
+        items = []
+        for op in self.ops:
+            if id(op) not in skip:
+                items += first.get(id(op), [op])
+        self._items[key] = items
+        return items
 
     def _run_eager(self, x, events=None, detect=None, repeat=1):
         if x.dim() != 4:
@@ -593,7 +677,9 @@
             stream = _lib.stream_ptr()
             out = None
             self._prev_op = None
-            for op in (o for o in self.ops for _ in range(repeat if events is not None else 1)):
+            items = self._launch_items(B, H, W, bufs)
+            self._last_items = items
+            for op in (o for o in items for _ in range(repeat if events is not None else 1)):
                 kind = op['kind']
                 first_rep = op is not getattr(self, '_prev_op', None)
                 self._prev_op = op
@@ -648,16 +734,15 @@
                         raise NotImplementedError("maxpool on a channel slice")
                     _lib.check(lib.mc_maxpool2x2(bufs[s.buf_id].data_ptr(), bufs[op['dst_buf']].data_ptr(), B, s.H, s.W,
                                                  op['C'], sb.ld, self.bufs[op['dst_buf']].ld, stream), op['name'])
+                elif kind == 'conv' and 'chain' in op:
+                    members = op['chain']
+                    descs = (_lib.mc_conv_desc * len(members))(*[self._conv_desc(m, bufs, B) for m in members])
+                    ws = self._conv_workspace(op['ws_off'] + op['ws_bytes'])
+                    descs[0].d_ws, descs[0].ws_bytes = ws.data_ptr() + op['ws_off'], op['ws_bytes']
+                    _lib.check(lib.mc_conv_chain_fwd(descs, len(members), stream), op['name'])
                 elif kind == 'conv':
-                    s = op['src']
-                    d = _lib.mc_conv_desc()
-                    sb = self.bufs[s.buf_id]
-                    d.d_in = bufs[s.buf_id].data_ptr() + 2 * s.ch_off
-                    d.d_wpack = op['wpack'].data_ptr()
-                    d.d_scale = op['scale'].data_ptr()
-                    d.d_shift = op['shift'].data_ptr()
+                    d = self._conv_desc(op, bufs, B)
                     epi = op['epi']
-                    dec = None
                     if epi == _lib.MC_EPI_NCHW_F32 and detect is not None:
                         thr, only_obj, want_cls = detect
                         A, nc = self.detect_geom
@@ -671,7 +756,7 @@
                         dec.A, dec.nc, dec.conf_thresh, dec.only_objectness = A, nc, float(thr), 1 if only_obj else 0
                         for i, a in enumerate(self.detect_anchors):
                             dec.anchors[i] = float(a)
-                        epi = _lib.MC_EPI_DECODE
+                        d.epi_mode = _lib.MC_EPI_DECODE
                         out = (boxes, cls)
                         d.decode = ctypes.pointer(dec)
                         d.d_out = None
@@ -679,17 +764,6 @@
                         out = torch.empty(B, op['N'], op['H'], op['W'], dtype=torch.float32, device=self.device)
                         bufs[op['dst_buf']] = out
                         d.d_out = out.data_ptr()
-                    else:
-                        d.d_out = bufs[op['dst_buf']].data_ptr()
-                    d.B, d.H, d.W = B, op['H'], op['W']
-                    d.Cin, d.Cin_ld = op['Cin'], sb.ld
-                    d.in_cols = sb.ld - s.ch_off
-                    d.N, d.Npad = op['N'], op['Npad']
-                    d.ksize, d.leaky, d.epi_mode = op['ksize'], op['leaky'], epi
-                    d.ldc, d.ch_off = op['ldc'], op['ch_off']
-                    d.block_n = op.get('block_n', 0)
-                    d.stages = op.get('stages', 0)
-                    d.block_k = op.get('block_k', 0)
                     if op.get('ws_bytes') is None:
                         op['ws_bytes'] = int(lib.mc_workspace_bytes_conv_fwd(ctypes.byref(d)))
                     if op['ws_bytes']:
@@ -710,7 +784,7 @@
 
     @property
     def num_launches(self):
-        return len(self.ops)
+        return len(self._last_items if self._last_items is not None else self.ops)
 
     def block_activation(self, ind):
         ref = self.block_out[ind]
```
